# alasdairtran/fourierflow

Measured on AMD Instinct MI355X. Metric: training-steps/sec (whole node), F-FNO 24L 64x64 torus (torus_li/markov/24_layers), higher is better.
Workload: dtype f32

## Files before the change

### fourierflow_amd/_capi.py

```python
from __future__ import annotations

import ctypes as C

ABI_VERSION = 13
BRANCH_SELF_RANGE = 1

P = C.c_void_p
I = C.c_int
F = C.c_float
SZ = C.c_size_t
L = C.c_long


class WnDesc(C.Structure):
    _fields_ = [("g", P), ("v", P), ("w", P), ("dw", P), ("dg", P), ("dv", P),
                ("rows", C.c_int32), ("cols", C.c_int32)]


class FxPackDesc(C.Structure):
    _fields_ = [("src", P), ("dst", P), ("sh", C.c_int32), ("sc", C.c_int32), ("type", C.c_int32), ("pad_", C.c_int32)]


class FusedBranch(C.Structure):
    _fields_ = [("in_", P), ("out", P), ("resid", P), ("spec_save", P), ("planes", P), ("tw", P),
                ("B", C.c_int32), ("M", C.c_int32), ("N", C.c_int32),
                ("K", C.c_int32), ("axis", C.c_int32), ("accumulate", C.c_int32),
                ("planes_format", C.c_int32), ("tile_lines", C.c_int32), ("in_amax", P), ("out_amax", P),
                ("storage", C.c_int32), ("flags", C.c_int32), ("dft_frags", P)]


class FfOpts(C.Structure):
    _fields_ = [("in_amax", P), ("out_amax", P), ("max_workgroups", C.c_int32), ("schedule", C.c_int32),
                ("storage", C.c_int32)]


class LayerFwdDesc(C.Structure):
    _fields_ = [("a", FusedBranch), ("b", FusedBranch), ("branch_kernel", C.c_int32), ("interleave", C.c_int32),
                ("pk1", P), ("b1", P), ("pk2", P), ("b2", P), ("s_sum", P), ("resid", P), ("out", P), ("mask", P),
                ("P", C.c_int32), ("C", C.c_int32), ("H", C.c_int32), ("ff_kernel", C.c_int32),
                ("ff_schedule", C.c_int32), ("ff_max_workgroups", C.c_int32), ("pad0_", C.c_int32), ("pad1_", C.c_int32), ("out_amax", P)]


class LayerBwdDesc(C.Structure):
    _fields_ = [("a", FusedBranch), ("b", FusedBranch), ("branch_kernel", C.c_int32), ("interleave", C.c_int32),
                ("g", P), ("g2", P), ("g_sum", P), ("mask", P), ("pk1b", P), ("pk2b", P), ("ds", P), ("s", P), ("pk1", P),
                ("b1", P), ("partial", P), ("nsplit", C.c_int32), ("P", C.c_int32), ("C", C.c_int32), ("H", C.c_int32),
                ("ff_kernel", C.c_int32), ("ff_schedule", C.c_int32), ("ff_max_workgroups", C.c_int32), ("pad_", C.c_int32), ("g_amax", P), ("s_amax", P), ("ds_amax", P)]


class LayerInferDesc(C.Structure):
    _fields_ = [("a", FusedBranch), ("b", FusedBranch), ("interleave", C.c_int32), ("pad_", C.c_int32),
                ("pk1", P), ("b1", P), ("pk2", P), ("b2", P), ("resid", P), ("out", P), ("C", C.c_int32), ("H", C.c_int32),
                ("out_amax", P)]


class InferStackLayer(C.Structure):
    _fields_ = [("planes_a", P), ("planes_b", P), ("pk1", P), ("b1", P), ("pk2", P), ("b2", P)]


class InferStackDesc(C.Structure):
    _fields_ = [("a", FusedBranch), ("b", FusedBranch), ("layers", P), ("n_layers", C.c_int32), ("C", C.c_int32), ("H", C.c_int32),
                ("mode", C.c_int32), ("last_out", P), ("sync", P)]


class AmaxDesc(C.Structure):
    _fields_ = [("x", P), ("n", C.c_size_t)]


class FxRedDesc(C.Structure):
    _fields_ = [("partial", P), ("dW1", P), ("dW2", P), ("db1", P), ("db2", P)]


class FfWgDesc(C.Structure):
    _fields_ = [("s", P), ("g", P), ("pk1", P), ("b1", P), ("pk1b", P), ("partial", P), ("s_amax", P), ("g_amax", P),
                ("s2", P), ("g2", P)]


class MarkovExtra(C.Structure):
    _fields_ = [("force", P), ("mu", P), ("use_position", C.c_int32), ("pad_", C.c_int32)]


class MarkovAdvanceDesc(C.Structure):
    _fields_ = [("affine", P), ("prev", P), ("traj", P), ("feats", P), ("derived", P), ("force", P), ("mu", P),
                ("force_stride", C.c_int64), ("L", C.c_int32), ("col", C.c_int32), ("D", C.c_int32),
                ("use_position", C.c_int32), ("normalize", C.c_int32), ("low", C.c_float), ("high", C.c_float),
                ("pad_", C.c_int32)]


class PadMap(C.Structure):
    _fields_ = [("size", C.c_int32 * 3), ("padded", C.c_int32 * 3)]


class PadDesc(C.Structure):
    _fields_ = [("plain", P), ("padded", P), ("R", C.c_int32), ("Cc", C.c_int32), ("inner", C.c_int32), ("Cp", C.c_int32)]


class FwPackDesc(C.Structure):
    _fields_ = [("w", P), ("wp", P), ("wpt", P), ("K", C.c_int32), ("real", C.c_int32)]


class X3PackDesc(C.Structure):
    _fields_ = [("planes", P), ("dst", P), ("K", C.c_int32), ("format", C.c_int32)]


class TrDesc(C.Structure):
    _fields_ = [("src", P), ("dst", P), ("rows", C.c_int32), ("cols", C.c_int32)]


class IPhiParams(C.Structure):
    NAMES = ("fc0.weight", "fc0.bias", "fc_code.weight", "fc_code.bias", "fc1.weight", "fc1.bias", "fc2.weight", "fc2.bias",
             "fc3.weight", "fc3.bias", "fc4.weight", "fc4.bias")
    _fields_ = [(n, P) for n in ("fc0_w", "fc0_b", "code_w", "code_b", "fc1_w", "fc1_b", "fc2_w", "fc2_b", "fc3_w", "fc3_b",
                                 "fc4_w", "fc4_b")]


class PcHeadParams(C.Structure):
    _fields_ = [(n, P) for n in ("bs_w", "bs_b", "fc1_w", "fc1_b", "fc2_w", "fc2_b")]


class GatherField(C.Structure):
    _fields_ = [("src", P), ("dst", P), ("src_sample", C.c_int64), ("src_offset", C.c_int64), ("src_q", C.c_int64),
                ("src_r", C.c_int64), ("dst_sample", C.c_int64), ("dst_offset", C.c_int64), ("dst_q", C.c_int64),
                ("dst_r", C.c_int64), ("Q", C.c_int32), ("R", C.c_int32)]


GATHER_MAX_FIELDS = 8

SIGNATURES = {
    "ffno_build_target": (C.c_char_p, []),
    "ffno_abi_version": (I, []),
    "ffno_amax": (I, [P, SZ, P, P]),
    "ffno_amax_batched": (I, [P, I, SZ, P, P]),
    "ffno_lds_tr16_probe": (I, [P, I, P, P, P]),
    "ffno_twiddle_fill_host": (I, [P, I]),
    "ffno_dft_fwd": (I, [P, P, P, I, I, I, I, I, I, I, P]),
    "ffno_fw_pack": (I, [P, P, P, I, I, P]),
    "ffno_fw_pack_batched": (I, [P, I, I, I, P]),
    "ffno_mode_mix": (I, [P, P, P, I, I, I, I, P]),
    "ffno_dft_inv": (I, [P, P, P, P, I, I, I, I, I, I, I, I, P]),
    "ffno_fw_grad_partial": (I, [P, P, P, I, I, I, I, I, I, SZ, SZ, P]),
    "ffno_fw_grad_partial_multi": (I, [P, P, P, I, I, I, I, I, SZ, SZ, SZ, P]),
    "ffno_fw_grad_reduce_multi": (I, [P, P, I, I, I, I, SZ, I, I, P]),
    "ffno_fw_grad_partial_h2": (I, [P, P, P, I, I, I, I, I, I, SZ, SZ, P, P, I, P]),
    "ffno_fw_grad_partial_multi_h2": (I, [P, P, P, I, I, I, I, I, SZ, SZ, SZ, P, P, I, P]),
    "ffno_fw_grad_reduce": (I, [P, P, I, I, I, I, P]),
    "ffno_spectral_fused_pair": (I, [P, P, I, I, I, I, P]),
    "ffno_spectral_x3_supported": (I, [I, I, I]),
    "ffno_spectral_x3_pack_bytes": (SZ, [I, I]),
    "ffno_spectral_x3_dft_frags_bytes": (SZ, [I, I]),
    "ffno_spectral_x3_dft_frags": (I, [P, I, I, I, I, P, P]),
    "ffno_spectral_x3_pack": (I, [P, I, I, I, P]),
    "ffno_spectral_x3": (I, [P, I, I, I, I, P]),
    "ffno_spectral_x3_pair": (I, [P, P, I, I, I, I, I, P]),
    "ffno_spectral_x3_staged_supported": (I, [I, I, I]),
    "ffno_spectral_x3_staged_pair": (I, [P, P, P, P, I, I, I, I, P]),
    "ffno_layer_fwd": (I, [P, P]),
    "ffno_layer_bwd": (I, [P, P]),
    "ffno_infer_mix_bytes": (SZ, [I, I, I]),
    "ffno_layer_infer_supported": (I, [I, I, I, I, I, I, I]),
    "ffno_spectral_x3_mix_pair": (I, [P, P, I, I, P]),
    "ffno_infer_ff": (I, [P, P, P, P, P, P, P, P, I, I, P, P]),
    "ffno_infer_sum": (I, [P, P, P, I, P, P]),
    "ffno_layer_infer": (I, [P, P]),
    "ffno_infer_stack_supported": (I, [I, I, I, I, I, I, I, I]),
    "ffno_infer_stack_sync_words": (SZ, [I]),
    "ffno_infer_stack_trace_words": (SZ, [I]),
    "ffno_infer_stack": (I, [P, P]),
    "ffno_spectral_staged_pair": (I, [P, P, P, P, I, I, I, I, P]),
    "ffno_spectral_fused_supported": (I, [I, I, I]),
    "ffno_spectral_fused": (I, [P, P, P, P, P, P, I, I, I, I, I, I, I, I, I, I, P, P]),
    "ffno_spectral2d_ws_floats": (SZ, [I, I, I, I, I]),
    "ffno_spectral2d_path": (I, [I, I, I, I, I]),
    "ffno_spectral2d_weights_version": (I, [P, C.c_ulonglong]),
    "ffno_spectral2d_fwd": (I, [P, P, P, P, P, P, P, I, I, I, I, I, I, P]),
    "ffno_spectral2d_bwd": (I, [P, P, P, P, P, P, P, P, P, P, I, I, I, I, I, I, I, I, P]),
    "ffno_ff_mask_words": (SZ, [I, I]),
    "ffno_ff_fwd": (I, [P, P, P, P, P, P, P, P, P, I, I, I, P]),
    "ffno_ff_bwd_data": (I, [P, P, P, P, P, P, I, I, I, P]),
    "ffno_ff_wgrad_partial_floats": (SZ, [I, I, I]),
    "ffno_ff_bwd_weights_partial": (I, [P, P, P, P, P, I, I, I, I, P]),
    "ffno_ff_bwd_weights_reduce": (I, [P, P, P, P, P, I, I, I, I, P]),
    "ffno_ffx_supported": (I, [I, I]),
    "ffno_ffx_pack_bytes": (SZ, [I, I]),
    "ffno_ffx_pack": (I, [P, I, I, I, P]),
    "ffno_ffx_fwd": (I, [P, P, P, P, P, P, P, P, I, I, I, P]),
    "ffno_ffx_mask_unpack": (I, [P, P, I, I, I, P]),
    "ffno_ffx_bwd_data": (I, [P, P, P, P, P, I, I, I, P]),
    "ffno_ffx_fwd2": (I, [P, P, P, P, P, P, P, P, P, P, I, I, I, P, P]),
    "ffno_ffx_bwd_data2": (I, [P, P, P, P, P, P, P, I, I, I, P, P]),
    "ffno_ffx_bwd_weights_partial": (I, [P, P, P, P, P, P, I, I, I, I, P]),
    "ffno_ffx_bwd_weights_reduce": (I, [P, P, P, P, P, I, I, I, I, P]),
    "ffno_ffx_bwd_weights_reduce_batched": (I, [P, I, I, I, I, P]),
    "ffno_ffh_pack_bytes": (SZ, [I, I]),
    "ffno_ffh_pack": (I, [P, I, I, I, P]),
    "ffno_ffh_fwd2": (I, [P, P, P, P, P, P, P, P, P, P, I, I, I, P, P]),
    "ffno_ffh_bwd_data2": (I, [P, P, P, P, P, P, P, I, I, I, P, P]),
    "ffno_ffh_bwd_weights_partial": (I, [P, P, P, P, P, P, I, I, I, I, P, P, I, P]),
    "ffno_ffh_bwd_weights_partial_multi": (I, [P, I, I, I, I, I, I, I, P]),
    "ffno_layernorm_fwd": (I, [P, P, P, P, P, P, L, I, F, P]),
    "ffno_layernorm_nsplit": (I, [L]),
    "ffno_layernorm_bwd": (I, [P, P, P, P, P, P, P, P, P, P, L, I, I, P]),
    "ffno_weightnorm_fwd": (I, [P, I, I, P]),
    "ffno_weightnorm_bwd": (I, [P, I, I, P]),
    "ffno_transpose_batched": (I, [P, I, I, I, P]),
    "ffno_lift_fwd": (I, [P, P, P, P, I, I, I, P, P, P]),
    "ffno_lift_bwd": (I, [P, P, P, P, P, I, I, I, I, I, P, P]),
    "ffno_lift_bwd2": (I, [P, P, P, P, P, P, I, I, I, I, I, P, P]),
    "ffno_lift_bwd_data": (I, [P, P, P, I, I, I, P, P]),
    "ffno_lift_fwd_bf16": (I, [P, P, P, P, I, I, I, P, P, P]),
    "ffno_lift_bwd_bf16": (I, [P, P, P, P, P, I, I, I, I, I, P, P]),
    "ffno_head_fwd_bf16": (I, [P, P, P, I, I, I, I, P, P]),
    "ffno_head_bwd_bf16": (I, [P, P, P, P, P, P, I, I, I, I, P, P, P]),
    "ffno_head_fold": (I, [P, P, P, P, P, I, I, I, P]),
    "ffno_head_fwd": (I, [P, P, P, I, I, I, I, P, P]),
    "ffno_head_bwd": (I, [P, P, P, P, P, P, I, I, I, I, P, P, P]),
    "ffno_head_param_grads": (I, [P, P, P, P, P, P, P, P, I, I, I, I, P]),
    "ffno_cdft_rows": (I, [P, P, I, I, I, I, I, P]),
    "ffno_fw2d_pack": (I, [P, P, P, P, I, I, P]),
    "ffno_fw2d_grad_reduce": (I, [P, P, P, I, I, I, I, P]),
    "ffno_cdft_rows2": (I, [P, P, I, I, I, I, I, I, P]),
    "ffno_fw3d_pack": (I, [P, P, P, P, P, P, I, I, I, I, P]),
    "ffno_fw3d_grad_reduce": (I, [P, P, P, P, P, I, I, I, I, I, I, P]),
    "ffno_dct_branch": (I, [P, P, P, P, P, P, P, I, I, I, I, I, I, I, I, P]),
    "ffno_fw_pack_real": (I, [P, P, P, I, I, P]),
    "ffno_mode_mix_real": (I, [P, P, P, I, I, I, P]),
    "ffno_fw_grad_reduce_real": (I, [P, P, I, I, I, I, P]),
    "ffno_cdft_rows_ws_floats": (SZ, [I, I, I, I]),
    "ffno_cdft_rows_mfma": (I, [P, P, P, P, I, I, I, I, I, I, P]),
    "ffno_fw2d_pack2": (I, [P, P, P, P, I, I, I, P]),
    "ffno_fw2d_grad_reduce2": (I, [P, P, P, I, I, I, I, I, P]),
    "ffno_plin_supported": (I, [I, I]),
    "ffno_plin_fwd": (I, [P, I, P, P, P, P, I, P, P, P, L, I, I, I, P]),
    "ffno_plin_bwd_data": (I, [P, I, P, P, P, I, P, L, I, I, I, I, P]),
    "ffno_plin_wgrad_nsplit": (I, [L]),
    "ffno_plin_wgrad_partial_floats": (SZ, [L, I, I]),
    "ffno_plin_bwd_weights": (I, [P, I, P, P, I, P, P, P, L, I, I, I, I, P]),
    "ffno_plin_pos_fwd": (I, [P, I, P, P, P, P, P, P, P, I, P, I, I, I, I, I, I, P]),
    "ffno_plin_pos_bwd_weights": (I, [P, I, P, P, I, P, P, P, P, P, P, P, I, I, I, I, I, I, I, P]),
    "ffno_glin_supported": (I, [I, I]),
    "ffno_glin_fwd": (I, [P, P, P, P, P, L, I, I, I, F, C.c_uint32, P]),
    "ffno_glin_bwd_data": (I, [P, P, P, P, L, I, I, F, C.c_uint32, I, P]),
    "ffno_glin_wgrad_nsplit": (I, [L]),
    "ffno_glin_wgrad_partial_floats": (SZ, [L, I, I]),
    "ffno_glin_bwd_weights": (I, [P, P, P, P, P, P, L, I, I, F, C.c_uint32, I, P]),
    "ffno_dropout": (I, [P, SZ, F, C.c_uint32, P]),
    "ffno_dropout_mask": (I, [P, SZ, F, C.c_uint32, P]),
    "ffno_pad_copy": (I, [P, I, I, P]),
    "ffno_velocity_ws_floats": (SZ, [I, I, I]),
    "ffno_velocity_features": (I, [P, P, P, I, I, I, F, F, P]),
    "ffno_lploss_tmp_floats": (SZ, [I, I]),
    "ffno_lploss_fwd_bwd": (I, [P, P, P, P, P, I, I, F, P, P]),
    "ffno_markov_features": (I, [P, P, P, P, P, P, I, I, I, I, F, F, F, F, I, I, P, P]),
    "ffno_markov_traj_ws_floats": (SZ, [I, I, I, I]),
    "ffno_markov_traj_step": (I, [P, P, P, P, P, P, P, I, I, I, I, I, I, P]),
    "ffno_markov_traj_metrics": (I, [P, P, I, I, I, I, F, P]),
    "ffno_vorticity_coarsen_ws_floats": (SZ, [I, I, I]),
    "ffno_vorticity_coarsen_step": (I, [P, P, P, P, I, I, I, I, I, I, I, F, F, P]),
    "ffno_markov_corr_metrics": (I, [P, P, I, I, I, F, P]),
    "ffno_prediction_export_step": (I, [P, P, P, P, I, I, I, I, I, I, F, F, P]),
    "ffno_energy_spectrum": (I, [P, P, P, I, I, P]),
    "ffno_markov_advance": (I, [P, P, P, I, I, I, P]),
    "ffno_markov_pairs": (I, [P, P, P, P, P, P, P, P, P, P, I, I, I, I, I, I, I, I, P]),
    "ffno_markov_pairs_tf": (I, [P, P, P, P, P, P, P, I, P, P, P, I, I, I, I, I, I, I, I, P]),
    "ffno_sample_gather": (I, [P, I, P, I, I, P]),
    "ffno_adamw_flat":(I, [P, P, P, P, SZ, F, F, F, F, F, I, F, P]),
    "ffno_adam_flat": (I, [P, P, P, P, SZ, F, F, F, F, F, I, F, P]),
    "ffno_axpy": (I, [P, P, F, SZ, P]),
    "ffno_nudft_supported": (I, [I, I, I]),
    "ffno_nudft_modes": (I, [P, P, P, I, I, I, I, I, I, P]),
    "ffno_nudft_points": (I, [P, P, P, P, P, I, I, I, I, I, I, I, P]),
    "ffno_nudft_axis_supported": (I, [I, I, I]),
    "ffno_nudft_axis_modes": (I, [P, P, P, I, I, I, I, I, P]),
    "ffno_nudft_axis_points": (I, [P, P, P, P, P, I, I, I, I, I, I, P]),
    "ffno_axis_modes_to_grid": (I, [P, P, I, I, I, I, I, I, P]),
    "ffno_grid_to_axis_modes": (I, [P, P, I, I, I, I, I, I, P]),
    "ffno_iphi_supported": (I, [I]),
    "ffno_iphi_bwd_ws_floats": (SZ, [I, I, I]),
    "ffno_iphi_fwd": (I, [P, P, P, P, P, P, I, I, I, P]),
    "ffno_iphi_bwd": (I, [P, P, P, P, P, P, P, P, P, I, I, I, P]),
    "ffno_pchead_supported": (I, [I, I, I]),
    "ffno_pchead_partial_floats": (SZ, [I, I, I, I]),
    "ffno_pchead_fwd": (I, [P, P, P, P, P, I, I, I, I, P]),
    "ffno_pchead_bwd": (I, [P, P, P, P, P, P, P, P, I, I, I, I, P]),
    "ffno_ns2d_supported": (I, [I]),
    "ffno_ns2d_derivs": (I, [P, P, I, I, P]),
    "ffno_ns2d_advect": (I, [P, P, SZ, P]),
    "ffno_ns2d_cn_update": (I, [P, P, P, P, F, I, I, I, P]),
    "ffno_ns2d_cn_update_harmonic": (I, [P, P, P, P, F, F, F, F, I, I, I, P]),
    "ffno_ns2d_harmonic_force": (I, [P, P, F, F, F, I, I, I, P]),
    "ffno_kf2d_supported": (I, [I]),
    "ffno_kf2d_derivs": (I, [P, P, F, I, I, P]),
    "ffno_kf2d_stage": (I, [P, P, P, F, F, F, F, F, F, F, I, F, F, F, F, I, I, I, P]),
    "ffno_kf2d_downsample": (I, [P, P, I, I, I, F, P]),
}


def bind(lib: C.CDLL):
    for name, (res, args) in SIGNATURES.items():
        fn = getattr(lib, name)
        fn.restype = res
        fn.argtypes = args
    return list(SIGNATURES)


ERRORS = {-1: "FFNO_EINVAL (null pointer / bad size)", -2: "FFNO_EUNSUPPORTED (shape outside the compiled set)",
          -3: "FFNO_EMODES (modes > L/2+1)"}


def check(rc: int, what: str):
    if rc == 0:
        return
    if rc == -3:
        raise ValueError(f"{what}: {ERRORS[rc]}")
    if rc in (-1, -2):
        raise ValueError(f"{what}: {ERRORS[rc]}")
    raise RuntimeError(f"{what}: HIP launch failed with hipError_t {rc}")
```

### fourierflow_amd/csrc/ffx.hip

```cpp
#include <algorithm>

#include "ffno_device.h"
#include "ffno.h"

#include <string.h>

namespace ffno {

constexpr int kFfRangeTarget = 4;

template <int C, int H, int CPW_ = 1>
struct FxCfg {
    static constexpr int CPW = CPW_;
    static constexpr int NW = H / (32 * CPW);
    static constexpr int NT = NW * 64;
    static constexpr int KS = C / 16;
    static constexpr int CTO = C / 32;
    static constexpr int NV = (32 * C / 4) / NT;
    static constexpr int G = CTO * 4;
    static constexpr int GPW = G / NW;
    static constexpr int PROW = 2 * C + 16;
    static constexpr int PPLANE = 32 * PROW;
    static constexpr int TROW = 64 + 16;
    static constexpr int TPLANE = C * TROW;
    static constexpr int PART = 2 * H * C + H + C;
    static_assert(NV >= 1 && NV * NT * 4 == 32 * C, "tile staging map");
    static_assert(GPW >= 1 && GPW * NW == G, "output reduction map");
};

struct FxPackDesc {
    const float* src;
    u32x4* dst;
    int sh, sc, type, pad;
};

template <class S>
__global__ __launch_bounds__(256) void ffx_pack_kernel(const FxPackDesc* __restrict__ descs, int C, int H) {
    const FxPackDesc d = descs[blockIdx.y];
    const int KS = C / 16, CTO = C / 32, NW = H / 32;
    const int nfrag = d.type == 1 ? NW * KS : NW * CTO * 2;
    const int t = blockIdx.x * blockDim.x + threadIdx.x;
    if (t >= nfrag * 64) return;
    const int frag = t >> 6, lane = t & 63, j = lane & 31, half = lane >> 5;
    float v[8];
    if (d.type == 1) {
        const int w = frag / KS, st = frag % KS;
        for (int e = 0; e < 8; ++e) v[e] = d.src[(long)(32 * w + j) * d.sh + (long)(16 * st + 8 * half + e) * d.sc];
    } else {
        const int s2 = frag & 1, mt = (frag >> 1) % CTO, w = (frag >> 1) / CTO;
        for (int e = 0; e < 8; ++e)
            v[e] = d.src[(long)(32 * w + (e & 3) + 8 * (2 * s2 + (e >> 2)) + 4 * half) * d.sh + (long)(32 * mt + j) * d.sc];
    }
    const typename S::Frag f = S::split8(v[0], v[1], v[2], v[3], v[4], v[5], v[6], v[7]);
    FFNO_UNROLL
    for (int p = 0; p < S::NP; ++p) d.dst[(frag * S::NP + p) * 64 + lane] = S::plane(f, p);
}

__device__ __forceinline__ Bf3 load_frag(const u32x4* __restrict__ pk, int frag, int lane) {
    Bf3 f;
    f.hi = pk[(frag * 3 + 0) * 64 + lane];
    f.mid = pk[(frag * 3 + 1) * 64 + lane];
    f.lo = pk[(frag * 3 + 2) * 64 + lane];
    return f;
}

__device__ __forceinline__ uint32_t push_sign(uint32_t acc, uint32_t x) {
    return plat::shift_in_msb(acc, x);
}
__device__ __forceinline__ uint32_t bit_mask(uint32_t x, int b) {
    return plat::bit_to_mask(x, b);
}

__device__ __forceinline__ Bf3 lds_frag(const char* base, int plane_bytes, int off) {
    Bf3 f;
    f.hi = *reinterpret_cast<const u32x4*>(base + off);
    f.mid = *reinterpret_cast<const u32x4*>(base + plane_bytes + off);
    f.lo = *reinterpret_cast<const u32x4*>(base + 2 * plane_bytes + off);
    return f;
}

__device__ __forceinline__ void stage4(char* base, int plane_bytes, int off, float x, float y, float z, float w) {
    unsigned h0, m0, l0, h1, m1, l1;
    split3_pair(x, y, h0, m0, l0);
    split3_pair(z, w, h1, m1, l1);
    *reinterpret_cast<uint2*>(base + off) = make_uint2(h0, h1);
    *reinterpret_cast<uint2*>(base + plane_bytes + off) = make_uint2(m0, m1);
    *reinterpret_cast<uint2*>(base + 2 * plane_bytes + off) = make_uint2(l0, l1);
}

template <class S>
__device__ __forceinline__ typename S::Frag load_frag_s(const u32x4* __restrict__ pk, int frag, int lane) {
    typename S::Frag f;
    FFNO_UNROLL
    for (int p = 0; p < S::NP; ++p) S::set_plane(f, p, pk[(frag * S::NP + p) * 64 + lane]);
    return f;
}
template <class S>
__device__ __forceinline__ typename S::Frag lds_frag_s(const char* base, int plane_bytes, int off) {
    typename S::Frag f;
    FFNO_UNROLL
    for (int p = 0; p < S::NP; ++p) S::set_plane(f, p, *reinterpret_cast<const u32x4*>(base + p * plane_bytes + off));
    return f;
}
template <class S>
__device__ __forceinline__ void stage4_s(char* base, int plane_bytes, int off, float x, float y, float z, float w) {
    uint2 pl[S::NP];
    S::split4(x, y, z, w, pl);
    FFNO_UNROLL
    for (int p = 0; p < S::NP; ++p) *reinterpret_cast<uint2*>(base + p * plane_bytes + off) = pl[p];
}

template <int C, int H, bool BWD, class S, class ST = StF32>
__global__ __launch_bounds__((FxCfg<C, H>::NT)) void ffx_chain_kernel(const typename ST::T* __restrict__ in,
                                                                     const typename ST::T* __restrict__ in2,
                                                                     typename ST::T* sum_out,
                                                                     const typename ST::T* resid,
                                                                     const u32x4* __restrict__ pk1,
                                                                     const float* __restrict__ bias1,
                                                                     const u32x4* __restrict__ pk2,
                                                                     const float* __restrict__ bias2, typename ST::T* out,
                                                                     uint32_t* mask, int P, const unsigned* in_amax, unsigned* out_amax) {
    using F = FxCfg<C, H>;
    constexpr int NW = F::NW, KS = F::KS, CTO = F::CTO, NV = F::NV, G = F::G, GPW = F::GPW, CPW = F::CPW;
    __shared__ __attribute__((aligned(16))) char sp[2][S::NP * F::PPLANE];
    __shared__ __attribute__((aligned(16))) float part[2][NW * G * 64 * 4];
    __shared__ __attribute__((aligned(16))) float b1s[H];
    __shared__ float b2s[C];

    const int tid = threadIdx.x, lane = tid & 63, wave = tid >> 6;
    const int j = lane & 31, half = lane >> 5;
    const int ntiles = (P + 31) >> 5;
    const float gscale = (S::SCALED && in_amax) ? range_scale(*in_amax, 1, kFfRangeTarget) : 1.f;
    const float rgscale = 1.f / gscale;
    float omax = 0.f;
    __shared__ float rfold[NW];

    using Frag = typename S::Frag;
    Frag A1[CPW][KS], A2[CPW][CTO][2];
    FFNO_UNROLL
    for (int ch = 0; ch < CPW; ++ch) {
        const int q = wave * CPW + ch;
        FFNO_UNROLL
        for (int st = 0; st < KS; ++st) A1[ch][st] = load_frag_s<S>(pk1, q * KS + st, lane);
        FFNO_UNROLL
        for (int mt = 0; mt < CTO; ++mt) {
            FFNO_UNROLL
            for (int s2 = 0; s2 < 2; ++s2) A2[ch][mt][s2] = load_frag_s<S>(pk2, (q * CTO + mt) * 2 + s2, lane);
        }
    }
    if (!BWD) {
        for (int e = tid; e < H; e += F::NT) b1s[e] = bias1[e] * gscale;
        for (int e = tid; e < C; e += F::NT) b2s[e] = bias2[e];
    }

    float4 nS[NV];
    typename ST::Raw4 pA[NV], pB[NV];
    auto gload_raw = [&](int tile) {
        FFNO_UNROLL
        for (int v = 0; v < NV; ++v) {
            const int f = tid + v * F::NT;
            const long px = (long)tile * 32 + f / (C / 4);
            pA[v] = pB[v] = ST::zero4();
            if (px < P) {
                const long off = px * C + 4 * (f % (C / 4));
                pA[v] = ST::ldr4(in + off);
                if (in2) pB[v] = ST::ldr4(in2 + off);
            }
        }
    };
    auto consume = [&](int tile) {
        FFNO_UNROLL
        for (int v = 0; v < NV; ++v) {
            nS[v] = ST::w4(pA[v]);
            if (in2) {
                const float4 b = ST::w4(pB[v]);
                nS[v].x += b.x, nS[v].y += b.y, nS[v].z += b.z, nS[v].w += b.w;
                nS[v] = st_rnd4<ST>(nS[v]);
                if (sum_out) {
                    const int f = tid + v * F::NT;
                    const long px = (long)tile * 32 + f / (C / 4);
                    if (px < P) ST::st4(sum_out + px * C + 4 * (f % (C / 4)), nS[v]);
                }
            }
            if (S::SCALED) nS[v].x *= gscale, nS[v].y *= gscale, nS[v].z *= gscale, nS[v].w *= gscale;
        }
    };
    auto stage = [&](int buf) {
        FFNO_UNROLL
        for (int v = 0; v < NV; ++v) {
            const int f = tid + v * F::NT;
            stage4_s<S>(sp[buf], F::PPLANE, (f / (C / 4)) * F::PROW + (f % (C / 4)) * 8, nS[v].x, nS[v].y, nS[v].z, nS[v].w);
        }
    };
    typename ST::Raw4 rres[GPW], rnext[GPW];
    auto rload = [&](int tile) {
        const long px = (long)tile * 32 + j;
        FFNO_UNROLL
        for (int u = 0; u < GPW; ++u) {
            const int gi = wave * GPW + u;
            rnext[u] = ST::zero4();
            if (!BWD && resid && px < P)
                rnext[u] = ST::ldr4(resid + px * C + 32 * (gi >> 2) + 8 * (gi & 3) + 4 * half);
        }
    };
    auto reduce = [&](int tile, int buf) {
        const long px = (long)tile * 32 + j;
        FFNO_UNROLL
        for (int u = 0; u < GPW; ++u) {
// ... 1544 lines not shown
```

### fourierflow_amd/csrc/pointwise.hip

```cpp
#include "ffno_device.h"
#include "ffno.h"

#include <math.h>

namespace ffno {

static inline int pw_status() {
    hipError_t e = hipGetLastError();
    return e == hipSuccess ? FFNO_OK : (int)e;
}

__global__ __launch_bounds__(256) void wn_fwd_kernel(const ffno_wn_desc* __restrict__ descs) {
    const ffno_wn_desc d = descs[blockIdx.y];
    const int lane = threadIdx.x & 63, row = blockIdx.x * 4 + (threadIdx.x >> 6);
    if (row >= d.rows) return;
    const float* v = d.v + (long)row * d.cols;
    float ss = 0.f;
    for (int c = lane; c < d.cols; c += 64) ss += v[c] * v[c];
    ss = wave_sum(ss);
    const float scale = d.g[row] / sqrtf(ss);
    float* w = d.w + (long)row * d.cols;
    for (int c = lane; c < d.cols; c += 64) w[c] = v[c] * scale;
}

__global__ __launch_bounds__(256) void wn_bwd_kernel(const ffno_wn_desc* __restrict__ descs) {
    const ffno_wn_desc d = descs[blockIdx.y];
    const int lane = threadIdx.x & 63, row = blockIdx.x * 4 + (threadIdx.x >> 6);
    if (row >= d.rows) return;
    const float* v = d.v + (long)row * d.cols;
    const float* dw = d.dw + (long)row * d.cols;
    float ss = 0.f, dot = 0.f;
    for (int c = lane; c < d.cols; c += 64) {
        ss += v[c] * v[c];
        dot += dw[c] * v[c];
    }
    ss = wave_sum(ss);
    dot = wave_sum(dot);
    const float inv = 1.f / sqrtf(ss);
    const float dg = dot * inv;
    const float g = d.g[row];
    if (lane == 0) d.dg[row] = dg;
    float* dv = d.dv + (long)row * d.cols;
    for (int c = lane; c < d.cols; c += 64) dv[c] = g * inv * (dw[c] - dg * inv * v[c]);
}

__global__ __launch_bounds__(256) void transpose_batched_kernel(const ffno_tr_desc* __restrict__ descs) {
    __shared__ float tile[32][33];
    const ffno_tr_desc d = descs[blockIdx.z];
    const int c0 = blockIdx.x * 32, r0 = blockIdx.y * 32;
    if (c0 >= d.cols || r0 >= d.rows) return;
    const int tx = threadIdx.x & 31, ty = threadIdx.x >> 5;
    for (int yy = ty; yy < 32; yy += 8)
        if (r0 + yy < d.rows && c0 + tx < d.cols) tile[yy][tx] = d.src[(long)(r0 + yy) * d.cols + c0 + tx];
    __syncthreads();
    for (int yy = ty; yy < 32; yy += 8)
        if (c0 + yy < d.cols && r0 + tx < d.rows) d.dst[(long)(c0 + yy) * d.rows + r0 + tx] = tile[tx][yy];
}

struct PadMapDev {
    int s1, s2;
    int p0, p1, p2;
    int s0;
    int enabled;
    __device__ __forceinline__ long map(long p) const {
        if (!enabled) return p;
        const long z = p % s2, t = p / s2;
        const long y = t % s1, t2 = t / s1;
        const long x = t2 % s0, b = t2 / s0;
        return ((b * p0 + x) * p1 + y) * p2 + z;
    }
};

static inline PadMapDev make_padmap(const ffno_padmap* pm) {
    PadMapDev d;
    d.enabled = 0;
    d.s0 = d.s1 = d.s2 = d.p0 = d.p1 = d.p2 = 1;
    if (pm) {
        d.s0 = pm->size[0];
        d.s1 = pm->size[1];
        d.s2 = pm->size[2];
        d.p0 = pm->padded[0];
        d.p1 = pm->padded[1];
        d.p2 = pm->padded[2];
        d.enabled = (d.s0 != d.p0 || d.s1 != d.p1 || d.s2 != d.p2) ? 1 : 0;
    }
    return d;
}

template <int C, class ST = StF32>
__global__ __launch_bounds__(512) void lift_fwd_kernel(const float* __restrict__ x, const float* __restrict__ W,
                                                       const float* __restrict__ b, typename ST::T* __restrict__ out, int P,
                                                       int Cin, PadMapDev pm, unsigned* out_amax) {
    FFNO_DYN_SMEM(smem);
    __shared__ float rfold[16];
    float omax = 0.f;
    float* Wt = reinterpret_cast<float*>(smem);
    for (int e = threadIdx.x; e < Cin * C; e += blockDim.x) Wt[(e % Cin) * C + (e / Cin)] = W[e];
    for (int e = threadIdx.x; e < C; e += blockDim.x) Wt[Cin * C + e] = b[e];
    __syncthreads();
    constexpr int LPP = C / 4;
    const int PPB = (int)blockDim.x / LPP;
    const int c4 = (threadIdx.x % LPP) * 4, pl = threadIdx.x / LPP;
    const float4 bias = *reinterpret_cast<const float4*>(Wt + Cin * C + c4);
    const long stride = (long)gridDim.x * PPB;
    for (long p = (long)blockIdx.x * PPB + pl; p < P; p += 2 * stride) {
        const long p1 = p + stride;
        const bool two = p1 < P;
        float4 acc0 = bias, acc1 = bias;
        const float* xp0 = x + p * Cin;
        const float* xp1 = x + (two ? p1 : p) * Cin;
        for (int i = 0; i < Cin; ++i) {
            const float xv0 = xp0[i], xv1 = xp1[i];
            const float4 w = *reinterpret_cast<const float4*>(Wt + i * C + c4);
            acc0.x = fmaf(xv0, w.x, acc0.x);
            acc0.y = fmaf(xv0, w.y, acc0.y);
            acc0.z = fmaf(xv0, w.z, acc0.z);
            acc0.w = fmaf(xv0, w.w, acc0.w);
            acc1.x = fmaf(xv1, w.x, acc1.x);
            acc1.y = fmaf(xv1, w.y, acc1.y);
            acc1.z = fmaf(xv1, w.z, acc1.z);
            acc1.w = fmaf(xv1, w.w, acc1.w);
        }
        ST::st4(out + pm.map(p) * C + c4, acc0);
        acc0 = st_rnd4<ST>(acc0);
        omax = fmaxf(fmaxf(omax, fmaxf(fabsf(acc0.x), fabsf(acc0.y))), fmaxf(fabsf(acc0.z), fabsf(acc0.w)));
        if (two) {
            ST::st4(out + pm.map(p1) * C + c4, acc1);
            acc1 = st_rnd4<ST>(acc1);
            omax = fmaxf(fmaxf(omax, fmaxf(fabsf(acc1.x), fabsf(acc1.y))), fmaxf(fabsf(acc1.z), fabsf(acc1.w)));
        }
    }
    if (out_amax) range_fold(omax, rfold, (int)blockDim.x >> 6, out_amax);
}

template <int C, class ST = StF32>
__global__ __launch_bounds__(256) void lift_bwd_partial_kernel(const float* __restrict__ x,
                                                               const typename ST::T* __restrict__ gout,
                                                               const typename ST::T* __restrict__ gout2,
                                                               float* __restrict__ partial, int P, int Cin,
                                                               int chunk, PadMapDev pm) {
    constexpr int TP = 32;
    constexpr int MAXU = (C * 64) / 256;
    __shared__ __attribute__((aligned(16))) float gs[TP * C];
    __shared__ float xs[TP * 64];
    const int npairs = C * (Cin + 1);
    float acc[MAXU];
    FFNO_UNROLL
    for (int u = 0; u < MAXU; ++u) acc[u] = 0.f;
    const long pbeg = (long)blockIdx.x * chunk, pend = min((long)P, pbeg + chunk);
    for (long p0 = pbeg; p0 < pend; p0 += TP) {
        const int np = (int)min((long)TP, pend - p0);
        __syncthreads();
        for (int e4 = threadIdx.x; e4 < TP * C / 4; e4 += 256) {
            const int e = 4 * e4;
            float4 gvv = make_float4(0.f, 0.f, 0.f, 0.f);
            if ((e / C) < np) {
                const long off = pm.map(p0 + e / C) * C + (e % C);
                gvv = ST::ld4(gout + off);
                if (gout2) {
                    const float4 g2 = ST::ld4(gout2 + off);
                    gvv = make_float4(ST::rnd(gvv.x + g2.x), ST::rnd(gvv.y + g2.y), ST::rnd(gvv.z + g2.z), ST::rnd(gvv.w + g2.w));
                }
            }
            *reinterpret_cast<float4*>(gs + e) = gvv;
        }
        for (int e = threadIdx.x; e < TP * (Cin + 1); e += 256) {
            const int pp = e / (Cin + 1), i = e % (Cin + 1);
            xs[pp * 64 + i] = (pp < np) ? (i < Cin ? x[(p0 + pp) * Cin + i] : 1.f) : 0.f;
        }
        __syncthreads();
        FFNO_UNROLL
        for (int u = 0; u < MAXU; ++u) {
            const int e = u * 256 + threadIdx.x;
            if (e < npairs) {
                const int c = e % C, i = e / C;
                float a = acc[u];
                for (int pp = 0; pp < TP; ++pp) a = fmaf(gs[pp * C + c], xs[pp * 64 + i], a);
                acc[u] = a;
            }
        }
    }
    FFNO_UNROLL
    for (int u = 0; u < MAXU; ++u) {
        const int e = u * 256 + threadIdx.x;
        if (e < npairs) partial[(long)blockIdx.x * npairs + e] = acc[u];
    }
}

template <int C>
__global__ __launch_bounds__(256) void lift_bwd_data_kernel(const float* __restrict__ gout, const float* __restrict__ W,
                                                            float* __restrict__ dx, int P, int Cin, PadMapDev pm) {
    FFNO_DYN_SMEM(smem);
    float* Wt = reinterpret_cast<float*>(smem);
    for (int e = threadIdx.x; e < Cin * C; e += blockDim.x) Wt[(e % Cin) * C + (e / Cin)] = W[e];
    __syncthreads();
    for (long p = (long)blockIdx.x * 256 + threadIdx.x; p < P; p += (long)gridDim.x * 256) {
        const float* g = gout + pm.map(p) * C;
        float4 gv[C / 4];
        FFNO_UNROLL
        for (int q = 0; q < C / 4; ++q) gv[q] = *reinterpret_cast<const float4*>(g + 4 * q);
        for (int i = 0; i < Cin; ++i) {
            float a = 0.f;
            FFNO_UNROLL
            for (int q = 0; q < C / 4; ++q) {
                const float4 w = *reinterpret_cast<const float4*>(Wt + i * C + 4 * q);
                a = fmaf(gv[q].x, w.x, a), a = fmaf(gv[q].y, w.y, a), a = fmaf(gv[q].z, w.z, a), a = fmaf(gv[q].w, w.w, a);
            }
            dx[p * Cin + i] = a;
        }
    }
}

__global__ __launch_bounds__(256) void lift_bwd_reduce_kernel(const float* __restrict__ partial, float* dW, float* db,
                                                              int Cin, int C, int nsplit, int accumulate) {
    __shared__ float red[256];
    const int npairs = C * (Cin + 1);
    const int e = blockIdx.x * 4 + (threadIdx.x & 3), lane = threadIdx.x >> 2;
    float a = 0.f;
    if (e < npairs)
        for (int sp = lane; sp < nsplit; sp += 64) a += partial[(long)sp * npairs + e];
    red[threadIdx.x] = a;
    __syncthreads();
    for (int w = 128; w >= 4; w >>= 1) {
        if ((int)threadIdx.x < w) red[threadIdx.x] += red[threadIdx.x + w];
        __syncthreads();
    }
    if (threadIdx.x < 4 && e < npairs) {
        const int c = e % C, i = e / C;
        float* dst = (i < Cin) ? (dW + c * Cin + i) : (db + c);
        *dst = accumulate ? (*dst + red[threadIdx.x]) : red[threadIdx.x];
    }
}

static constexpr int kHeadMaxOut = 8;

__global__ __launch_bounds__(256) void head_fold_kernel(const float* __restrict__ Wa, const float* __restrict__ ca,
                                                        const float* __restrict__ Wb, const float* __restrict__ cb,
                                                        float* fold, int C, int D, int O) {
    const int e = blockIdx.x * 4 + (threadIdx.x >> 6), lane = threadIdx.x & 63;
    if (e >= O * (C + 1)) return;
    const int o = e / (C + 1), c = e % (C + 1);
    float s = 0.f;
    for (int jd = lane; jd < D; jd += 64) s = fmaf(Wb[o * D + jd], (c == C) ? ca[jd] : Wa[jd * C + c], s);
    FFNO_UNROLL
    for (int m = 32; m >= 1; m >>= 1) s += __shfl_xor(s, m);
    if (lane == 0) fold[e] = s + ((c == C) ? cb[o] : 0.f);
}

template <int C, class ST = StF32>
__global__ __launch_bounds__(256) void head_fwd_kernel(const typename ST::T* __restrict__ b, const float* __restrict__ fold,
                                                       float* y, int P, int O, int accumulate, PadMapDev pm) {
    constexpr int LPP = C / 4, PPB = 256 / LPP;
    const int c4 = (threadIdx.x % LPP) * 4, pl = threadIdx.x / LPP;
    const long npass = ((long)P + PPB - 1) / PPB;
    for (long pass = blockIdx.x; pass < npass; pass += gridDim.x) {
        const long p = pass * PPB + pl;
        float4 v = make_float4(0.f, 0.f, 0.f, 0.f);
        if (p < P) v = ST::ld4(b + pm.map(p) * C + c4);
        for (int o = 0; o < O; ++o) {
            const float4 w = *reinterpret_cast<const float4*>(fold + o * (C + 1) + c4);
            float d = v.x * w.x + v.y * w.y + v.z * w.z + v.w * w.w;
            FFNO_UNROLL
            for (int m = LPP / 2; m >= 1; m >>= 1) d += __shfl_xor(d, m);
            if (p < P && c4 == 0) y[p * O + o] = (accumulate ? y[p * O + o] : 0.f) + d + fold[o * (C + 1) + C];
        }
    }
}

template <int C, class ST = StF32>
__global__ __launch_bounds__(1024) void head_bwd_kernel(const typename ST::T* __restrict__ b, const float* __restrict__ gy,
                                                        const float* __restrict__ fold, typename ST::T* __restrict__ gb,
                                                        float* __restrict__ partial, int P, int O, PadMapDev pm,
                                                        unsigned* gb_amax) {
    constexpr int LPP = C / 4;
    const int PPB = (int)blockDim.x / LPP;
    __shared__ float red[(1024 / LPP) * (C + 4)];
    __shared__ float rfold[16];
    float omax = 0.f;
    const int l = threadIdx.x % LPP, c4 = l * 4, pl = threadIdx.x / LPP;
    float4 acc[kHeadMaxOut];
    float sg[kHeadMaxOut];
    FFNO_UNROLL
    for (int o = 0; o < kHeadMaxOut; ++o) {
        acc[o] = make_float4(0.f, 0.f, 0.f, 0.f);
        sg[o] = 0.f;
    }
    for (long p = (long)blockIdx.x * PPB + pl; p < P; p += (long)gridDim.x * PPB) {
        const long q = pm.map(p);
        const float4 v = ST::ld4(b + q * C + c4);
        float4 gsum = make_float4(0.f, 0.f, 0.f, 0.f);
        FFNO_UNROLL
        for (int o = 0; o < kHeadMaxOut; ++o) {
            if (o < O) {
                const float g = gy[p * O + o];
                const float4 w = *reinterpret_cast<const float4*>(fold + o * (C + 1) + c4);
                acc[o].x = fmaf(g, v.x, acc[o].x);
                acc[o].y = fmaf(g, v.y, acc[o].y);
                acc[o].z = fmaf(g, v.z, acc[o].z);
                acc[o].w = fmaf(g, v.w, acc[o].w);
                sg[o] += g;
                gsum.x = fmaf(g, w.x, gsum.x);
                gsum.y = fmaf(g, w.y, gsum.y);
                gsum.z = fmaf(g, w.z, gsum.z);
                gsum.w = fmaf(g, w.w, gsum.w);
            }
        }
        if (gb) ST::st4(gb + q * C + c4, gsum);
        gsum = st_rnd4<ST>(gsum);
        omax = fmaxf(fmaxf(omax, fmaxf(fabsf(gsum.x), fabsf(gsum.y))), fmaxf(fabsf(gsum.z), fabsf(gsum.w)));
    }
    if (gb && gb_amax) range_fold(omax, rfold, (int)blockDim.x >> 6, gb_amax);
    for (int o = 0; o < O; ++o) {
        __syncthreads();
        float* r = red + pl * (C + 4);
        FFNO_UNROLL
        for (int oo = 0; oo < kHeadMaxOut; ++oo) {
            if (oo == o) {
                r[c4] = acc[oo].x;
                r[c4 + 1] = acc[oo].y;
                r[c4 + 2] = acc[oo].z;
                r[c4 + 3] = acc[oo].w;
                if (l == 0) r[C] = sg[oo];
            }
        }
        __syncthreads();
        for (int e = threadIdx.x; e <= C; e += blockDim.x) {
            float s = 0.f;
            for (int qq = 0; qq < PPB; ++qq) s += red[qq * (C + 4) + e];
            partial[((long)blockIdx.x * O + o) * (C + 1) + e] = s;
        }
    }
}

__global__ __launch_bounds__(256) void head_bwd_reduce_kernel(const float* __restrict__ partial, float* red, int C, int O,
                                                              int nsplit) {
    __shared__ float sm[256];
    const int n = O * (C + 1);
    const int e = blockIdx.x * 4 + (threadIdx.x & 3), lane = threadIdx.x >> 2;
    float a = 0.f;
    if (e < n)
        for (int sp = lane; sp < nsplit; sp += 64) a += partial[(long)sp * n + e];
    sm[threadIdx.x] = a;
    __syncthreads();
    for (int w = 128; w >= 4; w >>= 1) {
        if ((int)threadIdx.x < w) sm[threadIdx.x] += sm[threadIdx.x + w];
        __syncthreads();
    }
    if (threadIdx.x < 4 && e < n) red[e] = sm[threadIdx.x];
}

__global__ __launch_bounds__(256) void head_param_grads_kernel(const float* __restrict__ red, const float* __restrict__ Wa,
                                                               const float* __restrict__ ca, const float* __restrict__ Wb,
                                                               float* dWa, float* dca, float* dWb, float* dcb, int C, int D,
                                                               int O, int accumulate) {
    const int n0 = O * D, n1 = n0 + D, n2 = n1 + D * C, n3 = n2 + O;
    for (int idx = blockIdx.x * blockDim.x + threadIdx.x; idx < n3; idx += gridDim.x * blockDim.x) {
        if (idx < n0) {
            const int e = idx, o = e / D, jd = e % D;
            float s = ca[jd] * red[o * (C + 1) + C];
            for (int c = 0; c < C; ++c) s = fmaf(Wa[jd * C + c], red[o * (C + 1) + c], s);
            dWb[e] = accumulate ? dWb[e] + s : s;
        } else if (idx < n1) {
            const int jd = idx - n0;
            float t = 0.f;
            for (int o = 0; o < O; ++o) t = fmaf(Wb[o * D + jd], red[o * (C + 1) + C], t);
            dca[jd] = accumulate ? dca[jd] + t : t;
        } else if (idx < n2) {
            const int e = idx - n1;
            float t = 0.f;
            for (int o = 0; o < O; ++o) t = fmaf(Wb[o * D + e / C], red[o * (C + 1) + e % C], t);
            dWa[e] = accumulate ? dWa[e] + t : t;
        } else {
            const int o = idx - n2;
            const float S = red[o * (C + 1) + C];
            dcb[o] = accumulate ? dcb[o] + S : S;
        }
    }
}

struct MarkovSrc {
    const float* x;
    const float* force;
    const float* mu;
    int Cx, use_pos;
    long fstride;
};

__device__ __forceinline__ float markov_normalized(float v, const float* derived, int c, int D) {
    return (v - derived[c]) / derived[D + c];
}

__device__ __forceinline__ float markov_raw(const MarkovSrc& src, long p, int c, int M, int N, float low, float high) {
    if (c < src.Cx) return src.x[p * src.Cx + c];
    c -= src.Cx;
    if (src.use_pos) {
        if (c < 2) {
            const int n = (int)(p % N), m = (int)((p / N) % M);
            const int idx = c == 0 ? m : n, size = c == 0 ? M : N;
            return size > 1 ? low + (high - low) * (float)idx / (float)(size - 1) : low;
// ... 229 lines not shown
        metrics[4 + t] = l / (float)B;
        metrics[4 + n_steps + t] = p / (float)B;
    }
    float f = 0.f;
    for (int b = threadIdx.x; b < B; b += 256) {
        float d2 = 0.f, y2 = 0.f;
        for (int t = 0; t < n_steps; ++t) d2 += slice_sum(t, b, 5), y2 += slice_sum(t, b, 3);
        f += sqrtf(d2) / sqrtf(y2);
    }
    full[threadIdx.x] = f;
    __syncthreads();
    if (threadIdx.x == 0) {
        float lf = 0.f, la = 0.f, pm = 0.f;
        for (int i = 0; i < min(B, 256); ++i) lf += full[i];
        int diverged = n_steps;
        for (int t = n_steps - 1; t >= 0; --t)
            if (metrics[4 + n_steps + t] < threshold) diverged = t;
        for (int t = 0; t < n_steps; ++t) la += metrics[4 + t], pm += metrics[4 + n_steps + t];
        metrics[0] = la / (float)n_steps;
        metrics[1] = lf / (float)B;
        metrics[2] = (float)diverged;
        metrics[3] = pm / (float)n_steps;
    }
}

struct MarkovPairs {
    const float* data;
    const int32_t* ids;
    float *x, *y, *dx, *dy;
    const float* f;
    float* f_out;
    const float* mu;
    float* mu_out;
    int n, T, t0, k, P, total;
    int Tf;
};

__global__ __launch_bounds__(256) void markov_pairs_kernel(MarkovPairs a) {
    const int i = blockIdx.y, S = gridDim.x;
    const int chunk = (a.n + S - 1) / S;
    const int beg = blockIdx.x * chunk, end = min(a.n, beg + chunk);
    const int p = a.ids[i];
    const bool ok = (unsigned)p < (unsigned)a.total;
    const int b = ok ? p / a.P : 0, t = ok ? a.t0 + p % a.P : 0;
    const float nan = __builtin_nanf("");
    const long src = (long)b * a.n, dst = (long)i * a.n;
    if (a.mu_out && blockIdx.x == 0 && threadIdx.x == 0) a.mu_out[i] = ok ? a.mu[b] : nan;
    for (int e = beg + threadIdx.x; e < end; e += 256) {
        float xv = nan, yv = nan, pv = nan, fv = nan;
        if (ok) {
            const float* row = a.data + (src + e) * a.T;
            xv = row[t];
            if (a.y || a.dy) yv = row[t + a.k];
            if (a.dx) pv = row[t - a.k];
            if (a.f_out) fv = a.Tf ? a.f[(src + e) * a.Tf + t + a.k] : a.f[src + e];
        }
        if (a.x) a.x[dst + e] = xv;
        if (a.y) a.y[dst + e] = yv;
        if (a.dx) a.dx[dst + e] = xv - pv;
        if (a.dy) a.dy[dst + e] = yv - xv;
        if (a.f_out) a.f_out[dst + e] = fv;
    }
}

struct GatherField {
    const float* src;
    float* dst;
    long src_sample, src_offset, src_q, src_r, dst_sample, dst_offset, dst_q, dst_r;
    int Q, R, vec;
};
struct SampleGather {
    GatherField f[FFNO_GATHER_MAX_FIELDS];
    const int32_t* ids;
    int n;
};

__global__ __launch_bounds__(256) void sample_gather_kernel(SampleGather a) {
    const GatherField& g = a.f[blockIdx.z];
    const int i = blockIdx.y, S = gridDim.x;
    const int id = a.ids[i];
    if ((unsigned)id >= (unsigned)a.n) return;
    const float* sp = g.src + (long)id * g.src_sample + g.src_offset;
    float* dp = g.dst + (long)i * g.dst_sample + g.dst_offset;
    const bool wide = g.vec && (((uintptr_t)sp | (uintptr_t)dp) & 15) == 0;
    const int W = wide ? 4 : 1;
    const int U = (g.R + W - 1) / W;
    const long units = (long)g.Q * U;
    const long chunk = (units + S - 1) / S;
    const long beg = blockIdx.x * chunk, end = beg + chunk < units ? beg + chunk : units;
    for (long u = beg + threadIdx.x; u < end; u += 256) {
        const long q = u / U;
        const int r = (int)(u - q * U) * W;
        const float* s = sp + q * g.src_q + r * g.src_r;
        float* d = dp + q * g.dst_q + r * g.dst_r;
        if (wide && r + 4 <= g.R) {
            *reinterpret_cast<float4*>(d) = *reinterpret_cast<const float4*>(s);
        } else {
            const int m = min(W, g.R - r);
            for (int j = 0; j < m; ++j) d[j * g.dst_r] = s[j * g.src_r];
        }
    }
}

__global__ __launch_bounds__(256) void adamw_kernel(float* __restrict__ p, const float* __restrict__ g,
                                                    float* __restrict__ m, float* __restrict__ v, size_t n, float lr,
                                                    float beta1, float beta2, float eps, float wd, float bc1,
                                                    float bc2_sqrt, float gscale, int decoupled) {
    for (size_t i = (size_t)blockIdx.x * 256 + threadIdx.x; i < n; i += (size_t)gridDim.x * 256) {
        const float gi = decoupled ? g[i] * gscale : fmaf(wd, p[i], g[i] * gscale);
        float pi = decoupled ? p[i] * (1.f - lr * wd) : p[i];
        const float mi = beta1 * m[i] + (1.f - beta1) * gi;
        const float vi = beta2 * v[i] + (1.f - beta2) * gi * gi;
        m[i] = mi;
        v[i] = vi;
        const float denom = sqrtf(vi) / bc2_sqrt + eps;
        pi -= (lr / bc1) * (mi / denom);
        p[i] = pi;
    }
}

__global__ __launch_bounds__(256) void axpy_kernel(float* __restrict__ y, const float* __restrict__ x, float alpha,
                                                   size_t n) {
    for (size_t i = (size_t)blockIdx.x * 256 + threadIdx.x; i < n; i += (size_t)gridDim.x * 256)
        y[i] = fmaf(alpha, x[i], y[i]);
}

}

using namespace ffno;

__global__ __launch_bounds__(256) void amax_kernel(const float* __restrict__ x, size_t n, unsigned* word) {
    __shared__ float red[4];
    float m = 0.f;
    const size_t n4 = n / 4;
    for (size_t i = (size_t)blockIdx.x * 256 + threadIdx.x; i < n4; i += (size_t)gridDim.x * 256) {
        const float4 v = reinterpret_cast<const float4*>(x)[i];
        m = fmaxf(fmaxf(m, fmaxf(fabsf(v.x), fabsf(v.y))), fmaxf(fabsf(v.z), fabsf(v.w)));
    }
    for (size_t i = 4 * n4 + (size_t)blockIdx.x * 256 + threadIdx.x; i < n; i += (size_t)gridDim.x * 256) m = fmaxf(m, fabsf(x[i]));
    range_fold(m, red, 4, word);
}
extern "C" int ffno_amax(const float* x, size_t n, uint32_t* word, void* stream) {
    if (!x || !word || n == 0 || (reinterpret_cast<uintptr_t>(x) & 15u)) return FFNO_EINVAL;
    const int blocks = (int)std::min<size_t>((size_t)4 * device_cu_count(), (n / 4 + 255) / 256 + 1);
    FFNO_LAUNCH(amax_kernel, dim3(blocks), dim3(256), 0, (hipStream_t)stream, x, n, word);
    hipError_t e = hipGetLastError();
    return e == hipSuccess ? FFNO_OK : (int)e;
}

struct AmaxDesc {
    const float* x;
    size_t n;
};
__global__ __launch_bounds__(256) void amax_batched_kernel(const AmaxDesc* __restrict__ descs, unsigned* word) {
    __shared__ float red[4];
    const AmaxDesc d = descs[blockIdx.y];
    const size_t act = min((size_t)gridDim.x, (d.n + 1023) / 1024);
    if (blockIdx.x >= act) return;
    float m = 0.f;
    const bool al = (reinterpret_cast<uintptr_t>(d.x) & 15u) == 0;
    const size_t n4 = al ? d.n / 4 : 0;
    for (size_t i = (size_t)blockIdx.x * 256 + threadIdx.x; i < n4; i += act * 256) {
        const float4 v = reinterpret_cast<const float4*>(d.x)[i];
        m = fmaxf(fmaxf(m, fmaxf(fabsf(v.x), fabsf(v.y))), fmaxf(fabsf(v.z), fabsf(v.w)));
    }
    for (size_t i = 4 * n4 + (size_t)blockIdx.x * 256 + threadIdx.x; i < d.n; i += act * 256) m = fmaxf(m, fabsf(d.x[i]));
    range_fold(m, red, 4, word);
}
extern "C" int ffno_amax_batched(const ffno_amax_desc* descs_dev, int n, size_t max_n, uint32_t* word, void* stream) {
    static_assert(sizeof(ffno_amax_desc) == sizeof(AmaxDesc), "descriptor layout");
    if (!descs_dev || !word || n <= 0 || max_n == 0) return FFNO_EINVAL;
    const int blocks = (int)std::min<size_t>(128, (max_n + 2047) / 2048);
    FFNO_LAUNCH(amax_batched_kernel, dim3(blocks, n), dim3(256), 0, (hipStream_t)stream,
                reinterpret_cast<const AmaxDesc*>(descs_dev), word);
    hipError_t e = hipGetLastError();
    return e == hipSuccess ? FFNO_OK : (int)e;
}

extern "C" const char* ffno_build_target(void) {
    return FFNO_BUILD_TARGET;
}
extern "C" int ffno_abi_version(void) { return FFNO_ABI_VERSION; }

extern "C" int ffno_twiddle_fill_host(float* tw_host, int L) {
    if (!tw_host || L <= 0) return FFNO_EINVAL;
    const double inv = 1.0 / sqrt((double)L);
    for (int jx = 0; jx < L; ++jx) {
        const double th = 2.0 * M_PI * (double)jx / (double)L;
        double c = cos(th), s = sin(th);
        if (4 * jx == L || 4 * jx == 3 * L) c = 0.0;
        if (jx == 0 || 2 * jx == L) s = 0.0;
        tw_host[jx] = (float)(c * inv);
        tw_host[L + jx] = (float)(s * inv);
    }
    return FFNO_OK;
}

extern "C" int ffno_weightnorm_fwd(const ffno_wn_desc* descs_dev, int n, int max_rows, void* stream) {
    if (!descs_dev || n <= 0 || max_rows <= 0) return FFNO_EINVAL;
    FFNO_LAUNCH(wn_fwd_kernel, dim3((max_rows + 3) / 4, n), dim3(256), 0, (hipStream_t)stream, descs_dev);
    return pw_status();
}
extern "C" int ffno_weightnorm_bwd(const ffno_wn_desc* descs_dev, int n, int max_rows, void* stream) {
    if (!descs_dev || n <= 0 || max_rows <= 0) return FFNO_EINVAL;
    FFNO_LAUNCH(wn_bwd_kernel, dim3((max_rows + 3) / 4, n), dim3(256), 0, (hipStream_t)stream, descs_dev);
    return pw_status();
}

extern "C" int ffno_transpose_batched(const ffno_tr_desc* descs_dev, int n, int max_rows, int max_cols, void* stream) {
    if (!descs_dev || n <= 0 || max_rows <= 0 || max_cols <= 0) return FFNO_EINVAL;
    FFNO_LAUNCH(transpose_batched_kernel, dim3((max_cols + 31) / 32, (max_rows + 31) / 32, n), dim3(256), 0,
                (hipStream_t)stream, descs_dev);
    return pw_status();
}

template <class ST>
static int lift_fwd_impl(const float* x, const float* W, const float* b, typename ST::T* out, int P, int Cin, int C,
                         const ffno_padmap* pad, uint32_t* out_amax, void* stream) {
    if (!x || !W || !b || !out || P <= 0 || Cin <= 0) return FFNO_EINVAL;
    if (Cin > 63) return FFNO_EUNSUPPORTED;
    const PadMapDev pm = make_padmap(pad);
    const size_t smem = sizeof(float) * (size_t)(Cin + 1) * C;
    const int ppb = 512 / (C / 4);
    const dim3 grid((unsigned)min(((long)P + ppb - 1) / ppb, (long)device_cu_count())), block(512);
    hipStream_t s = (hipStream_t)stream;
    if (C == 64)
        FFNO_LAUNCH((lift_fwd_kernel<64, ST>), grid, block, smem, s, x, W, b, out, P, Cin, pm, out_amax);
    else if (C == 32)
        FFNO_LAUNCH((lift_fwd_kernel<32, ST>), grid, block, smem, s, x, W, b, out, P, Cin, pm, out_amax);
    else
        return FFNO_EUNSUPPORTED;
    return pw_status();
}
extern "C" int ffno_lift_fwd(const float* x, const float* W, const float* b, float* out, int P, int Cin, int C,
                             const ffno_padmap* pad, uint32_t* out_amax, void* stream) {
    return lift_fwd_impl<StF32>(x, W, b, out, P, Cin, C, pad, out_amax, stream);
}
extern "C" int ffno_lift_fwd_bf16(const float* x, const float* W, const float* b, uint16_t* out, int P, int Cin, int C,
                                  const ffno_padmap* pad, uint32_t* out_amax, void* stream) {
    return lift_fwd_impl<StBf16>(x, W, b, out, P, Cin, C, pad, out_amax, stream);
}

template <class ST>
static int lift_bwd_impl(const float* x, const typename ST::T* gout, const typename ST::T* gout2, float* partial, float* dW, float* db,
                         int P, int Cin, int C, int nsplit, int accumulate, const ffno_padmap* pad, void* stream) {
    if (!x || !gout || !partial || !dW || !db || P <= 0 || Cin <= 0 || nsplit <= 0) return FFNO_EINVAL;
    if (Cin > 63) return FFNO_EUNSUPPORTED;
    const PadMapDev pm = make_padmap(pad);
    const int chunk = (P + nsplit - 1) / nsplit;
    hipStream_t s = (hipStream_t)stream;
    if (C == 64)
        FFNO_LAUNCH((lift_bwd_partial_kernel<64, ST>), dim3(nsplit), dim3(256), 0, s, x, gout, gout2, partial, P, Cin, chunk, pm);
    else if (C == 32)
        FFNO_LAUNCH((lift_bwd_partial_kernel<32, ST>), dim3(nsplit), dim3(256), 0, s, x, gout, gout2, partial, P, Cin, chunk, pm);
    else
        return FFNO_EUNSUPPORTED;
    int rc = pw_status();
    if (rc) return rc;
    const int npairs = C * (Cin + 1);
    FFNO_LAUNCH(lift_bwd_reduce_kernel, dim3((npairs + 3) / 4), dim3(256), 0, s, partial, dW, db, Cin, C, nsplit,
                accumulate);
    return pw_status();
}
extern "C" int ffno_lift_bwd(const float* x, const float* gout, float* partial, float* dW, float* db, int P,
                             int Cin, int C, int nsplit, int accumulate, const ffno_padmap* pad, void* stream) {
    return lift_bwd_impl<StF32>(x, gout, nullptr, partial, dW, db, P, Cin, C, nsplit, accumulate, pad, stream);
}
extern "C" int ffno_lift_bwd2(const float* x, const float* gout, const float* gout2, float* partial, float* dW, float* db, int P,
                              int Cin, int C, int nsplit, int accumulate, const ffno_padmap* pad, void* stream) {
    return lift_bwd_impl<StF32>(x, gout, gout2, partial, dW, db, P, Cin, C, nsplit, accumulate, pad, stream);
}
extern "C" int ffno_lift_bwd_bf16(const float* x, const uint16_t* gout, float* partial, float* dW, float* db, int P,
                                  int Cin, int C, int nsplit, int accumulate, const ffno_padmap* pad, void* stream) {
    return lift_bwd_impl<StBf16>(x, gout, nullptr, partial, dW, db, P, Cin, C, nsplit, accumulate, pad, stream);
}

extern "C" int ffno_lift_bwd_data(const float* gout, const float* W, float* dx, int P, int Cin, int C,
                                  const ffno_padmap* pad, void* stream) {
    if (!gout || !W || !dx || P <= 0 || Cin <= 0) return FFNO_EINVAL;
    if (Cin > 63) return FFNO_EUNSUPPORTED;
    const PadMapDev pm = make_padmap(pad);
    const dim3 grid((unsigned)std::min<long>(((long)P + 255) / 256, 4L * device_cu_count()));
    const size_t smem = sizeof(float) * (size_t)Cin * C;
    hipStream_t s = (hipStream_t)stream;
    if (C == 64)
        FFNO_LAUNCH((lift_bwd_data_kernel<64>), grid, dim3(256), smem, s, gout, W, dx, P, Cin, pm);
    else if (C == 32)
        FFNO_LAUNCH((lift_bwd_data_kernel<32>), grid, dim3(256), smem, s, gout, W, dx, P, Cin, pm);
    else
        return FFNO_EUNSUPPORTED;
    return pw_status();
}

extern "C" int ffno_head_fold(const float* Wa, const float* ca, const float* Wb, const float* cb, float* fold,
                              int C, int D, int O, void* stream) {
    if (!Wa || !ca || !Wb || !cb || !fold || C <= 0 || D <= 0 || O <= 0) return FFNO_EINVAL;
    if (O > kHeadMaxOut) return FFNO_EUNSUPPORTED;
    FFNO_LAUNCH(head_fold_kernel, dim3((O * (C + 1) + 3) / 4), dim3(256), 0, (hipStream_t)stream, Wa, ca, Wb, cb, fold, C,
                D, O);
    return pw_status();
}

template <class ST>
static int head_fwd_impl(const typename ST::T* b, const float* fold, float* y, int P, int C, int O, int accumulate,
                         const ffno_padmap* pad, void* stream) {
    if (!b || !fold || !y || P <= 0 || O <= 0) return FFNO_EINVAL;
    if (O > kHeadMaxOut) return FFNO_EUNSUPPORTED;
    const PadMapDev pm = make_padmap(pad);
    const int ppb = 256 / (C / 4);
    const dim3 grid((unsigned)min(((long)P + ppb - 1) / ppb, 2048L)), block(256);
    hipStream_t s = (hipStream_t)stream;
    if (C == 64)
        FFNO_LAUNCH((head_fwd_kernel<64, ST>), grid, block, 0, s, b, fold, y, P, O, accumulate, pm);
    else if (C == 32)
        FFNO_LAUNCH((head_fwd_kernel<32, ST>), grid, block, 0, s, b, fold, y, P, O, accumulate, pm);
    else
        return FFNO_EUNSUPPORTED;
    return pw_status();
}
extern "C" int ffno_head_fwd(const float* b, const float* fold, float* y, int P, int C, int O, int accumulate,
// ... 236 lines not shown
```

### fourierflow_amd/csrc/spectral.hip

```cpp
#include "ffno_device.h"
#include "ffno_lines.h"
#include "ffno.h"

namespace ffno {

template <int CT>
struct ColVec;
template <>
struct ColVec<1> {
    float v[1];
    __device__ __forceinline__ void load(const float* p) { v[0] = p[0]; }
    __device__ __forceinline__ void store(float* p) const { p[0] = v[0]; }
};
template <>
struct ColVec<2> {
    float v[2];
    __device__ __forceinline__ void load(const float* p) {
        float2 t = *reinterpret_cast<const float2*>(p);
        v[0] = t.x;
        v[1] = t.y;
    }
    __device__ __forceinline__ void store(float* p) const { *reinterpret_cast<float2*>(p) = make_float2(v[0], v[1]); }
};

template <int C, int RT>
__device__ __forceinline__ void dft_fwd_body(const float* __restrict__ x, float* __restrict__ spec,
                                             const float* __restrict__ tw, int R, int L, int K, const LineMap& lm,
                                             int scale_ck, int bidx, int nblk, int Lv) {
    constexpr int CT = C / 32;
    FFNO_DYN_SMEM(smem);
    float* tws = reinterpret_cast<float*>(smem);
    for (int i = threadIdx.x; i < 2 * L; i += blockDim.x) tws[i] = tw[i];
    __syncthreads();

    const int lane = threadIdx.x & 63, wave = threadIdx.x >> 6;
    const int j = lane & 31, half = lane >> 5;
    const int nsteps = (Lv + 1) >> 1;

    const long nitems = (long)R * RT;
    for (long item = (long)bidx * 4 + wave; item < nitems; item += (long)nblk * 4) {
        const int line = (int)(item / RT), rt = (int)(item % RT);
        const int kk = 32 * rt + j, k = kk >> 1, ri = kk & 1;
        const bool valid = kk < 2 * K;
        const float ck = (scale_ck && !(k == 0 || 2 * k == L)) ? 2.f : 1.f;
        const float amul = valid ? (ri ? -ck : ck) : 0.f;
        const int tbase = ri ? L : 0;
        const int km = valid ? k : 0;
        const int step = (2 * km) % L;
        int idx = (km * half) % L;
        const float* xl = x + lm.base(line) + CT * j;
        f32x16 acc[CT];
        FFNO_UNROLL
        for (int ct = 0; ct < CT; ++ct) acc[ct] = zero16();
        constexpr int UN = 8;
        ColVec<CT> b[UN], bn[UN];
        auto load_trip = [&](ColVec<CT> (&dst)[UN], int t0) {
            FFNO_UNROLL
            for (int u = 0; u < UN; ++u) {
                const int n = 2 * (t0 + u) + half;
                if (n < Lv) {
                    dst[u].load(xl + (long)n * lm.elem_stride);
                } else {
                    FFNO_UNROLL
                    for (int ct = 0; ct < CT; ++ct) dst[u].v[ct] = 0.f;
                }
            }
        };
        load_trip(bn, 0);
        for (int t0 = 0; t0 < nsteps; t0 += UN) {
            FFNO_UNROLL
            for (int u = 0; u < UN; ++u) b[u] = bn[u];
            if (t0 + UN < nsteps) load_trip(bn, t0 + UN);
            FFNO_UNROLL
            for (int u = 0; u < UN; ++u) {
                const float a = amul * tws[tbase + idx];
                idx += step;
                if (idx >= L) idx -= L;
                FFNO_UNROLL
                for (int ct = 0; ct < CT; ++ct) acc[ct] = mfma32(a, b[u].v[ct], acc[ct]);
            }
        }
        FFNO_UNROLL
        for (int r = 0; r < 16; ++r) {
            const int kr = 32 * rt + drow(r, half);
            if (kr < 2 * K) {
                ColVec<CT> o;
                FFNO_UNROLL
                for (int ct = 0; ct < CT; ++ct) o.v[ct] = acc[ct][r];
                o.store(spec + (((long)(kr >> 1) * R + line) * 2 + (kr & 1)) * C + CT * j);
            }
        }
    }
}

template <int C, int RT>
__global__ __launch_bounds__(256) void dft_fwd_kernel(const float* __restrict__ x, float* __restrict__ spec,
                                                      const float* __restrict__ tw, int R, int L, int K,
                                                      LineMap lm, int scale_ck) {
    dft_fwd_body<C, RT>(x, spec, tw, R, L, K, lm, scale_ck, blockIdx.x, gridDim.x, L);
}

template <int C, int RT>
__global__ __launch_bounds__(256) void dft_fwd_lv_kernel(const float* __restrict__ x, float* __restrict__ spec,
                                                         const float* __restrict__ tw, int R, int L, int K, LineMap lm,
                                                         int scale_ck, int Lv) {
    dft_fwd_body<C, RT>(x, spec, tw, R, L, K, lm, scale_ck, blockIdx.x, gridDim.x, Lv);
}

struct StageArgs {
    const float* in;
    float* out;
    const float* resid;
    const float* planes;
    const float* tw;
    int R, L, K;
    LineMap lm;
    int accumulate;
};

template <int C, int RT>
__global__ __launch_bounds__(256) void dft_fwd_pair_kernel(StageArgs a, StageArgs b, int n0, int scale_ck) {
    if ((int)blockIdx.x < n0)
        dft_fwd_body<C, RT>(a.in, a.out, a.tw, a.R, a.L, a.K, a.lm, scale_ck, blockIdx.x, n0, a.L);
    else
        dft_fwd_body<C, RT>(b.in, b.out, b.tw, b.R, b.L, b.K, b.lm, scale_ck, blockIdx.x - n0, gridDim.x - n0, b.L);
}

template <int C>
__device__ __forceinline__ void dft_inv_body(const float* __restrict__ spec, float* out, const float* resid,
                                             const float* __restrict__ tw, int R, int L, int K, const LineMap& lm,
                                             int apply_ck, int accumulate, int bidx, int nblk, int Lv) {
    constexpr int CT = C / 32;
    FFNO_DYN_SMEM(smem);
    float* tws = reinterpret_cast<float*>(smem);
    for (int i = threadIdx.x; i < 2 * L; i += blockDim.x) tws[i] = tw[i];
    __syncthreads();

    const int lane = threadIdx.x & 63, wave = threadIdx.x >> 6;
    const int j = lane & 31, half = lane >> 5;
    const float sgn = half ? -1.f : 1.f;
    const int tbase = half ? L : 0;
    const int RTtot = (Lv + 31) >> 5;

    const int NP = (RTtot + 1) >> 1;
    const long nitems = (long)R * NP;
    for (long item = (long)bidx * 4 + wave; item < nitems; item += (long)nblk * 4) {
        const int line = (int)(item / NP);
        const long lbase = lm.base(line) + CT * j;
        {
            const int rt0 = 2 * (int)(item % NP);
            const int n0 = 32 * rt0 + j, n1 = n0 + 32;
            const int st0 = n0 % L, st1 = n1 % L;
            int i0 = 0, i1 = 0;
            f32x16 acc[2][CT];
            FFNO_UNROLL
            for (int q = 0; q < 2; ++q) {
                FFNO_UNROLL
                for (int ct = 0; ct < CT; ++ct) acc[q][ct] = zero16();
            }
            ColVec<CT> b[4], bn[4];
            auto load_trip = [&](ColVec<CT> (&dst)[4], int t0) {
                FFNO_UNROLL
                for (int u = 0; u < 4; ++u) {
                    const int t = t0 + u;
                    if (t < K) {
                        dst[u].load(spec + (((long)t * R + line) * 2 + half) * C + CT * j);
                    } else {
                        FFNO_UNROLL
                        for (int ct = 0; ct < CT; ++ct) dst[u].v[ct] = 0.f;
                    }
                }
            };
            load_trip(bn, 0);
            for (int t0 = 0; t0 < K; t0 += 4) {
                FFNO_UNROLL
                for (int u = 0; u < 4; ++u) b[u] = bn[u];
                if (t0 + 4 < K) load_trip(bn, t0 + 4);
                FFNO_UNROLL
                for (int u = 0; u < 4; ++u) {
                    const int t = t0 + u;
                    const float ck = (apply_ck && !(t == 0 || 2 * t == L)) ? 2.f : 1.f;
                    const float a0 = sgn * ck * tws[tbase + i0];
                    const float a1 = sgn * ck * tws[tbase + i1];
                    i0 += st0;
                    if (i0 >= L) i0 -= L;
                    i1 += st1;
                    if (i1 >= L) i1 -= L;
                    FFNO_UNROLL
                    for (int ct = 0; ct < CT; ++ct) {
                        acc[0][ct] = mfma32(a0, b[u].v[ct], acc[0][ct]);
                        acc[1][ct] = mfma32(a1, b[u].v[ct], acc[1][ct]);
                    }
                }
            }
            FFNO_UNROLL
            for (int q = 0; q < 2; ++q) {
                FFNO_UNROLL
                for (int r = 0; r < 16; ++r) {
                    const int n = 32 * (rt0 + q) + drow(r, half);
                    if (n < Lv) {
                        const long a = lbase + (long)n * lm.elem_stride;
                        ColVec<CT> o;
                        FFNO_UNROLL
                        for (int ct = 0; ct < CT; ++ct) o.v[ct] = acc[q][ct][r];
                        if (accumulate) {
                            ColVec<CT> p;
                            p.load(out + a);
                            FFNO_UNROLL
                            for (int ct = 0; ct < CT; ++ct) o.v[ct] += p.v[ct];
                        }
                        if (resid) {
                            ColVec<CT> p;
                            p.load(resid + a);
                            FFNO_UNROLL
                            for (int ct = 0; ct < CT; ++ct) o.v[ct] += p.v[ct];
                        }
                        o.store(out + a);
                    }
                }
            }
        }
    }
}

template <int C>
__global__ __launch_bounds__(256) void dft_inv_kernel(const float* __restrict__ spec, float* out,
                                                      const float* resid, const float* __restrict__ tw,
                                                      int R, int L, int K, LineMap lm, int apply_ck,
                                                      int accumulate) {
    dft_inv_body<C>(spec, out, resid, tw, R, L, K, lm, apply_ck, accumulate, blockIdx.x, gridDim.x, L);
}

template <int C>
__global__ __launch_bounds__(256) void dft_inv_lv_kernel(const float* __restrict__ spec, float* out, const float* resid,
                                                         const float* __restrict__ tw, int R, int L, int K, LineMap lm,
                                                         int apply_ck, int accumulate, int Lv) {
    dft_inv_body<C>(spec, out, resid, tw, R, L, K, lm, apply_ck, accumulate, blockIdx.x, gridDim.x, Lv);
}

template <int C>
__global__ __launch_bounds__(256) void dft_inv_pair_kernel(StageArgs a, StageArgs b, int n0, int apply_ck) {
    if ((int)blockIdx.x < n0)
        dft_inv_body<C>(a.in, a.out, a.resid, a.tw, a.R, a.L, a.K, a.lm, apply_ck, a.accumulate, blockIdx.x, n0, a.L);
    else
        dft_inv_body<C>(b.in, b.out, b.resid, b.tw, b.R, b.L, b.K, b.lm, apply_ck, b.accumulate, blockIdx.x - n0,
                        gridDim.x - n0, b.L);
}

__global__ void fw_pack_kernel(const float* __restrict__ w, float* __restrict__ wp, float* __restrict__ wpt,
                               int C, int K) {
    const long total = (long)C * C * K * 2;
    for (long e = (long)blockIdx.x * blockDim.x + threadIdx.x; e < total; e += (long)gridDim.x * blockDim.x) {
        const int o = e % C;
        const int i = (e / C) % C;
        const int ri = (e / ((long)C * C)) % 2;
        const int k = e / ((long)C * C * 2);
        const float v = w[(((long)i * C + o) * K + k) * 2 + ri];
        wp[e] = v;
        wpt[(((long)k * 2 + ri) * C + o) * C + i] = v;
    }
}

__global__ void fw_pack_batched_kernel(const ffno_fwpack_desc* __restrict__ descs, int C) {
    const ffno_fwpack_desc d = descs[blockIdx.y];
    const int K = d.K;
    const long total = (long)C * C * K * 2;
    for (long e = (long)blockIdx.x * blockDim.x + threadIdx.x; e < total; e += (long)gridDim.x * blockDim.x) {
        const int o = e % C;
        const int i = (e / C) % C;
        const int ri = (e / ((long)C * C)) % 2;
        const int k = e / ((long)C * C * 2);
        const float v = d.real ? (ri ? 0.f : d.w[((long)i * C + o) * K + k]) : d.w[(((long)i * C + o) * K + k) * 2 + ri];
        d.wp[e] = v;
        d.wpt[(((long)k * 2 + ri) * C + o) * C + i] = v;
    }
}

template <int C, bool REAL = false>
__device__ __forceinline__ void mode_mix_body(const float* __restrict__ spec_in, const float* __restrict__ planes,
                                              float* __restrict__ spec_out, int R, int conj_t, int k) {
    constexpr int CT = C / 32;
    constexpr int PARTS = REAL ? 1 : 2;
    __shared__ __attribute__((aligned(16))) float smem_mix[2 * C * C];
    float* Wr = smem_mix;
    float* Wi = Wr + C * C;

    const int lane = threadIdx.x & 63, wave = threadIdx.x >> 6;
    const int j = lane & 31, half = lane >> 5;
    const float* xin = spec_in + (long)k * R * 2 * C;
    float* yout = spec_out + (long)k * R * 2 * C;
    const int nitems = PARTS * ((R + 31) >> 5);
    int item = blockIdx.x * 4 + wave;

    float a[C];
    auto load_a = [&](int it) {
        const int row = (it / PARTS) * 32 + j;
        FFNO_UNROLL
        for (int u = 0; u < C / 4; ++u) {
            float4 v = make_float4(0.f, 0.f, 0.f, 0.f);
            if (it < nitems && row < R) v = *reinterpret_cast<const float4*>(xin + ((long)row * 2 + half) * C + 4 * u);
            a[4 * u + 0] = v.x;
            a[4 * u + 1] = v.y;
            a[4 * u + 2] = v.z;
            a[4 * u + 3] = v.w;
        }
    };
    load_a(item);
    {
        const float* pk = planes + (long)k * 2 * C * C;
        for (int i = threadIdx.x * 4; i < PARTS * C * C; i += blockDim.x * 4)
            *reinterpret_cast<float4*>(Wr + i) = *reinterpret_cast<const float4*>(pk + i);
    }
    __syncthreads();

    for (; item < nitems; item += gridDim.x * 4) {
        const int row0 = (item / PARTS) * 32, q = REAL ? 0 : (item & 1);
        const float* plane = (REAL || half == q) ? Wr : Wi;
        const float sign = REAL ? 1.f
                                : (conj_t == 0 ? ((half == 1 && q == 0) ? -1.f : 1.f) : ((half == 0 && q == 1) ? -1.f : 1.f));
        f32x16 acc[CT];
        FFNO_UNROLL
        for (int ct = 0; ct < CT; ++ct) acc[ct] = zero16();
        FFNO_UNROLL
        for (int t = 0; t < C; ++t) {
            if ((t & 7) == 0) FFNO_SCHED_FENCE();
            FFNO_UNROLL
            for (int ct = 0; ct < CT; ++ct) {
                const float b = sign * plane[t * C + 32 * ct + j];
                acc[ct] = mfma32(a[t], b, acc[ct]);
            }
        }
        FFNO_SCHED_FENCE();
        load_a(item + gridDim.x * 4);
        FFNO_UNROLL
        for (int ct = 0; ct < CT; ++ct) {
            FFNO_UNROLL
            for (int r = 0; r < 16; ++r) {
                const int row = row0 + drow(r, half);
                if (row < R) yout[((long)row * 2 + q) * C + 32 * ct + j] = acc[ct][r];
            }
        }
    }
}

template <int C>
__global__ __launch_bounds__(256, 2) void mode_mix_kernel(const float* __restrict__ spec_in,
                                                       const float* __restrict__ planes,
                                                       float* __restrict__ spec_out, int R, int K,
                                                       int conj_t) {
    mode_mix_body<C>(spec_in, planes, spec_out, R, conj_t, blockIdx.y);
}

template <int C>
__global__ __launch_bounds__(256, 2) void mode_mix_real_kernel(const float* __restrict__ spec_in,
                                                            const float* __restrict__ planes,
                                                            float* __restrict__ spec_out, int R, int K) {
    mode_mix_body<C, true>(spec_in, planes, spec_out, R, 0, blockIdx.y);
}

template <int C>
__global__ __launch_bounds__(256, 2) void mode_mix_pair_kernel(StageArgs a, StageArgs b, int conj_t) {
    if ((int)blockIdx.y < a.K)
        mode_mix_body<C>(a.in, a.planes, a.out, a.R, conj_t, blockIdx.y);
    else
        mode_mix_body<C>(b.in, b.planes, b.out, b.R, conj_t, blockIdx.y - a.K);
}

template <int C>
struct FusedCfg {
    static constexpr int LINES = 8;
    static constexpr int KMAX = 1024 / C;
    static constexpr int LSMAX = 2 * KMAX * C + 4;
};

struct FusedArgs {
    const float* in;
    float* out;
    const float* resid;
    float* spec_save;
    const float* planes;
    const float* tw;
    int R, L, K;
    LineMap lm;
    int fwd_ck, inv_ck, conj_t, accumulate;
    unsigned* out_amax;
};

template <int C>
__device__ __forceinline__ void spectral_fused_body(const FusedArgs& A, int bidx) {
    const float* __restrict__ in = A.in;
    float* out = A.out;
    const float* resid = A.resid;
    float* __restrict__ spec_save = A.spec_save;
    const float* __restrict__ planes = A.planes;
    const float* __restrict__ tw = A.tw;
    const int R = A.R, L = A.L, K = A.K;
    const LineMap lm = A.lm;
    const int fwd_ck = A.fwd_ck, inv_ck = A.inv_ck, conj_t = A.conj_t, accumulate = A.accumulate;
    using F = FusedCfg<C>;
    constexpr int CT = C / 32;
    __shared__ __attribute__((aligned(16))) float XS[F::LINES * F::LSMAX];
    FFNO_DYN_SMEM(smem);
    float* tws = reinterpret_cast<float*>(smem);
    for (int i = threadIdx.x; i < 2 * L; i += blockDim.x) tws[i] = tw[i];

    const int lane = threadIdx.x & 63, wave = threadIdx.x >> 6;
    const int j = lane & 31, half = lane >> 5;
    const int LS = 2 * K * C + 4;
    const int line = bidx * F::LINES + wave;
    const bool live = line < R;
    float* xs = XS + wave * LS;
    __syncthreads();

    {
        const int kk = j, k = kk >> 1, ri = kk & 1;
        const bool rowok = kk < 2 * K;
        const float ck = (fwd_ck && !(k == 0 || 2 * k == L)) ? 2.f : 1.f;
        const float amul = rowok ? (ri ? -ck : ck) : 0.f;
        const int tbase = ri ? L : 0;
        const int km = rowok ? k : 0;
        const int step = (2 * km) % L;
        int idx = (km * half) % L;
        f32x16 acc[CT];
        FFNO_UNROLL
        for (int ct = 0; ct < CT; ++ct) acc[ct] = zero16();
        if (live) {
            const float* xl = in + lm.base(line) + CT * j;
            const int nsteps = (L + 1) >> 1;
// ... 1288 lines not shown
```

### fourierflow_amd/csrc/spectral_x3.hip

```cpp
#include <type_traits>

#include "ffno_device.h"
#include "ffno_lines.h"
#include "ffno_x3_dft.h"
#include "ffno_infer_body.h"
#include "ffno.h"

namespace ffno {

struct X3Cfg {
    static constexpr int C = 64;
    static constexpr int NW = 8;
    static constexpr int KK = 32;
    static constexpr int RS = 68;
    static constexpr int LSF = KK * RS + 8;
    static constexpr int FRAG = 3 * 64;
    static constexpr int MODE_FRAGS = 16;
};

struct X3Args {
    const float* in;
    float* out;
    const float* resid;
    float* spec_save;
    const u32x4* wpk;
    const float* tw;
    int R, L, K;
    LineMap lm;
    int fwd_ck, inv_ck, conj_t, accumulate;
    const unsigned* in_amax;
    unsigned* out_amax;
    const u32x4* dft;
    u32x4* mix_out;
    float* mix_scale;
    int self_range;
};

struct X3PackDesc {
    const float* planes;
    u32x4* dst;
    int K, format;
};

__global__ __launch_bounds__(256) void x3_pack_kernel(const X3PackDesc* __restrict__ descs) {
    constexpr int C = X3Cfg::C;
    const X3PackDesc d = descs[blockIdx.y];
    const int nfrag = d.K * X3Cfg::MODE_FRAGS;
    const int t = blockIdx.x * blockDim.x + threadIdx.x;
    if (t >= nfrag * 64) return;
    const int frag = t >> 6, lane = t & 63, j = lane & 31, half = lane >> 5;
    const int pt = frag & 3, st = (frag >> 2) & 3, k = frag >> 4;
    const int p = pt >> 1, tt = pt & 1;
    const float* src = d.planes + ((long)(k * 2 + p) * C + (16 * st + 8 * half)) * C + 2 * j + tt;
    float v[8];
    FFNO_UNROLL
    for (int e = 0; e < 8; ++e) v[e] = src[(long)e * C];
    if (d.format == 1) {
        const Hf2 f = split2_8(v[0], v[1], v[2], v[3], v[4], v[5], v[6], v[7]);
        const int fo = (k * 4 + pt) * 4 + st;
        d.dst[(fo * 2 + 0) * 64 + lane] = f.hi;
        d.dst[(fo * 2 + 1) * 64 + lane] = f.lo;
        return;
    }
    if (d.format == 2) {
        const int fm = frag & 15, s2 = fm & 1, t16 = (fm >> 1) & 3, pp = fm >> 3;
        const int j16 = lane & 15, g = lane >> 4;
        const float* src2 = d.planes + ((long)(k * 2 + pp) * C + (32 * s2 + 8 * g)) * C + 4 * j16 + t16;
        float w[8];
        FFNO_UNROLL
        for (int e = 0; e < 8; ++e) w[e] = src2[(long)e * C];
        const Hf2 f = split2_8(w[0], w[1], w[2], w[3], w[4], w[5], w[6], w[7]);
        d.dst[(frag * 2 + 0) * 64 + lane] = f.hi;
        d.dst[(frag * 2 + 1) * 64 + lane] = f.lo;
        return;
    }
    const Bf3 f = split3_8(v[0], v[1], v[2], v[3], v[4], v[5], v[6], v[7]);
    d.dst[(frag * 3 + 0) * 64 + lane] = f.hi;
    d.dst[(frag * 3 + 1) * 64 + lane] = f.mid;
    d.dst[(frag * 3 + 2) * 64 + lane] = f.lo;
}

__device__ __forceinline__ Bf3 x3_load_frag(const u32x4* __restrict__ pk, int frag, int lane) {
    Bf3 f;
    f.hi = pk[(frag * 3 + 0) * 64 + lane];
    f.mid = pk[(frag * 3 + 1) * 64 + lane];
    f.lo = pk[(frag * 3 + 2) * 64 + lane];
    return f;
}

__global__ __launch_bounds__(64) void x3k_dft_frags_kernel(const float* __restrict__ tw, int L, int K, int fwd_ck, int inv_ck,
                                                           X3kDft d, u32x4* __restrict__ out) {
    const int frag = blockIdx.x, lane = threadIdx.x, j = lane & 31, half = lane >> 5;
    float f[8];
    if (frag < d.nfwd) {
        const int u = frag & 3, chunk = (frag >> 2) % d.nchunks, rt = (frag >> 2) / d.nchunks;
        const int kk = 32 * rt + j, k = kk >> 1, ri = kk & 1;
        const bool rowok = kk < 2 * K;
        const float ck = (fwd_ck && !(k == 0 || 2 * k == L)) ? 2.f : 1.f;
        const float amul = rowok ? (ri ? -ck : ck) : 0.f;
        const int km = rowok ? k : 0;
        FFNO_UNROLL
        for (int e = 0; e < 8; ++e) {
            const int n = 16 * (4 * chunk + u) + 8 * half + e;
            f[e] = n < L ? amul * tw[(ri ? L : 0) + (int)(((long)km * n) % L)] : 0.f;
        }
    } else {
        const int g = frag - d.nfwd, st = g % d.NST, tile = g / d.NST;
        const int n = 32 * tile + j;
        FFNO_UNROLL
        for (int e = 0; e < 8; ++e) {
            const int kk = 16 * st + 8 * half + e, t = kk >> 1, part = kk & 1;
            const float ck = (inv_ck && !(t == 0 || 2 * t == L)) ? 2.f : 1.f;
            f[e] = (kk < 2 * K && n < L) ? (part ? -ck : ck) * tw[(part ? L : 0) + (int)(((long)n * t) % L)] : 0.f;
        }
    }
    const Hf2 h = split2_8(f[0], f[1], f[2], f[3], f[4], f[5], f[6], f[7]);
    out[(frag * 2 + 0) * 64 + lane] = h.hi;
    out[(frag * 2 + 1) * 64 + lane] = h.lo;
}
template <int NL, bool MIXH2, class ST = StF32, bool MIXOUT = false, bool EXTLDS = false, bool DFTTAB = false>
__device__ __forceinline__ void spectral_x3_body(const X3Args A, int bidx, int skew_cycles, float* ext_lds = nullptr, int tid_in = 0,
                                                 unsigned long long* tr = nullptr) {
    using F = X3Cfg;
    constexpr int C = F::C, RS = F::RS, LSF = F::LSF;
    constexpr int NLW = NL / F::NW;
    constexpr bool DFTH2 = MIXH2;
    using DftFrag = typename std::conditional<DFTH2, Hf3, Bf3>::type;
    static_assert(NL == 16 || NL == 8, "16 or 8 lines per workgroup");
    __shared__ __attribute__((aligned(16))) float XS_own[EXTLDS ? 4 : NL * F::LSF];
    float* XS = XS_own;
    float* tws;
    if constexpr (EXTLDS) {
        XS = ext_lds;
        tws = ext_lds + NL * F::LSF;
    } else {
        FFNO_DYN_SMEM(smem);
        tws = reinterpret_cast<float*>(smem);
    }

    const float* __restrict__ in = A.in;
    const int R = A.R, L = A.L, K = A.K;
    const LineMap lm = A.lm;
    const float rs_w = (MIXH2 && A.wpk && A.in_amax) ? range_scale(*A.in_amax, 1 + (ceil_log2_int(L) + 1) / 2, 15) : 1.f;
    const float rrs = 1.f / rs_w;
    const float sx_w = (DFTH2 && A.in_amax) ? range_scale(*A.in_amax, 0, 10) : 1.f;
    const float unx_w = DFTH2 ? kHf2Unscale / sx_w : 1.f;
    float omax = 0.f;
    __shared__ float rfold[F::NW];
    __shared__ float lrrs[MIXOUT ? NL : 1];

    const int tidx = EXTLDS ? tid_in : (int)threadIdx.x;
    const int lane = tidx & 63, wave = tidx >> 6;
    const int j = lane & 31, half = lane >> 5;
    const int lw = NLW * wave;
    const int line0 = bidx * NL + lw;
    const bool live0 = line0 < R, live1 = NLW > 1 && line0 + 1 < R;
    const long es = lm.elem_stride;
    const unsigned lo0 = (unsigned)((lm.base(min(line0, R - 1)) + 2 * j) * ST::BYTES);
    const unsigned lo1 = (unsigned)((lm.base(min(line0 + 1, R - 1)) + 2 * j) * ST::BYTES);
    if (skew_cycles > 0) plat::sleep_cycles(skew_cycles);

    {
        const int kk = j, k = kk >> 1, ri = kk & 1;
        const bool rowok = kk < 2 * K;
        const float ck = (A.fwd_ck && !(k == 0 || 2 * k == L)) ? 2.f : 1.f;
        const float amul = rowok ? (ri ? -ck : ck) : 0.f;
        const int tbase = ri ? L : 0;
        const int km = rowok ? k : 0;

        using Raw = typename std::conditional<ST::BF16, unsigned, float2>::type;
        Raw raw[4][8];
        const unsigned esb = (unsigned)(es * ST::BYTES);
        auto load_rows = [&](int chunk, int u, unsigned lo) {
            FFNO_UNROLL
            for (int e = 0; e < 8; ++e) {
                const int n = min(16 * (4 * chunk + u) + 8 * half + e, L - 1);
                raw[u][e] = *reinterpret_cast<const Raw*>(reinterpret_cast<const char*>(in) + (lo + (unsigned)n * esb));
            }
        };
        DftFrag Ff[4];
        const int k8 = (km * 8) % L;
        static_assert(!DFTTAB || DFTH2, "the table holds split-fp16 fragments");
        auto build_F = [&](int chunk) {
            if constexpr (DFTTAB) {
                FFNO_UNROLL
                for (int u = 0; u < 4; ++u) Ff[u] = x3k_load_dft(A.dft, chunk * 4 + u, lane);
                return;
            }
            int idx = (km * (64 * chunk + 8 * half)) % L;
            FFNO_UNROLL
            for (int u = 0; u < 4; ++u) {
                float f[8];
                FFNO_UNROLL
                for (int e = 0; e < 8; ++e) {
                    const int n = 16 * (4 * chunk + u) + 8 * half + e;
                    f[e] = n < L ? amul * tws[tbase + idx] : 0.f;
                    idx += km;
                    if (idx >= L) idx -= L;
                }
                idx += k8;
                if (idx >= L) idx -= L;
                if constexpr (DFTH2)
                    Ff[u] = split2s_8(f[0], f[1], f[2], f[3], f[4], f[5], f[6], f[7]);
                else
                    Ff[u] = split3_8(f[0], f[1], f[2], f[3], f[4], f[5], f[6], f[7]);
            }
        };
        const int nchunks = (L + 63) >> 6;
        if constexpr (DFTTAB) build_F(0);
        FFNO_UNROLL
        for (int u = 0; u < 4; ++u) load_rows(0, u, lo0);
        if constexpr (!DFTTAB) {
            for (int i = tidx; i < 2 * L; i += blockDim.x) tws[i] = A.tw[i];
            __syncthreads();
        }
        if (tr && tidx == 0) tr[3] = plat::realtime();
        if constexpr (!DFTTAB) build_F(0);
        if (tr && tidx == 0) tr[6] = plat::realtime();
        FFNO_UNROLL
        for (int ln = 0; ln < NLW; ++ln) {
            f32x16 acc0 = zero16(), acc1 = zero16();
            float sx = sx_w, unx = unx_w, rs = rs_w;
            if constexpr (MIXOUT && !ST::BF16) {
                if (A.self_range) {
                    float lmx = 0.f;
                    FFNO_UNROLL
                    for (int u = 0; u < 4; ++u) {
                        FFNO_UNROLL
                        for (int e = 0; e < 8; ++e) lmx = fmaxf(lmx, fmaxf(fabsf(raw[u][e].x), fabsf(raw[u][e].y)));
                    }
                    FFNO_UNROLL
                    for (int sh = 32; sh >= 1; sh >>= 1) lmx = fmaxf(lmx, __shfl_xor(lmx, sh));
// ... 2555 lines not shown
```

### fourierflow_amd/engine.py

```python
from __future__ import annotations

import collections
import ctypes
import os
from typing import Dict, List, NamedTuple, Optional, Sequence, Tuple

import numpy as np
import torch

from . import _capi, _lib
from ._corner_chain import CornerChain
from ._engine_core import EngineCore

_p = _lib.ptr

MODES = {"full": 0, "low-pass": 1, "no-fourier": 2}
HEAD_DIM = 128
_SUPPORTED_CH = {(64, 256), (64, 128), (32, 128), (32, 64)}
X3_INTERLEAVE = 3
FF_WGRAD_ROUNDS = 3
FW_GRAD_WGS = 512


def _fmix32(h: int) -> int:
# ... 96 lines not shown
        self.SY = self.SD = None
        self.SY2 = self.SD2 = None
        self.T = self.G1 = None
        self.TS = None
        self.chain = self.scr = None
        self.mask_words = None
        self.rw_kinds = self.RW = None
        self.rw_bwd_clean = False
        self.TL = self.LNS = None
        self.TLF = self.LNSF = None
        self.DT = self.DTF = None
        self.lnpart = None
        self.F = self.YL = None
        self.MASKF = self.DSF = None
        self.GF = self.redl = None
        self.HG = None
        self.DA = self.glpart = None
        self.MASK = None
        self.DS = None
        self.G = self.defer_wgrad = None
        self.lazy_sums = None
        self.nsplit_ff = self.nsplit_ffm = None
        self.ffpart = None
        self.defer_reduce = self.ffparts = None
        self.wg_jobs = self.wg_table = None
        self.red_jobs = self.red_table = None
        self.nsplit_fw = self.fwpart = None
        self.fwpart_multi = self.fwgrad_tab = self.fwgrad_sig = None
        self.nsplit_lift = self.liftpart = None
        self.nsplit_head = self.headpart = None
        self.red = None
        self.MIX = None
        self.stack_sync = None
        self.stack_late = None
        self.stack_checked = False
        self.stack_calls = 0


class FFNOEngine(EngineCore):

    can_return_view = True

    def __init__(self, *, modes, width: int, input_dim: int, n_layers: int, factor: int, share_weight: bool,
                 share_fork: bool = False, ff_weight_norm: bool = False, mode: str = "full", spatial_dims: int = 2,
                 padding: int = 0, output_dim: int = 1, use_fork: bool = False, first_axis_first: bool = False,
                 spectral: str = "factorized", layer_norm: bool = False, n_ff_layers: int = 2, dropout: float = 0.0,
                 in_dropout: float = 0.0):
        if mode not in MODES:
            raise ValueError(f"mode must be one of {list(MODES)}, got {mode!r}")
        if spatial_dims not in (2, 3):
            raise ValueError("spatial_dims must be 2 or 3")
        C, H = width, factor * width
        if (C, H) not in _SUPPORTED_CH:
            raise ValueError(f"(width, factor*width)=({C},{H}) is outside the compiled HIP kernel set {_SUPPORTED_CH}")
        if not (0 < input_dim < 64):
            raise ValueError("input_dim must be in 1..63")
        if not (1 <= output_dim <= 8):
            raise ValueError("output_dim must be in 1..8")
        if n_ff_layers < 2:
            raise NotImplementedError("n_ff_layers = 1 (a single width -> width linear) is not built")
        if not (0.0 <= dropout < 1.0 and 0.0 <= in_dropout < 1.0):
            raise ValueError("dropout / in_dropout must lie in [0, 1)")
        self.n_ff, self.dropout, self.in_dropout = int(n_ff_layers), float(dropout), float(in_dropout)
        self.general_ff = self.n_ff != 2 or self.dropout > 0.0
        self.drop_seed = int(torch.initial_seed()) & 0x7FFFFFFF
        self.layer_norm = bool(layer_norm)
        if spectral not in ("factorized", "plus", "dct"):
            raise ValueError("spectral must be 'factorized', 'plus' or 'dct'")
        if spectral == "dct" and mode != "full":
            raise ValueError("the DCT operators (CNOFactorized*) have no `mode` switch")
        if spectral == "plus" and (spatial_dims != 2 or padding or mode == "low-pass"):
            raise ValueError("the non-factorized (FNOPlus2DBlock) spectral conv is 2-D, unpadded, mode 'full' or 'no-fourier'")
        self.spectral = spectral
        self.nd = spatial_dims
        self.first_axis_first = bool(first_axis_first)
        self.Ks: Tuple[int, ...] = tuple(modes) if isinstance(modes, (tuple, list)) else (int(modes),) * spatial_dims
        if len(self.Ks) != spatial_dims:
            raise ValueError("one mode count per spatial axis")
        self.K = self.Ks[0]
        self.C, self.H, self.Cin, self.L, self.O, self.pad = C, H, input_dim, n_layers, output_dim, padding
        self.mode, self.mode_id = mode, MODES[mode]
        self.share_weight, self.share_fork, self.wnorm = share_weight, share_fork, ff_weight_norm
        self.use_fork = use_fork
        self._plain_layer = not (use_fork or self.layer_norm or self.general_ff)

        self.linears: Dict[str, _Linear] = {}
        shapes: Dict[str, Tuple[int, ...]] = {}

        def add_linear(prefix, rows, cols):
            if prefix in self.linears:
                return
            self.linears[prefix] = _Linear(prefix, rows, cols, ff_weight_norm)
            if ff_weight_norm:
                shapes[prefix + "weight_g"] = (rows, 1)
                shapes[prefix + "weight_v"] = (rows, cols)
            else:
                shapes[prefix + "weight"] = (rows, cols)
            shapes[prefix + "bias"] = (rows,)
            if layer_norm and prefix.endswith(f"_ff.layers.{self.n_ff - 1}.0."):
                shapes[prefix[:-2] + "3.weight"] = (rows,)
                shapes[prefix[:-2] + "3.bias"] = (rows,)

        add_linear("in_proj.", C, input_dim)
        self.ff_prefix: List[str] = []
        self.fc_prefix: List[str] = []
        self.fw_names: List[Tuple[str, ...]] = []
        def add_ff(prefix):
            for k in range(self.n_ff):
                add_linear(prefix + f"layers.{k}.0.", C if k == self.n_ff - 1 else H, C if k == 0 else H)

        if share_fork:
            if use_fork:
                add_ff("forecast_ff.")
            add_ff("backcast_ff.")
        for l in range(n_layers):
            if use_fork:
                fc = "forecast_ff." if share_fork else f"spectral_layers.{l}.forecast_ff."
                self.fc_prefix.append(fc)
                add_ff(fc)
            fp = "backcast_ff." if share_fork else f"spectral_layers.{l}.backcast_ff."
            self.ff_prefix.append(fp)
            add_ff(fp)
            if mode == "full":
                base = "fourier_weight." if share_weight else f"spectral_layers.{l}.fourier_weight."
                names = tuple(base + str(w) for w in range(self.nd))
                self.fw_names.append(names)
                for w, n in enumerate(names):
                    shapes.setdefault(n, (C, C, self.Ks[w], self.Ks[w], 2) if spectral == "plus"
                                      else (C, C, self.Ks[w]) if spectral == "dct" else (C, C, self.Ks[w], 2))
        add_linear("out.0.", HEAD_DIM, C)
        add_linear("out.1.", output_dim, HEAD_DIM)
        self._lay_out(shapes)
        self._fw_sets: List[Tuple[str, ...]] = []
        for names in self.fw_names:
            if names not in self._fw_sets:
                self._fw_sets.append(names)
        self._fw_set_of = [self._fw_sets.index(names) for names in self.fw_names] or [0] * n_layers

        self._reset_state()
        self.use_fused = True
        self.use_x3 = True
        self.ff_wgrad_deferred = True
        self.ff_lazy_sums = "s"
        self.ff_schedule = 0
        self.ff_max_workgroups = 0
        self.x3_min_lines = 1
        self.ff_wgrad_slices = 512 if width == 32 else 256
        self.use_layer_calls = True
        self.infer_self_range = True
        self.infer_stack_any_batch = False
        self.infer_min_lines = None
        self.timer = None
        self.weight_range_check_every = 1
        self._read_environment()

    def _read_environment(self):
        env = os.environ
        self.ff_split = env.get("FFNO_FF_SPLIT", "fp16x2")
        self.x3_mix_split = env.get("FFNO_X3_MIX_SPLIT", "fp16x2")
        self.storage = env.get("FFNO_STORAGE", "fp32")
        self.use_infer_layer = env.get("FFNO_INFER_LAYER", "1") != "0"
        self.use_infer_stack = env.get("FFNO_INFER_STACK", "1") != "0"
        self.ff_defer_max_bytes = int(env.get("FFNO_FF_DEFER_MAX_BYTES", 16 << 30))

    def _reset_state(self):
        self.params: Dict[str, torch.Tensor] = {}
        self.device = None
        self._bind_sig = None
        self._issue_stream = None
        self._training = False
        self._drop_calls = 0
        self._in_drop_seed = 0
        self._last_plan = None
        self._saved = None
        self.dx = None
        self.forecast_list = []
        self.infer_stack_last = False
        self._wr_count = 0
        self._wr_warned = False
        self._reset_device_state()

    def _reset_device_state(self):
        self._ptr_sig = None
        self._prep_sig = None
        self._ws = None
        self._ws_key = None
        self._ws_cache = {}
        self._tw: Dict[int, torch.Tensor] = {}
        self._dft_tabs = {}
        self._desc_dev = None
        self._n_desc = 0
        self._max_rows = 0
        self._fx_flat = None
        self._fx_dev = None
        self._n_fx = 0
        self._fwpack = _lib.CachedTable()
        self._x3pack = _lib.CachedTable()
        self._wr_word = None
        self._wr_late = _DeferredWord(self.device)
        self._wr_table = _lib.CachedTable()

    def _bf16(self) -> bool:
        if self.storage not in ("fp32", "bf16"):
            raise ValueError("storage must be 'fp32' or 'bf16', got %r" % (self.storage,))
        return self.storage == "bf16"

    def _st(self) -> int:
        return 1 if self._bf16() else 0

    def _conc(self) -> bool:
        return bool(self._ffx() and not self.use_fork
                    and self.mode != "no-fourier" and self.spectral == "factorized")

    @staticmethod
    def _schedule(fused, views):
        n = len(fused)
        fz = [w for w in range(n) if fused[w]]
        sg = [w for w in range(n) if not fused[w]]
        pair = None
        if len(fz) >= 2:
            pair = (fz[-2], fz[-1])
            if (views[pair[0]].K > 16) != (views[pair[1]].K > 16):
                pair = None
        elif len(sg) >= 2:
            a, b = sg[-2], sg[-1]
            rt = lambda v: (2 * v.K + 31) // 32
            if rt(views[a]) == rt(views[b]) <= 4:
                pair = (a, b)
        if pair is None:
            return list(range(n)), None
        return [w for w in range(n) if w not in pair], pair

    def _pair(self, name, ws, v0, v1, src, dst0, dst1, resid0, save0, save1, planes0, planes1, fwd: bool, st, acc0: int = 0,
              fused: bool = True, x3: bool = False, rin=None, rout=None, resid1=None):
        lib = _lib.get_lib()
        ck_f, ck_i, conj = (0, 1, 0) if fwd else (1, 0, 1)
        if not fused:
            sv0 = save0 if save0 is not None else ws.SD
            sv1 = save1 if save1 is not None else ws.SD2
            ba = self._branch(v0, src, dst0, resid0, sv0, planes0, acc0, False, fwd, None, rout if x3 else None)
            bb = self._branch(v1, src, dst1, resid1, sv1, planes1, 0, False, fwd, None, rout if x3 else None)
            fn = lib.ffno_spectral_x3_staged_pair if x3 else lib.ffno_spectral_staged_pair
            self._k("spectral_staged_pair" + ("" if fwd else "(adj)"), fn, ctypes.byref(ba),
                    ctypes.byref(bb), _p(ws.SY), _p(ws.SY2), self.C, ck_f, ck_i, conj, st)
            if not x3:
                self._fold(dst0, rout, st)
                self._fold(dst1, rout, st)
            return
        ba = self._branch(v0, src, dst0, resid0, save0, planes0, acc0, x3, fwd, rin, rout)
        bb = self._branch(v1, src, dst1, resid1, save1, planes1, 0, x3, fwd, rin, rout)
        if x3:
            self._k(name, lib.ffno_spectral_x3_pair, ctypes.byref(ba), ctypes.byref(bb), self.C, ck_f, ck_i, conj,
                    X3_INTERLEAVE, st)
            return
        self._k(name, lib.ffno_spectral_fused_pair, ctypes.byref(ba), ctypes.byref(bb), self.C, ck_f, ck_i, conj, st)

    def _branch(self, v, src, dst, resid, save, planes, acc, x3=False, fwd=True, rin=None, rout=None):
        fmt = int(v.x3fmt) if (x3 and planes is not None and self._x3_h2()) else 0
        dft = self._dft_frags(v.L, v.K, fwd) if fmt else None
        return _capi.FusedBranch(_p(src), _p(dst), resid, _p(save), _p(planes), _p(self._twiddle(v.L)), v.Bv, v.Mv, v.Nv, v.K,
                                 v.a01, acc, fmt, 0, rin if fmt else None, rout, self._st(), 0, _p(dft))

    def _dft_frags(self, L: int, K: int, fwd: bool):
        key = (L, K, bool(fwd))
        tab = self._dft_tabs.get(key)
        if tab is None:
            lib = _lib.get_lib()
            nb = int(lib.ffno_spectral_x3_dft_frags_bytes(L, K)) if self.C in (32, 64) else 0
            if nb:
                tab = torch.empty(nb // 4, dtype=torch.int32, device=self.device)
                ck_f, ck_i = (0, 1) if fwd else (1, 0)
                self._k("dft_frags", lib.ffno_spectral_x3_dft_frags, _p(self._twiddle(L)), L, K, ck_f, ck_i, _p(tab),
                        _lib.current_stream(self.device))
            else:
                tab = False
            self._dft_tabs[key] = tab
        return tab if tab is not False else None

    def _ranged(self) -> bool:
        return bool((self._ffx() and self._h2()) or (self.use_x3 and self.spectral == "factorized" and self._x3_h2()))

    def _rw(self, ws, kind: str, l: int):
        return ctypes.c_void_p(ws.RW.data_ptr() + 4 * (ws.rw_kinds[kind] * (self.L + 1) + l)) if self._ranged() else None

    def _fw_words(self, ws, l0: int):
        if not (self._x3_h2() and self._ranged() and self.spectral == "factorized" and self.use_x3):
            return None, None
        return self._rw(ws, "x", l0), self._rw(ws, "d", l0)

    def _fold(self, t, word, st):
        if word is None or t is None:
            return
        self._k("amax", _lib.get_lib().ffno_amax, _p(t), t.numel(), word, st)

    def _x3_h2(self) -> bool:
        if self.x3_mix_split not in ("fp16x2", "bf16x3"):
            raise ValueError("x3_mix_split must be 'fp16x2' or 'bf16x3', got %r" % (self.x3_mix_split,))
        return self.x3_mix_split == "fp16x2"

    def _ffx(self) -> bool:
        return not self.general_ff

    def _h2(self) -> bool:
        if self.ff_split not in ("fp16x2", "bf16x3"):
            raise ValueError("ff_split must be 'fp16x2' or 'bf16x3', got %r" % (self.ff_split,))
        return self.ff_split == "fp16x2"

    def _ffs_fwd2(self, s, s2, s_sum, resid, l0, b0, b1, out, mask, P, st, rin=None, rout=None):
        lib = _lib.get_lib()
        fn = lib.ffno_ffh_fwd2 if self._h2() else lib.ffno_ffx_fwd2
        o = _capi.FfOpts(rin, rout, int(self.ff_max_workgroups), int(self.ff_schedule), self._st())
        self._k("ff_fwd", fn, _p(s), _p(s2), _p(s_sum), _p(resid), _p(l0.fx[0]), _p(b0), _p(l0.fx[1]), _p(b1), _p(out), _p(mask),
                P, self.C, self.H, ctypes.byref(o), st)

    def _ffs_bwd2(self, g, g2, g_sum, mask, l0, ds, P, st, rin=None, rout=None):
        lib = _lib.get_lib()
        fn = lib.ffno_ffh_bwd_data2 if self._h2() else lib.ffno_ffx_bwd_data2
        o = _capi.FfOpts(rin, rout, int(self.ff_max_workgroups), int(self.ff_schedule), self._st())
        self._k("ff_bwd_data", fn, _p(g), _p(g2), _p(g_sum), _p(mask), _p(l0.fx[2]), _p(l0.fx[3]), _p(ds),
                P, self.C, self.H, ctypes.byref(o), st)

    def _ffs_wgrad(self, s, g, l0, b0, part, P, nsplit, st, rs=None, rg=None):
        lib = _lib.get_lib()
        args = (_p(s), _p(g), _p(l0.fx[0]), _p(b0), _p(l0.fx[2]), _p(part), P, self.C, self.H, nsplit)
        if self._h2():
            self._k("ff_bwd_weights_partial", lib.ffno_ffh_bwd_weights_partial, *args, rs, rg, self._st(), st)
        else:
            self._k("ff_bwd_weights_partial", lib.ffno_ffx_bwd_weights_partial, *args, st)

    def bind(self, params: Dict[str, torch.Tensor]):
        sig = tuple(params[n].data_ptr() for n in self.param_names) if all(n in params for n in self.param_names) else None
        if sig is not None and self.params and sig == self._bind_sig:
            self.params = {n: params[n] for n in self.param_names}
            return
        dev = self._validate(params)
        self.params = {n: params[n] for n in self.param_names}
        self._bind_sig = sig
        if dev != self.device:
            self.device = dev
            self._alloc_param_buffers()
        self._ptr_sig = None

    def _alloc_param_buffers(self):
        dev = self.device
        f32 = dict(dtype=torch.float32, device=dev)
        self.gflat = torch.zeros(self.n_params, **f32)
        n_eff = sum(l.rows * l.cols for l in self.linears.values()) if self.wnorm else 0
        self.weff_flat = torch.empty(max(n_eff, 1), **f32)
        self.gweff_flat = torch.zeros(max(n_eff, 1), **f32)
        self.fold = torch.zeros(self.O * (self.C + 1), **f32)
        plane_modes = [2 * self.K * self.K] if self.spectral == "plus" else list(self.Ks)
        self.planes = [[(torch.empty(2 * K * self.C * self.C, **f32), torch.empty(2 * K * self.C * self.C, **f32))
                        for K in plane_modes] for _ in range(max(len(self._fw_sets), 1))]
        lib = _lib.get_lib()
        self.xplanes = [[None] * len(plane_modes) for _ in self.planes]
        if self.spectral == "factorized" and self.mode == "full":
            for si in range(len(self.planes)):
                for w, K in enumerate(plane_modes):
                    nb = int(lib.ffno_spectral_x3_pack_bytes(self.C, K))
                    if nb:
                        self.xplanes[si][w] = tuple(torch.empty(nb // 4, dtype=torch.int32, device=dev) for _ in range(2))
        self._reset_device_state()

    def _refresh_pointers(self):
        sig = tuple(self.params[n].data_ptr() for n in self.param_names) + (self.ff_split,)
        if sig == self._ptr_sig:
            return
        self._ptr_sig = sig
        off = 0
        descs = []
        for lin in self.linears.values():
            n = lin.rows * lin.cols
            if lin.wnorm:
                lin.weff = self.weff_flat[off:off + n].view(lin.rows, lin.cols)
                lin.gweff = self.gweff_flat[off:off + n].view(lin.rows, lin.cols)
                off += n
                g, v = self.params[lin.prefix + "weight_g"], self.params[lin.prefix + "weight_v"]
                descs.append(_capi.WnDesc(g.data_ptr(), v.data_ptr(), lin.weff.data_ptr(), lin.gweff.data_ptr(),
                                          self.grad_view(lin.prefix + "weight_g").data_ptr(),
                                          self.grad_view(lin.prefix + "weight_v").data_ptr(), lin.rows, lin.cols))
            else:
                lin.weff = self.params[lin.prefix + "weight"]
                lin.gweff = self.grad_view(lin.prefix + "weight")
        self._n_desc = len(descs)
        lib = _lib.get_lib()
        blocks = list(dict.fromkeys(self.ff_prefix + self.fc_prefix))
        if self._ffx():
            words = int((lib.ffno_ffh_pack_bytes if self._h2() else lib.ffno_ffx_pack_bytes)(self.C, self.H)) // 4
            if self._fx_flat is None or self._fx_flat.numel() != 4 * words * len(blocks):
                self._fx_flat = torch.empty(4 * words * len(blocks), dtype=torch.int32, device=self.device)
            fdescs = []
            for bi, pfx in enumerate(blocks):
                l0, l1 = self.linears[pfx + "layers.0.0."], self.linears[pfx + "layers.1.0."]
                pk = [self._fx_flat[(4 * bi + q) * words:(4 * bi + q + 1) * words] for q in range(4)]
                l0.fx = pk
                l1.fx = pk
                C_, H_ = self.C, self.H
                for (src, sh, sc, ty), dst in zip(((l0.weff, C_, 1, 1), (l1.weff, 1, H_, 2), (l1.weff, 1, H_, 1),
                                                   (l0.weff, C_, 1, 2)), pk):
                    fdescs.append(_capi.FxPackDesc(src.data_ptr(), dst.data_ptr(), sh, sc, ty, 0))
            self._n_fx = len(fdescs)
            self._fx_dev = _lib.device_table(_capi.FxPackDesc, fdescs, self.device)
        self._max_rows = max([l.rows for l in self.linears.values()])
        self._desc_dev = _lib.device_table(_capi.WnDesc, descs, self.device) if descs else None

    def _twiddle(self, L: int) -> torch.Tensor:
        tw = self._tw.get(L)
        if tw is None:
            tw = self._tw[L] = _lib.twiddle(L, self.device)
        return tw

    def _views(self, B: int, Sp: Sequence[int]) -> List[_View]:
        C = self.C
        if self.spectral == "plus":
            return [CornerChain(B, Sp, (self.K, self.K), C, lambda *a: self._k(*a), self.device)]
        if self.nd == 2:
            M, N = Sp
            if self.first_axis_first:
                return [_View(B, M, N, 1, self.Ks[0], C), _View(B, M, N, 0, self.Ks[1], C)]
            return [_View(B, M, N, 0, self.Ks[0], C), _View(B, M, N, 1, self.Ks[1], C)]
        X, Y, Z = Sp
        return [_View(B, X, Y * Z, 1, self.Ks[0], C),
                _View(B * X, Y, Z, 1, self.Ks[1], C),
                _View(B, X * Y, Z, 0, self.Ks[2], C)]

    def _workspace_key(self, B: int, S: Tuple[int, ...], save: bool):
        return (B, tuple(S), bool(save), self._ffx(), self._conc(), self.general_ff, self._bf16(),
                (self._h2(), self._ranged(), bool(self.ff_wgrad_deferred), str(self.ff_lazy_sums), int(self.ff_wgrad_slices),
                 bool(self.use_x3), bool(self.use_fused), int(self.ff_defer_max_bytes)))

    def _workspace(self, B: int, S: Tuple[int, ...], save: bool):
        key = self._workspace_key(B, S, save)
        if self._ws_key == key:
            return self._ws
        cache = self._ws_cache
        if key in cache:
            self._ws, self._ws_key = cache[key], key
            return self._ws
        lib = _lib.get_lib()
        dev, C, H, L, O = self.device, self.C, self.H, self.L, self.O
        Sp = tuple(s + self.pad for s in S)
        P_in = B * int(np.prod(S))
        P = B * int(np.prod(Sp))
        f32 = dict(dtype=torch.float32, device=dev)
        act = dict(dtype=torch.bfloat16 if self._bf16() else torch.float32, device=dev)
        ns = L if save else 1
        ws = _Workspace()
        ws.P, ws.P_in, ws.Sp = P, P_in, Sp
        ws.views = self._views(B, Sp)
        if self.pad:
            s3 = (1,) * (3 - self.nd) + tuple(S)
            p3 = (1,) * (3 - self.nd) + tuple(Sp)
            ws.padmap = _capi.PadMap((ctypes.c_int32 * 3)(*s3), (ctypes.c_int32 * 3)(*p3))
            ws.pm = ctypes.byref(ws.padmap)
        ws.X = torch.empty(P, C, **act)
        ws.Blast = torch.empty(P, C, **act)
        ws.Y = torch.empty(P_in * O, **f32)
        ws.S = torch.empty(ns, P, C, **act)
        nv = len(ws.views)
        ws.SXall = [torch.empty(ns, v.spec, **f32) for v in ws.views]
        ws.SY = torch.empty(max(v.spec for v in ws.views), **f32)
        ws.SD = torch.empty(max(v.spec for v in ws.views), **f32)
        if self._conc():
            ws.SD2 = torch.empty_like(ws.SD)
            ws.SY2 = torch.empty_like(ws.SY)
            ws.T = torch.empty(P, C, **act)
            if save:
                ws.G1 = torch.empty(P, C, **act)
        if self.spectral == "plus":
            ws.chain = ws.views[0]
            ws.scr = ws.chain.scratch(lambda n: torch.empty(n, **f32))
        ws.mask_words = int(lib.ffno_ff_mask_words(P, H))
        ws.rw_kinds = {"x": 0, "s": 1, "g": 2, "d": 3, "t": 4, "f": 5}
        ws.RW = torch.zeros(len(ws.rw_kinds) * (L + 1), dtype=torch.int32, device=dev)
        if self.layer_norm:
            ws.TL = torch.empty(ns, P, C, **f32)
            ws.LNS = torch.empty(ns, P, 2, **f32)
            if self.use_fork:
                ws.TLF = torch.empty(ns, P, C, **f32)
                ws.LNSF = torch.empty(ns, P, 2, **f32)
            if save:
                ws.DT = torch.empty(P, C, **f32)
                ws.lnpart = torch.empty(2 * C * int(lib.ffno_layernorm_nsplit(P)), **f32)
                if self.use_fork:
                    ws.DTF = torch.empty(P, C, **f32)
        if self.use_fork:
            ws.F = torch.empty(ns, P, C, **f32)
            ws.YL = torch.empty(L, P_in * O, **f32)
        if self.general_ff:
            kinds = ["backcast"] + (["forecast"] if self.use_fork else [])
            ws.HG = {kind: [[torch.empty(P, H, **f32) for _ in range(self.n_ff - 1)] for _ in range(ns)] for kind in kinds}
            if save:
                ws.DA = [torch.empty(P, H, **f32) for _ in range(2)]
                ws.glpart = torch.empty(int(lib.ffno_glin_wgrad_partial_floats(P, H, H)), **f32)
        if save and self.use_fork:
            ws.MASKF = torch.zeros(ns, ws.mask_words, dtype=torch.int32, device=dev)
            ws.DSF = torch.empty(P, C, **f32)
            ws.GF = torch.empty(P, C, **f32)
            ws.redl = torch.empty(O * (C + 1), **f32)
        if save:
            ws.MASK = torch.zeros(ns, ws.mask_words, dtype=torch.int32, device=dev)
            ws.DS = torch.empty(P, C, **act)
            ws.defer_wgrad = bool(self.ff_wgrad_deferred and self._ffx() and self._h2() and self._ranged() and not self.share_fork
                                  and self._plain_layer and (C, H) in ((64, 256), (32, 128)) and self.mode != "no-fourier")
            if 2 * L * P * C * (2 if self._bf16() else 4) > int(self.ff_defer_max_bytes):
                ws.defer_wgrad = False
            ws.G = [torch.empty(P, C, **act) for _ in range(L + 1 if ws.defer_wgrad else 2)]
            if self.ff_lazy_sums not in ("s", "0", ""):
                raise ValueError("ff_lazy_sums must be 's' or '0', got %r" % (self.ff_lazy_sums,))
            ws.lazy_sums = "s" if (ws.defer_wgrad and self.ff_lazy_sums == "s" and self._conc() and (C, H) == (64, 256)) else ""
            if ws.lazy_sums:
                ws.TS = [torch.empty(P, C, **act) for _ in range(L)]
            ws.SDall = [torch.empty(L, v.spec, **f32) for v in ws.views] if self.mode == "full" else None
            ws.nsplit_ff = max(1, min(int(self.ff_wgrad_slices), (P + 127) // 128))
            cus = torch.cuda.get_device_properties(dev).multi_processor_count if dev.type == "cuda" else 256
            ws.nsplit_ffm = max(1, min(ws.nsplit_ff, (FF_WGRAD_ROUNDS * (3 if H <= 128 else 1) * cus) // L))
            ws.wg_table = _lib.CachedTable()
            ws.ffpart = torch.empty(int(lib.ffno_ff_wgrad_partial_floats(C, H, ws.nsplit_ff)), **f32)
            ws.defer_reduce = bool(self._ffx() and not self.share_fork)
            if ws.defer_reduce:
                njobs = L * (2 if self.use_fork else 1)
                ws.ffparts = torch.empty(njobs, ws.ffpart.numel(), **f32)
                ws.red_table = _lib.CachedTable()
            ws.nsplit_fw = [max(1, min(max(1, FW_GRAD_WGS // v.K), (L * v.R + 63) // 64)) for v in ws.views]
            if self.spectral == "plus":
                ws.nsplit_fw = [1]
            ws.fwpart = [[torch.empty(ws.nsplit_fw[w] * 2 * ws.views[w].modes * C * C, **f32) for w in range(nv)]
                         for _ in range(max(len(self._fw_sets), 1))]
            ws.fwpart_multi, ws.fwgrad_tab, ws.fwgrad_sig = [None] * nv, [None] * nv, [None] * nv
            ws.nsplit_lift = max(1, min(1024, (P_in + 127) // 128))
            ws.liftpart = torch.empty(ws.nsplit_lift * C * (self.Cin + 1), **f32)
            ws.nsplit_head = max(1, min(256, (P_in + 255) // 256))
            ws.headpart = torch.empty(ws.nsplit_head * O * (C + 1), **f32)
            ws.red = torch.empty(O * (C + 1), **f32)
        self._ws, self._ws_key = ws, key
        cache[key] = ws
        while len(cache) > 4:
            cache.pop(next(iter(cache)))
        return ws

    def _saved_pass(self, what: str = "backward()") -> _Saved:
        sv = self._saved
        if sv is None:
            raise RuntimeError(f"{what} needs a preceding forward(save_for_backward=True)")
        if self._workspace_key(sv.B, sv.S, True) != sv.ws_key:
            raise RuntimeError("an engine attribute that shapes the workspace (ff_split / x3_mix_split / ff_wgrad_deferred / "
                               "ff_lazy_sums / ff_wgrad_slices / use_x3 / use_fused / storage) changed between forward() and "
                               "backward(): run the forward pass again")
        return sv

    def weights_changed(self):
        self._prep_sig = None

    def _prepare_weights(self, st, x3fmt: List[int]):
        lib = _lib.get_lib()
        self._refresh_pointers()
        try:
            sig = (tuple((t.data_ptr(), t._version) for t in self.params.values()), self.ff_split, self.x3_mix_split,
                   tuple(x3fmt), self.use_x3, getattr(st, "value", st))
        except RuntimeError:
            sig = None
        if sig is not None and sig == self._prep_sig:
            return
        self._prep_sig = sig
        if self._desc_dev is not None:
            self._k("weightnorm_fwd", lib.ffno_weightnorm_fwd, _p(self._desc_dev), self._n_desc, self._max_rows, st)
        if self._ffx() and self._n_fx:
            self._k("ffx_pack", lib.ffno_ffh_pack if self._h2() else lib.ffno_ffx_pack, _p(self._fx_dev), self._n_fx, self.C,
                    self.H, st)
        for i, names in enumerate(self._fw_sets if self.spectral == "plus" else []):
            self._k("fw2d_pack", lib.ffno_fw2d_pack, _p(self.params[names[0]]), _p(self.params[names[1]]),
                    _p(self.planes[i][0][0]), _p(self.planes[i][0][1]), self.C, self.K, st)
        if self.spectral != "plus" and self._fw_sets:
            rows = tuple((self.params[n].data_ptr(), self.planes[i][w][0].data_ptr(), self.planes[i][w][1].data_ptr(), self.Ks[w],
                          int(self.spectral == "dct")) for i, names in enumerate(self._fw_sets) for w, n in enumerate(names))
            self._k("fw_pack", lib.ffno_fw_pack_batched, _p(self._fwpack.get(_capi.FwPackDesc, rows, self.device)), len(rows),
                    self.C, max(self.Ks), st)
            if self.use_x3 and any(x is not None for row in self.xplanes for x in row):
                rows = tuple((self.planes[i][w][d].data_ptr(), xp[d].data_ptr(), self.Ks[w], x3fmt[w])
                             for i, row in enumerate(self.xplanes) for w, xp in enumerate(row) if xp is not None for d in range(2))
                self._k("fw_pack_x3", lib.ffno_spectral_x3_pack, _p(self._x3pack.get(_capi.X3PackDesc, rows, self.device)),
                        len(rows), self.C, max(r[2] for r in rows), st)
        o0, o1 = self.linears["out.0."], self.linears["out.1."]
        self._k("head_fold", lib.ffno_head_fold, _p(o0.weff), _p(self.params["out.0.bias"]), _p(o1.weff),
                _p(self.params["out.1.bias"]), _p(self.fold), self.C, HEAD_DIM, self.O, st)
        self._check_weight_range(st, x3fmt)

    def _check_weight_range(self, st, x3fmt: List[int]):
        every = int(self.weight_range_check_every)
        fp16_ff, fp16_mix = self._ffx() and self._h2(), any(x3fmt)
        if every <= 0 or not (fp16_ff or fp16_mix):
            return
        host = self._wr_late.take()
        if host is not None:
            wmax = float(host.view(torch.float32)[0])
            if 0.0 < wmax < 2.0 ** -9 and not self._wr_warned:
                import warnings
                self._wr_warned = True
                warnings.warn(f"every weight that goes into the split-fp16 packs is below {wmax:.3g}: the packs keep a fixed "
                              f"absolute error of 2^-36 there, i.e. relative accuracy degrades as the weights shrink "
                              f"(1e-6 at 2e-5); ff_split / x3_mix_split = 'bf16x3' is exact at any magnitude", RuntimeWarning)
            if not wmax < 65504.0:
                raise FloatingPointError(
                    f"a weight of magnitude {wmax:.3g} does not fit the split-fp16 packs (|W| < 65504): set "
                    f"engine.ff_split = engine.x3_mix_split = 'bf16x3' (FFNO_FF_SPLIT / FFNO_X3_MIX_SPLIT) -- any fp32 range")
        self._wr_count += 1
        if (self._wr_count - 1) % every or self._wr_late.pending:
            return
        lib = _lib.get_lib()
        if self._wr_word is None:
            self._wr_word = torch.zeros(1, dtype=torch.int32, device=self.device)
        self._wr_word.zero_()
        srcs = []
        if fp16_ff:
            if self.wnorm:
                srcs.append(self.weff_flat)
            else:
                srcs += [self.params[p + "weight"] for p in self.linears if "_ff." in p and p + "weight" in self.params]
        if fp16_mix:
            srcs += [self.params[n] for names in self._fw_sets for n in names]
        rows = tuple((t.data_ptr(), t.numel()) for t in srcs)
        self._k("amax", lib.ffno_amax_batched, _p(self._wr_table.get(_capi.AmaxDesc, rows, self.device)), len(rows),
                max(n for _, n in rows), _p(self._wr_word), st)
        self._wr_late.post(self._wr_word)

    def _ff_weights(self, l, prefixes=None):
        fp = (prefixes or self.ff_prefix)[l]
        l0, l1 = self.linears[fp + "layers.0.0."], self.linears[fp + "layers.1.0."]
        return l0, l1, self.params[fp + "layers.0.0.bias"], self.params[fp + "layers.1.0.bias"]

    def _ff_bwd_weights(self, ws, s, s2, g, l0, l1, b0, gb0, gb1, accumulate, P, st, rs=None, rg=None):
        lib = _lib.get_lib()
        if ws.defer_reduce:
            assert not accumulate
            part = ws.ffparts[len(ws.red_jobs)]
            if ws.wg_jobs is not None:
                ws.wg_jobs.append((s.data_ptr(), g.data_ptr(), l0.fx[0].data_ptr(), b0.data_ptr(), l0.fx[2].data_ptr(),
                                   part.data_ptr(), rs.value, rg.value, s2.data_ptr() if s2 is not None else 0, 0))
            else:
                self._ffs_wgrad(s, g, l0, b0, part, P, ws.nsplit_ff, st, rs, rg)
            ws.red_jobs.append((part.data_ptr(), l0.gweff.data_ptr(), l1.gweff.data_ptr(), gb0.data_ptr(), gb1.data_ptr()))
        else:
            self._ffs_wgrad(s, g, l0, b0, ws.ffpart, P, ws.nsplit_ff, st, rs, rg)
            self._k("ff_bwd_weights_reduce", lib.ffno_ffx_bwd_weights_reduce, _p(ws.ffpart), _p(l0.gweff), _p(l1.gweff),
                    _p(gb0), _p(gb1), self.C, self.H, ws.nsplit_ff, accumulate, st)

    def _drop_args(self, layer: int, kind: str, k: int):
        if not (self.dropout > 0.0 and self._training):
            return 0.0, 0
        return self.dropout, _site_seed(self.drop_seed, self._drop_calls, layer, k + 1, int(kind == "forecast"))

    def _ffg_fwd(self, ws, prefix, kind, layer, sv, s, resid, out, P, st, rout=None):
        lib = _lib.get_lib()
        a = s
        for k in range(self.n_ff):
            last = k == self.n_ff - 1
            lin = self.linears[prefix + f"layers.{k}.0."]
            dst = out if last else ws.HG[kind][sv][k]
            p, seed = self._drop_args(layer, kind, k)
            self._k("ff_fwd", lib.ffno_glin_fwd, _p(a), _p(lin.weff), _p(self.params[prefix + f"layers.{k}.0.bias"]),
                    _p(resid) if last else None, _p(dst), P, lin.cols, lin.rows, int(not last), p, seed, st)
            a = dst
        self._fold(out, rout, st)

    def _ffg_bwd(self, ws, prefix, kind, layer, s, g, ds, accumulate, P, st, rout=None):
        lib = _lib.get_lib()
        gv = self.grad_view
        g_cur = g
        for k in reversed(range(self.n_ff)):
            last = k == self.n_ff - 1
            lin = self.linears[prefix + f"layers.{k}.0."]
            x_in = s if k == 0 else ws.HG[kind][layer][k - 1]
            y = None if last else ws.HG[kind][layer][k]
            p, seed = self._drop_args(layer, kind, k)
            self._k("ff_bwd_weights_partial", lib.ffno_glin_bwd_weights, _p(g_cur), _p(y), _p(x_in), _p(ws.glpart), _p(lin.gweff),
                    _p(gv(prefix + f"layers.{k}.0.bias")), P, lin.cols, lin.rows, p, seed, int(accumulate), st)
            dx = ds if k == 0 else ws.DA[k & 1]
            self._k("ff_bwd_data", lib.ffno_glin_bwd_data, _p(g_cur), _p(y), _p(lin.weff), _p(dx), P, lin.cols, lin.rows, p, seed,
                    0, st)
            g_cur = dx
        self._fold(ds, rout, st)

    def _planes_for(self, si, w, adj: int, x3: bool):
        if self.mode != "full":
            return None
        return self.xplanes[si][w][adj] if x3 else self.planes[si][w][adj]

    def _can_fuse(self, views):
        lib = _lib.get_lib()
        if self.spectral == "plus":
            return [False]
        if self.spectral == "dct":
            return [False] * len(views)
        return [bool(self.use_fused and self.mode != "no-fourier"
                     and (lib.ffno_spectral_fused_supported(self.C, v.K, v.L) or self._x3_ok(w, v, views)))
                for w, v in enumerate(views)]

    def _x3_ok(self, w, v, views) -> bool:
        lib = _lib.get_lib()
        if not (self.use_x3 and self.spectral == "factorized" and self.mode != "no-fourier"):
            return False
        P4 = 4 * self.C * max(u.Bv * u.Mv * u.Nv for u in views)
        return bool(v.R >= self.x3_min_lines and P4 < 2 ** 32 and lib.ffno_spectral_x3_supported(self.C, v.K, v.L)
                    and (self.mode != "full" or self.xplanes[0][w] is not None))

    def _infer_ok(self, ws, conc, pair, singles, x3pair, fused) -> bool:
        if not (self.use_infer_layer and conc and pair is not None and not singles and x3pair and fused[pair[0]]):
            return False
        if not (self.nd == 2 and self.mode == "full" and self.spectral == "factorized" and self._ffx() and self._h2() and self._x3_h2()
                and not self._bf16() and self._plain_layer and (self.C, self.H) == (64, 256)):
            return False
        va, vb = ws.views[pair[0]], ws.views[pair[1]]
        if {va.a01, vb.a01} != {0, 1} or (va.Bv, va.Mv, va.Nv) != (vb.Bv, vb.Mv, vb.Nv):
            return False
        if any(v.x3fmt != 1 for v in (va, vb)):
            return False
        row, col = (va, vb) if va.a01 == 0 else (vb, va)
        lib = _lib.get_lib()
        if not lib.ffno_layer_infer_supported(va.Bv, va.Mv, va.Nv, self.C, self.H, row.K, col.K):
            return False
        if self._dft_frags(row.L, row.K, True) is None or self._dft_frags(col.L, col.K, True) is None:
            return False
        cus = torch.cuda.get_device_properties(self.device).multi_processor_count if self.device.type == "cuda" else 256
        need = self.infer_min_lines if self.infer_min_lines is not None else 4 * cus + 1
        return va.R + vb.R >= need

    def _stack_pays(self, B: int) -> bool:
        if self.infer_stack_any_batch:
            return True
        if B <= 16:
            return True
        tail = B % 32
        return tail == 0 or tail > 16

    def _run_infer_stack(self, ws, pair, st) -> bool:
        lib = _lib.get_lib()
        C, H, L = self.C, self.H, self.L
        a, b = pair
        va, vb = ws.views[a], ws.views[b]
        row, col = (va, vb) if va.a01 == 0 else (vb, va)
        if int(lib.ffno_infer_stack_supported(va.Bv, va.Mv, va.Nv, C, H, row.K, col.K, L)) != 2:
            return False
        if not self._stack_pays(va.Bv):
            return False
        if ws.stack_sync is None:
            n = int(lib.ffno_infer_stack_sync_words(va.Bv))
            ws.stack_sync = torch.zeros(n, dtype=torch.int32, device=self.device)
            ws.stack_late = _DeferredWord(self.device)
        host = ws.stack_late.take()
        if host is not None and int(host[0]) != 0:
            self.use_infer_stack = False
            raise RuntimeError("ffno_infer_stack: the previous forward pass reported a workgroup without a group or a barrier "
                               "time-out (error word %d): its result was invalid; the persistent launch is now off for this "
                               "engine (engine.use_infer_stack)" % int(host[0]))
        ba = self._branch(va, ws.X, ws.MIX[0], None, None, None, 0, True, True, None, None)
        bb = self._branch(vb, ws.X, ws.MIX[1], None, None, None, 0, True, True, None, None)
        for br, v in ((ba, va), (bb, vb)):
            br.planes_format, br.flags, br.in_amax = 1, _capi.BRANCH_SELF_RANGE, None
            br.dft_frags = _p(self._dft_frags(v.L, v.K, True))
        rows = []
        for l in range(L):
            si = self._fw_set_of[l]
            l0, l1, b0, b1 = self._ff_weights(l)
            rows.append(_capi.InferStackLayer(_p(self._planes_for(si, a, 0, True)), _p(self._planes_for(si, b, 0, True)), _p(l0.fx[0]),
                                              _p(b0), _p(l0.fx[1]), _p(b1)))
        arr = (_capi.InferStackLayer * L)(*rows)
        d = _capi.InferStackDesc(ba, bb, ctypes.cast(arr, ctypes.c_void_p), L, C, H, 0, _p(ws.Blast), _p(ws.stack_sync))
        rc = self._timed("infer_stack", lib.ffno_infer_stack, ctypes.byref(d), st)
        if rc != 0:
            self.use_infer_stack = False
            return False
        err_word = ws.stack_sync[-1:]
        ws.stack_calls += 1
        if not ws.stack_checked:
            ws.stack_checked = True
            if int(err_word.cpu()[0]) != 0:
                self.use_infer_stack = False
# ... 538 lines not shown
```

### include/ffno.h

```cpp
#ifndef FFNO_H_
#define FFNO_H_

#include <stddef.h>
#include <stdint.h>

#ifdef __cplusplus
extern "C" {
#endif

#define FFNO_OK 0
#define FFNO_EINVAL (-1)
#define FFNO_EUNSUPPORTED (-2)
#define FFNO_EMODES (-3)

#define FFNO_STORE_F32 0
#define FFNO_STORE_BF16 1

#define FFNO_MODE_FULL 0
#define FFNO_MODE_LOWPASS 1
#define FFNO_MODE_NOFOURIER 2

const char* ffno_build_target(void);
#define FFNO_ABI_VERSION 13
int ffno_abi_version(void);

int ffno_amax(const float* x, size_t n, uint32_t* word, void* stream);
typedef struct ffno_amax_desc {
    const float* x;
    size_t n;
} ffno_amax_desc;
int ffno_amax_batched(const ffno_amax_desc* descs_dev, int n, size_t max_n, uint32_t* word, void* stream);

int ffno_twiddle_fill_host(float* tw_host, int L);

int ffno_dft_fwd(const float* x, float* spec, const float* tw, int B, int M, int N, int C, int K,
                 int axis, int scale_ck, void* stream);

int ffno_fw_pack(const float* w, float* wp, float* wpt, int C, int K, void* stream);
typedef struct ffno_fwpack_desc {
    const float* w;
    float* wp;
    float* wpt;
    int32_t K, real;
} ffno_fwpack_desc;
int ffno_fw_pack_batched(const ffno_fwpack_desc* descs, int n, int C, int max_K, void* stream);

int ffno_mode_mix(const float* spec_in, const float* planes, float* spec_out, int R, int C, int K,
                  int conj_transpose, void* stream);

int ffno_dft_inv(const float* spec, float* out, const float* resid, const float* tw, int B, int M,
                 int N, int C, int K, int axis, int apply_ck, int accumulate, void* stream);

int ffno_fw_grad_partial(const float* spec_x, const float* spec_dy, float* partial, int R, int C,
                         int K, int nsplit, int beta, int nlayers, size_t layer_stride_x,
                         size_t layer_stride_dy, void* stream);
int ffno_fw_grad_reduce(const float* partial, float* gw, int C, int K, int nsplit, int accumulate,
                        void* stream);
int ffno_fw_grad_partial_h2(const float* spec_x, const float* spec_dy, float* partial, int R, int C, int K, int nsplit, int beta,
                            int nlayers, size_t layer_stride_x, size_t layer_stride_dy, const uint32_t* x_words,
                            const uint32_t* d_words, int L, void* stream);
int ffno_fw_grad_partial_multi_h2(const float* spec_x, const float* spec_dy, float* partial, int R, int C, int K, int nsplit, int n,
                                  size_t stride_x, size_t stride_dy, size_t stride_p, const uint32_t* x_words,
                                  const uint32_t* d_words, int L, void* stream);
int ffno_fw_grad_partial_multi(const float* spec_x, const float* spec_dy, float* partial, int R, int C, int K,
                               int nsplit, int n, size_t stride_x, size_t stride_dy, size_t stride_p,
                               void* stream);
int ffno_fw_grad_reduce_multi(const float* partial, float* const* gws, int n, int C, int K, int nsplit,
                              size_t stride_p, int accumulate, int real, void* stream);

int ffno_spectral_fused_supported(int C, int K, int L);
int ffno_spectral_fused(const float* in, float* out, const float* resid, float* spec_save,
                        const float* planes, const float* tw, int B, int M, int N, int C, int K,
                        int axis, int scale_ck_fwd, int apply_ck_inv, int conj_transpose,
                        int accumulate, uint32_t* out_amax , void* stream);
typedef struct ffno_fused_branch {
    const float* in;
    float* out;
    const float* resid;
    float* spec_save;
    const float* planes;
    const float* tw;
    int32_t B, M, N;
    int32_t K, axis, accumulate;
    int32_t planes_format;
    int32_t tile_lines;
    const uint32_t* in_amax;
    uint32_t* out_amax;
    int32_t storage;
    int32_t flags;
    const void* dft_frags;
} ffno_fused_branch;
#define FFNO_PLANES_BF16X3 0
#define FFNO_PLANES_FP16X2 1
#define FFNO_PLANES_FP16X2_M16 2
#define FFNO_BRANCH_SELF_RANGE 1
#define FFNO_X3_TILE_LATENCY 1
#define FFNO_X3_TILE_LATENCY_SPLIT 2
size_t ffno_spectral_x3_dft_frags_bytes(int L, int K);
int ffno_spectral_x3_dft_frags(const float* tw, int L, int K, int scale_ck_fwd, int apply_ck_inv, void* frags, void* stream);
int ffno_spectral_fused_pair(const ffno_fused_branch* a, const ffno_fused_branch* b, int C, int scale_ck_fwd,
                             int apply_ck_inv, int conj_transpose, void* stream);
typedef struct ffno_x3pack_desc {
    const float* planes;
    void* dst;
    int32_t K;
    int32_t format;
} ffno_x3pack_desc;
int ffno_spectral_x3_supported(int C, int K, int L);
size_t ffno_spectral_x3_pack_bytes(int C, int K);
int ffno_spectral_x3_pack(const ffno_x3pack_desc* descs_dev, int n, int C, int max_K, void* stream);
int ffno_spectral_x3(const ffno_fused_branch* br, int C, int scale_ck_fwd, int apply_ck_inv, int conj_transpose,
                     void* stream);
int ffno_spectral_x3_pair(const ffno_fused_branch* a, const ffno_fused_branch* b, int C, int scale_ck_fwd,
                          int apply_ck_inv, int conj_transpose, int interleave, void* stream);
int ffno_spectral_x3_staged_supported(int C, int K, int L);
int ffno_spectral_x3_staged_pair(const ffno_fused_branch* a, const ffno_fused_branch* b, float* mix_a, float* mix_b, int C,
                                 int scale_ck_fwd, int apply_ck_inv, int conj_transpose, void* stream);

#define FFNO_BRANCH_FUSED 0
#define FFNO_BRANCH_X3 1
#define FFNO_FF_BF16X3 0
#define FFNO_FF_FP16X2 1
typedef struct ffno_layer_fwd_desc {
    ffno_fused_branch a, b;
    int32_t branch_kernel, interleave;
    const void* pk1;
    const float* b1;
    const void* pk2;
    const float* b2;
    float* s_sum;
    const float* resid;
    float* out;
    void* mask;
    int32_t P, C, H;
    int32_t ff_kernel;
    int32_t ff_schedule, ff_max_workgroups, pad0_, pad1_;
    uint32_t* out_amax;
} ffno_layer_fwd_desc;
typedef struct ffno_layer_bwd_desc {
    ffno_fused_branch a, b;
    int32_t branch_kernel, interleave;
    const float* g;
    const float* g2;
    float* g_sum;
    const void* mask;
    const void* pk1b;
    const void* pk2b;
    float* ds;
    const float* s;
    const void* pk1;
    const float* b1;
    float* partial;
    int32_t nsplit, P, C, H;
    int32_t ff_kernel, ff_schedule, ff_max_workgroups, pad_;
    const uint32_t* g_amax;
    const uint32_t* s_amax;
    uint32_t* ds_amax;
} ffno_layer_bwd_desc;
int ffno_layer_fwd(const ffno_layer_fwd_desc* d, void* stream);
int ffno_layer_bwd(const ffno_layer_bwd_desc* d, void* stream);

typedef struct ffno_layer_infer_desc {
    ffno_fused_branch a, b;
    int32_t interleave, pad_;
    const void* pk1;
    const float* b1;
    const void* pk2;
    const float* b2;
    const float* resid;
    float* out;
    int32_t C, H;
    uint32_t* out_amax;
} ffno_layer_infer_desc;
size_t ffno_infer_mix_bytes(int C, int K, int lines);
int ffno_layer_infer_supported(int B, int M, int N, int C, int H, int K_rows, int K_cols);
int ffno_spectral_x3_mix_pair(const ffno_fused_branch* a, const ffno_fused_branch* b, int C, int interleave, void* stream);
int ffno_infer_ff(const ffno_fused_branch* a, const ffno_fused_branch* b, const void* pk1, const float* b1, const void* pk2,
                  const float* b2, const float* resid, float* out, int C, int H, uint32_t* out_amax, void* stream);
int ffno_infer_sum(const ffno_fused_branch* a, const ffno_fused_branch* b, float* out, int C, uint32_t* out_amax, void* stream);
int ffno_layer_infer(const ffno_layer_infer_desc* d, void* stream);

typedef struct ffno_infer_stack_layer {
    const void* planes_a;
    const void* planes_b;
    const void* pk1;
    const float* b1;
    const void* pk2;
    const float* b2;
} ffno_infer_stack_layer;
typedef struct ffno_infer_stack_desc {
    ffno_fused_branch a, b;
    const ffno_infer_stack_layer* layers;
    int32_t n_layers, C, H, mode;
    float* last_out;
    uint32_t* sync;
} ffno_infer_stack_desc;
int ffno_infer_stack_supported(int B, int M, int N, int C, int H, int K_rows, int K_cols, int n_layers);
size_t ffno_infer_stack_sync_words(int B);
size_t ffno_infer_stack_trace_words(int n_layers);
int ffno_infer_stack(const ffno_infer_stack_desc* d, void* stream);

int ffno_spectral_staged_pair(const ffno_fused_branch* a, const ffno_fused_branch* b, float* mix_a,
                              float* mix_b, int C, int scale_ck_fwd, int apply_ck_inv,
                              int conj_transpose, void* stream);

size_t ffno_spectral2d_ws_floats(int B, int M, int N, int C, int K);
#define FFNO_SPECTRAL2D_STAGES 0
#define FFNO_SPECTRAL2D_FUSED_X3 1
int ffno_spectral2d_path(int B, int M, int N, int C, int K);
int ffno_spectral2d_weights_version(const float* ws, unsigned long long version);
int ffno_spectral2d_fwd(const float* x, const float* w_y, const float* w_x, float* out, float* ws,
                        const float* tw_n, const float* tw_m, int B, int M, int N, int C, int K,
                        int mode, void* stream);
int ffno_spectral2d_bwd(const float* x, const float* w_y, const float* w_x, const float* gy,
                        float* gx, float* gw_y, float* gw_x, float* ws, const float* tw_n,
                        const float* tw_m, int B, int M, int N, int C, int K, int mode,
                        int accumulate_gx, int accumulate_gw, void* stream);

size_t ffno_ff_mask_words(int P, int H);
int ffno_ff_fwd(const float* s, const float* resid, const float* W1, const float* b1,
                const float* W2, const float* b2, float* out, float* h, uint32_t* mask, int P,
                int C, int H, void* stream);
int ffno_ff_bwd_data(const float* db, const uint32_t* mask, const float* W1t, const float* W2t,
                     float* dh, float* ds, int P, int C, int H, void* stream);
size_t ffno_ff_wgrad_partial_floats(int C, int H, int nsplit);
int ffno_ff_bwd_weights_partial(const float* s, const float* db, const float* h, const float* dh,
                                float* partial, int P, int C, int H, int nsplit, void* stream);
int ffno_ff_bwd_weights_reduce(const float* partial, float* dW1, float* dW2, float* db1, float* db2,
                               int C, int H, int nsplit, int accumulate, void* stream);

typedef struct ffno_fxpack_desc {
    const float* src;
    void* dst;
    int32_t sh, sc;
    int32_t type;
    int32_t pad_;
} ffno_fxpack_desc;
int ffno_ffx_supported(int C, int H);
typedef struct ffno_ff_opts {
    const uint32_t* in_amax;
    uint32_t* out_amax;
    int32_t max_workgroups;
    int32_t schedule;
    int32_t storage;
} ffno_ff_opts;
#define FFNO_FF_SCHED_IN_PHASE 1
#define FFNO_FF_SCHED_WAVE_TILES 2
#define FFNO_FF_SCHED_ROLE_SPLIT 3
size_t ffno_ffx_pack_bytes(int C, int H);
int ffno_ffx_pack(const ffno_fxpack_desc* descs_dev, int n, int C, int H, void* stream);
int ffno_ffx_fwd(const float* s, const float* resid, const void* pk1, const float* b1, const void* pk2,
                 const float* b2, float* out, void* mask, int P, int C, int H, void* stream);
int ffno_ffx_mask_unpack(const void* mask, uint8_t* active, int P, int C, int H, void* stream);
int ffno_ffx_fwd2(const float* s, const float* s2, float* s_sum, const float* resid, const void* pk1, const float* b1,
                  const void* pk2, const float* b2, float* out, void* mask, int P, int C, int H, const ffno_ff_opts* opts,
                  void* stream);
int ffno_ffx_bwd_data2(const float* db, const float* db2, float* db_sum, const void* mask, const void* pk1b,
                       const void* pk2b, float* ds, int P, int C, int H, const ffno_ff_opts* opts, void* stream);
int ffno_ffx_bwd_data(const float* db, const void* mask, const void* pk1b, const void* pk2b, float* ds,
                      int P, int C, int H, void* stream);
int ffno_ffx_bwd_weights_partial(const float* s, const float* db, const void* pk1, const float* b1,
                                 const void* pk1b, float* partial, int P, int C, int H, int nsplit,
                                 void* stream);
int ffno_ffx_bwd_weights_reduce(const float* partial, float* dW1, float* dW2, float* db1, float* db2,
                                int C, int H, int nsplit, int accumulate, void* stream);
typedef struct ffno_fxred_desc {
    const float* partial;
    float* dW1;
    float* dW2;
    float* db1;
    float* db2;
} ffno_fxred_desc;
int ffno_ffx_bwd_weights_reduce_batched(const ffno_fxred_desc* descs_dev, int n, int C, int H, int nsplit,
                                        void* stream);

size_t ffno_ffh_pack_bytes(int C, int H);
int ffno_ffh_pack(const ffno_fxpack_desc* descs_dev, int n, int C, int H, void* stream);
int ffno_ffh_fwd2(const float* s, const float* s2, float* s_sum, const float* resid, const void* pk1, const float* b1,
                  const void* pk2, const float* b2, float* out, void* mask, int P, int C, int H, const ffno_ff_opts* opts,
                  void* stream);
int ffno_ffh_bwd_data2(const float* db, const float* db2, float* db_sum, const void* mask, const void* pk1b,
                       const void* pk2b, float* ds, int P, int C, int H, const ffno_ff_opts* opts, void* stream);
int ffno_ffh_bwd_weights_partial(const float* s, const float* db, const void* pk1, const float* b1, const void* pk1b,
                                 float* partial, int P, int C, int H, int nsplit, const uint32_t* s_amax,
                                 const uint32_t* db_amax, int storage , void* stream);
typedef struct ffno_ffwg_desc {
    const void* s;
    const void* g;
    const void* pk1;
    const float* b1;
    const void* pk1b;
    float* partial;
    const uint32_t* s_amax;
    const uint32_t* g_amax;
    const void* s2;
    const void* g2;
} ffno_ffwg_desc;
int ffno_ffh_bwd_weights_partial_multi(const ffno_ffwg_desc* descs, int n, int P, int C, int H, int nsplit, int storage,
                                       int two_addends , void* stream);

int ffno_lds_tr16_probe(const uint16_t* image, int n16, const int32_t* byte_off, uint16_t* out, void* stream);

int ffno_layernorm_fwd(const float* t, const float* gamma, const float* beta, const float* resid, float* out, float* stats,
                       long P, int C, float eps, void* stream);
int ffno_layernorm_nsplit(long P);
int ffno_layernorm_bwd(const float* t, const float* stats, const float* gamma, const float* g, const float* g2, float* g_sum,
                       float* dt, float* partial, float* dgamma, float* dbeta, long P, int C, int accumulate, void* stream);

typedef struct ffno_wn_desc {
    const float* g;
    const float* v;
    float* w;
    const float* dw;
    float* dg;
    float* dv;
    int32_t rows;
    int32_t cols;
} ffno_wn_desc;
int ffno_weightnorm_fwd(const ffno_wn_desc* descs_dev, int n, int max_rows, void* stream);
int ffno_weightnorm_bwd(const ffno_wn_desc* descs_dev, int n, int max_rows, void* stream);

typedef struct ffno_tr_desc {
    const float* src;
    float* dst;
    int32_t rows;
    int32_t cols;
} ffno_tr_desc;
int ffno_transpose_batched(const ffno_tr_desc* descs_dev, int n, int max_rows, int max_cols, void* stream);

typedef struct ffno_padmap {
    int32_t size[3];
    int32_t padded[3];
} ffno_padmap;

int ffno_lift_fwd(const float* x, const float* W, const float* b, float* out, int P, int Cin, int C,
                  const ffno_padmap* pad, uint32_t* out_amax , void* stream);
int ffno_lift_bwd(const float* x, const float* gout, float* partial, float* dW, float* db, int P,
                  int Cin, int C, int nsplit, int accumulate, const ffno_padmap* pad, void* stream);
int ffno_lift_fwd_bf16(const float* x, const float* W, const float* b, uint16_t* out, int P, int Cin, int C,
                       const ffno_padmap* pad, uint32_t* out_amax, void* stream);
int ffno_lift_bwd2(const float* x, const float* gout, const float* gout2, float* partial, float* dW, float* db, int P,
                   int Cin, int C, int nsplit, int accumulate, const ffno_padmap* pad, void* stream);
int ffno_lift_bwd_bf16(const float* x, const uint16_t* gout, float* partial, float* dW, float* db, int P,
                       int Cin, int C, int nsplit, int accumulate, const ffno_padmap* pad, void* stream);
int ffno_lift_bwd_data(const float* gout, const float* W, float* dx, int P, int Cin, int C,
                       const ffno_padmap* pad, void* stream);

int ffno_head_fold(const float* Wa, const float* ca, const float* Wb, const float* cb, float* fold,
                   int C, int D, int O, void* stream);
int ffno_head_fwd(const float* b, const float* fold, float* y, int P, int C, int O, int accumulate,
                  const ffno_padmap* pad, void* stream);
int ffno_head_bwd(const float* b, const float* gy, const float* fold, float* gb, float* partial,
                  float* red, int P, int C, int O, int nsplit, const ffno_padmap* pad,
                  uint32_t* gb_amax , void* stream);
int ffno_head_fwd_bf16(const uint16_t* b, const float* fold, float* y, int P, int C, int O, int accumulate,
                       const ffno_padmap* pad, void* stream);
int ffno_head_bwd_bf16(const uint16_t* b, const float* gy, const float* fold, uint16_t* gb, float* partial,
                       float* red, int P, int C, int O, int nsplit, const ffno_padmap* pad, uint32_t* gb_amax, void* stream);
int ffno_head_param_grads(const float* red, const float* Wa, const float* ca, const float* Wb,
                          float* dWa, float* dca, float* dWb, float* dcb, int C, int D, int O,
                          int accumulate, void* stream);

int ffno_cdft_rows(const float* in, float* out, int B, int M, int C, int K, int inverse, void* stream);
int ffno_fw2d_pack(const float* w0, const float* w1, float* wp, float* wpt, int C, int K, void* stream);
int ffno_fw2d_grad_reduce(const float* partial, float* gw0, float* gw1, int C, int K, int nsplit,
                          int accumulate, void* stream);
int ffno_cdft_rows2(const float* in, float* out, int B, int M, int C, int Kx, int Ky, int inverse,
                    void* stream);
int ffno_fw2d_pack2(const float* w0, const float* w1, float* wp, float* wpt, int C, int Kx, int Ky,
                    void* stream);
int ffno_fw2d_grad_reduce2(const float* partial, float* gw0, float* gw1, int C, int Kx, int Ky, int nsplit,
                           int accumulate, void* stream);
size_t ffno_cdft_rows_ws_floats(int B, int C, int Kx, int Ky);
int ffno_cdft_rows_mfma(const float* in, float* out, float* ws, const float* tw, int B, int M, int C,
                        int Kx, int Ky, int inverse, void* stream);

int ffno_fw3d_pack(const float* w1, const float* w2, const float* w3, const float* w4, float* wp, float* wpt,
                   int C, int K1, int K2, int K3, void* stream);
int ffno_fw3d_grad_reduce(const float* partial, float* g1, float* g2, float* g3, float* g4, int C, int K1,
                          int K2, int K3, int nsplit, int accumulate, void* stream);

int ffno_dct_branch(const float* in, float* out, const float* resid, float* spec, float* mix,
                    const float* planes, const float* tw2, int B, int M, int N, int C, int K, int axis,
                    int conj_transpose, int accumulate, void* stream);
int ffno_fw_pack_real(const float* w, float* wp, float* wpt, int C, int K, void* stream);
int ffno_mode_mix_real(const float* spec_in, const float* planes, float* spec_out, int R, int C, int K,
                       void* stream);
int ffno_fw_grad_reduce_real(const float* partial, float* gw, int C, int K, int nsplit, int accumulate,
                             void* stream);

size_t ffno_velocity_ws_floats(int B, int X, int Y);
int ffno_velocity_features(const float* vorticity, float* out, float* ws, int B, int X, int Y,
                           float len_x, float len_y, void* stream);

size_t ffno_lploss_tmp_floats(int B, int n_per_sample);
int ffno_lploss_fwd_bwd(const float* pred, const float* target, float* loss_out, float* gpred,
                        float* tmp, int B, int n_per_sample, float gscale, const float* affine,
                        void* stream);

typedef struct ffno_markov_extra {
    const float* force;
    const float* mu;
    int32_t use_position;
    int32_t pad_;
} ffno_markov_extra;
int ffno_markov_features(const float* x, float* state, float* derived, const float* noise, float* out,
                         float* partial, int B, int M, int N, int Cx, float low, float high,
                         float noise_std, float eps, int accumulate, int normalize,
                         const ffno_markov_extra* extra, void* stream);

size_t ffno_markov_traj_ws_floats(int B, int M, int N, int n_steps);
int ffno_markov_traj_step(const float* out, const float* affine, const float* prev, const float* data, float* im,
                          float* preds, float* sums, int B, int M, int N, int T, int n_steps, int t, void* stream);
int ffno_markov_traj_metrics(const float* sums, float* metrics, int B, int M, int N, int n_steps, float threshold,
                             void* stream);

size_t ffno_vorticity_coarsen_ws_floats(int B, int m, int n_steps);
int ffno_vorticity_coarsen_step(const float* vel, const float* corr, float* preds2, float* sums, int B, int X, int Y, int m,
                                int Tc, int n_steps, int t, float len_x, float len_y, void* stream);
int ffno_markov_corr_metrics(const float* sums, float* metrics, int B, int m, int n_steps, float threshold, void* stream);

int ffno_prediction_export_step(const float* vel, float* vort, float* vx, float* vy, int B, int X, int Y, int m, int n_steps,
                                int t, float len_x, float len_y, void* stream);
int ffno_energy_spectrum(const float* u_h, const float* v_h, float* E, int n_img, int m, void* stream);

typedef struct ffno_markov_advance_desc {
    const float* affine;
    const float* prev;
    float* traj;
    float* feats;
    const float* derived;
    const float* force;
    const float* mu;
    int64_t force_stride;
    int32_t L, col, D;
    int32_t use_position, normalize;
    float low, high;
    int32_t pad_;
} ffno_markov_advance_desc;
int ffno_markov_advance(const float* out, float* field, const ffno_markov_advance_desc* desc, int B, int M, int N,
                        void* stream);

int ffno_markov_pairs(const float* data, const int32_t* ids, float* x, float* y, float* dx, float* dy, const float* f,
                      float* f_out, const float* mu, float* mu_out, int n, int M, int N, int T, int t0, int k, int P, int B,
                      void* stream);
int ffno_markov_pairs_tf(const float* data, const int32_t* ids, float* x, float* y, float* dx, float* dy, const float* f, int Tf,
                         float* f_out, const float* mu, float* mu_out, int n, int M, int N, int T, int t0, int k, int P, int B,
                         void* stream);

#define FFNO_GATHER_MAX_FIELDS 8
typedef struct ffno_gather_field {
    const float* src;
    float* dst;
    int64_t src_sample, src_offset, src_q, src_r;
    int64_t dst_sample, dst_offset, dst_q, dst_r;
    int32_t Q, R;
} ffno_gather_field;
int ffno_sample_gather(const ffno_gather_field* fields, int n_fields, const int32_t* ids, int n, int B, void* stream);

int ffno_adamw_flat(float* p, const float* g, float* m, float* v, size_t n, float lr, float beta1,
                    float beta2, float eps, float weight_decay, int step, float grad_scale,
                    void* stream);
int ffno_adam_flat(float* p, const float* g, float* m, float* v, size_t n, float lr, float beta1,
                   float beta2, float eps, float weight_decay, int step, float grad_scale, void* stream);

#define FFNO_ACT_NONE 0
#define FFNO_ACT_RELU 1
#define FFNO_ACT_GELU 2
int ffno_plin_supported(int Cin, int Cout);
int ffno_plin_fwd(const float* x, int ldx, const float* W, const float* b, const float* add, float* out,
                  int ldo, const float* res, float* out2, float* pre_out, long P, int Cin, int Cout,
                  int act_mode, void* stream);
int ffno_plin_bwd_data(const float* g, int ldg, const float* act, const float* W, float* dx, int ldx,
                       float* dpre_out, long P, int Cin, int Cout, int accumulate, int act_mode,
// ... 100 lines not shown
```

Measured before the change: 182.8.

## Fuse per-step weight preparation into a single multi-section prepare kernel

Adds a step_prepare kernel that runs weight-norm, FF fragment packing, Fourier weight packing, x3 packing, head fold and amax range checks in one launch, split by block-index sections. Weight-normalised FF weights are packed straight from g and v, with row scales computed in LDS, so the separate weight-norm write and reread is skipped. The x3 planes are built directly from parameters. The aim is to remove several small kernel launches and intermediate memory traffic per training step, at the cost of a large multi-role kernel and some recomputed row norms across blocks.

```diff
diff --git a/fourierflow_amd/_capi.py b/fourierflow_amd/_capi.py
--- a/fourierflow_amd/_capi.py
+++ b/fourierflow_amd/_capi.py
@@ -2,7 +2,7 @@
 
 import ctypes as C
 
-ABI_VERSION = 13
+ABI_VERSION = 14
 BRANCH_SELF_RANGE = 1
 
 P = C.c_void_p
@@ -101,6 +101,23 @@
 
 class X3PackDesc(C.Structure):
     _fields_ = [("planes", P), ("dst", P), ("K", C.c_int32), ("format", C.c_int32)]
+
+
+class FxPrepDesc(C.Structure):
+    _fields_ = [("src", P), ("g", P), ("dst", P), ("sh", C.c_int32), ("sc", C.c_int32), ("type", C.c_int32), ("cols", C.c_int32)]
+
+
+class X3PrepDesc(C.Structure):
+    _fields_ = [("w", P), ("dst", P), ("K", C.c_int32), ("format", C.c_int32), ("transposed", C.c_int32), ("pad_", C.c_int32)]
+
+
+class PrepPlan(C.Structure):
+    _fields_ = [("wn", P), ("fx", P), ("fw", P), ("x3", P), ("amax", P), ("word", P), ("amax_max_n", C.c_size_t),
+                ("head_wa", P), ("head_ga", P), ("head_ca", P), ("head_wb", P), ("head_gb", P), ("head_cb", P), ("fold", P),
+                ("n_wn", C.c_int32), ("wn_max_rows", C.c_int32), ("wn_amax", C.c_int32), ("n_fx", C.c_int32),
+                ("ff_split", C.c_int32), ("n_fw", C.c_int32), ("fw_max_K", C.c_int32), ("n_x3", C.c_int32),
+                ("x3_max_K", C.c_int32), ("n_amax", C.c_int32), ("C", C.c_int32), ("H", C.c_int32), ("D", C.c_int32),
+                ("O", C.c_int32)]
 
 
 class TrDesc(C.Structure):
@@ -202,6 +219,8 @@
     "ffno_layernorm_bwd": (I, [P, P, P, P, P, P, P, P, P, P, L, I, I, P]),
     "ffno_weightnorm_fwd": (I, [P, I, I, P]),
     "ffno_weightnorm_bwd": (I, [P, I, I, P]),
+    "ffno_step_prepare_supported": (I, [I, I]),
+    "ffno_step_prepare": (I, [P, P]),
     "ffno_transpose_batched": (I, [P, I, I, I, P]),
     "ffno_lift_fwd": (I, [P, P, P, P, I, I, I, P, P, P]),
     "ffno_lift_bwd": (I, [P, P, P, P, P, I, I, I, I, I, P, P]),
diff --git a/fourierflow_amd/csrc/ffno_prep.h b/fourierflow_amd/csrc/ffno_prep.h
--- /dev/null
+++ b/fourierflow_amd/csrc/ffno_prep.h
@@ -0,0 +1,165 @@
+#pragma once
+#include "ffno_device.h"
+
+namespace ffno {
+
+__device__ __forceinline__ float wn_row_scale(const float* __restrict__ g, const float* __restrict__ v, int row, int cols,
+                                              int lane) {
+    const float* vr = v + (long)row * cols;
+    float ss = 0.f;
+    for (int c = lane; c < cols; c += 64) ss += vr[c] * vr[c];
+    ss = wave_sum(ss);
+    return g[row] / sqrtf(ss);
+}
+
+template <int NPL, int U>
+__device__ __forceinline__ void wn_row_scales(const float* __restrict__ g, const float* __restrict__ v, int r0, int stride,
+                                              int rend, int cols, int lane, float (&x)[U][NPL], float (&sc)[U]) {
+    float gg[U];
+    FFNO_UNROLL
+    for (int u = 0; u < U; ++u) {
+        const int row = r0 + u * stride;
+        gg[u] = row < rend ? g[row] : 0.f;
+        FFNO_UNROLL
+        for (int q = 0; q < NPL; ++q) {
+            const int c = lane + 64 * q;
+            x[u][q] = (row < rend && c < cols) ? v[(long)row * cols + c] : 0.f;
+        }
+    }
+    FFNO_UNROLL
+    for (int u = 0; u < U; ++u) {
+        float ss = 0.f;
+        FFNO_UNROLL
+        for (int q = 0; q < NPL; ++q) {
+            ss += x[u][q] * x[u][q];
+            FFNO_PIN(ss);
+        }
+        ss = wave_sum(ss);
+        sc[u] = r0 + u * stride < rend ? gg[u] / sqrtf(ss) : 0.f;
+    }
+}
+template <int NPL, int U>
+__device__ __forceinline__ void wn_scales_to_lds_n(const float* __restrict__ g, const float* __restrict__ v, int row0, int nrows,
+                                                   int cols, float* scale, int wave, int lane) {
+    for (int r = row0 + wave; r < row0 + nrows; r += 4 * U) {
+        float x[U][NPL], sc[U];
+        wn_row_scales<NPL, U>(g, v, r, 4, row0 + nrows, cols, lane, x, sc);
+        FFNO_UNROLL
+        for (int u = 0; u < U; ++u)
+            if (lane == 0 && r + 4 * u < row0 + nrows) scale[r + 4 * u - row0] = sc[u];
+    }
+}
+template <int U>
+__device__ __forceinline__ void wn_scales_to_lds(const float* __restrict__ g, const float* __restrict__ v, int row0, int nrows,
+                                                 int cols, float* scale, int wave, int lane) {
+    if (cols <= 64)
+        wn_scales_to_lds_n<1, U>(g, v, row0, nrows, cols, scale, wave, lane);
+    else if (cols <= 128)
+        wn_scales_to_lds_n<2, (U > 32 ? 32 : U)>(g, v, row0, nrows, cols, scale, wave, lane);
+    else if (cols <= 256)
+        wn_scales_to_lds_n<4, (U > 16 ? 16 : U)>(g, v, row0, nrows, cols, scale, wave, lane);
+    else
+        for (int r = wave; r < nrows; r += 4) {
+            const float sc = wn_row_scale(g, v, row0 + r, cols, lane);
+            if (lane == 0) scale[r] = sc;
+        }
+}
+
+struct StoredWeights {
+    const float* w;
+    __device__ __forceinline__ float operator()(long off) const { return w[off]; }
+};
+struct NormedWeights {
+    const float* v;
+    const float* scale;
+    int cols, row0;
+    __device__ __forceinline__ float operator()(long off) const {
+        float x = v[off] * scale[(int)((unsigned)off / (unsigned)cols) - row0];
+        FFNO_PIN(x);
+        return x;
+    }
+};
+
+template <class S, class Src>
+__device__ __forceinline__ void fx_pack_body(const Src& src, u32x4* dst, int sh, int sc, int type, int C, int H, int t) {
+    const int KS = C / 16, CTO = C / 32, NW = H / 32;
+    const int nfrag = type == 1 ? NW * KS : NW * CTO * 2;
+    if (t >= nfrag * 64) return;
+    const int frag = t >> 6, lane = t & 63, j = lane & 31, half = lane >> 5;
+    float v[8];
+    if (type == 1) {
+        const int w = frag / KS, st = frag % KS;
+        for (int e = 0; e < 8; ++e) v[e] = src((long)(32 * w + j) * sh + (long)(16 * st + 8 * half + e) * sc);
+    } else {
+        const int s2 = frag & 1, mt = (frag >> 1) % CTO, w = (frag >> 1) / CTO;
+        for (int e = 0; e < 8; ++e)
+            v[e] = src((long)(32 * w + (e & 3) + 8 * (2 * s2 + (e >> 2)) + 4 * half) * sh + (long)(32 * mt + j) * sc);
+    }
+    const typename S::Frag f = S::split8(v[0], v[1], v[2], v[3], v[4], v[5], v[6], v[7]);
+    FFNO_UNROLL
+    for (int p = 0; p < S::NP; ++p) dst[(frag * S::NP + p) * 64 + lane] = S::plane(f, p);
+}
+
+__device__ __forceinline__ void fw_pack_body(const float* __restrict__ w, float* __restrict__ wp, float* __restrict__ wpt, int C,
+                                             int K, int real, int bx, int nb) {
+    const long total = (long)C * C * K * 2;
+    for (long e = (long)bx * blockDim.x + threadIdx.x; e < total; e += (long)nb * blockDim.x) {
+        const int o = e % C;
+        const int i = (e / C) % C;
+        const int ri = (e / ((long)C * C)) % 2;
+        const int k = e / ((long)C * C * 2);
+        const float v = real ? (ri ? 0.f : w[((long)i * C + o) * K + k]) : w[(((long)i * C + o) * K + k) * 2 + ri];
+        wp[e] = v;
+        wpt[(((long)k * 2 + ri) * C + o) * C + i] = v;
+    }
+}
+
+struct StoredPlanes {
+    const float* planes;
+    __device__ __forceinline__ float operator()(int k, int p, int i, int o) const {
+        return planes[((long)(k * 2 + p) * 64 + i) * 64 + o];
+    }
+};
+struct ParamPlanes {
+    const float* w;
+    int K, transposed;
+    __device__ __forceinline__ float operator()(int k, int p, int i, int o) const {
+        return transposed ? w[(((long)o * 64 + i) * K + k) * 2 + p] : w[(((long)i * 64 + o) * K + k) * 2 + p];
+    }
+};
+
+template <class Src>
+__device__ __forceinline__ void x3_pack_body(const Src& src, u32x4* dst, int K, int format, int t) {
+    const int nfrag = K * 16;
+    if (t >= nfrag * 64) return;
+    const int frag = t >> 6, lane = t & 63, j = lane & 31, half = lane >> 5;
+    const int pt = frag & 3, st = (frag >> 2) & 3, k = frag >> 4;
+    const int p = pt >> 1, tt = pt & 1;
+    if (format == 2) {
+        const int fm = frag & 15, s2 = fm & 1, t16 = (fm >> 1) & 3, pp = fm >> 3;
+        const int j16 = lane & 15, g = lane >> 4;
+        float w[8];
+        FFNO_UNROLL
+        for (int e = 0; e < 8; ++e) w[e] = src(k, pp, 32 * s2 + 8 * g + e, 4 * j16 + t16);
+        const Hf2 f = split2_8(w[0], w[1], w[2], w[3], w[4], w[5], w[6], w[7]);
+        dst[(frag * 2 + 0) * 64 + lane] = f.hi;
+        dst[(frag * 2 + 1) * 64 + lane] = f.lo;
+        return;
+    }
+    float v[8];
+    FFNO_UNROLL
+    for (int e = 0; e < 8; ++e) v[e] = src(k, p, 16 * st + 8 * half + e, 2 * j + tt);
+    if (format == 1) {
+        const Hf2 f = split2_8(v[0], v[1], v[2], v[3], v[4], v[5], v[6], v[7]);
+        const int fo = (k * 4 + pt) * 4 + st;
+        dst[(fo * 2 + 0) * 64 + lane] = f.hi;
+        dst[(fo * 2 + 1) * 64 + lane] = f.lo;
+        return;
+    }
+    const Bf3 f = split3_8(v[0], v[1], v[2], v[3], v[4], v[5], v[6], v[7]);
+    dst[(frag * 3 + 0) * 64 + lane] = f.hi;
+    dst[(frag * 3 + 1) * 64 + lane] = f.mid;
+    dst[(frag * 3 + 2) * 64 + lane] = f.lo;
+}
+
+}
diff --git a/fourierflow_amd/csrc/ffx.hip b/fourierflow_amd/csrc/ffx.hip
--- a/fourierflow_amd/csrc/ffx.hip
+++ b/fourierflow_amd/csrc/ffx.hip
@@ -1,6 +1,7 @@
 #include <algorithm>
 
 #include "ffno_device.h"
+#include "ffno_prep.h"
 #include "ffno.h"
 
 #include <string.h>
@@ -37,23 +38,7 @@
 template <class S>
 __global__ __launch_bounds__(256) void ffx_pack_kernel(const FxPackDesc* __restrict__ descs, int C, int H) {
     const FxPackDesc d = descs[blockIdx.y];
-    const int KS = C / 16, CTO = C / 32, NW = H / 32;
-    const int nfrag = d.type == 1 ? NW * KS : NW * CTO * 2;
-    const int t = blockIdx.x * blockDim.x + threadIdx.x;
-    if (t >= nfrag * 64) return;
-    const int frag = t >> 6, lane = t & 63, j = lane & 31, half = lane >> 5;
-    float v[8];
-    if (d.type == 1) {
-        const int w = frag / KS, st = frag % KS;
-        for (int e = 0; e < 8; ++e) v[e] = d.src[(long)(32 * w + j) * d.sh + (long)(16 * st + 8 * half + e) * d.sc];
-    } else {
-        const int s2 = frag & 1, mt = (frag >> 1) % CTO, w = (frag >> 1) / CTO;
-        for (int e = 0; e < 8; ++e)
-            v[e] = d.src[(long)(32 * w + (e & 3) + 8 * (2 * s2 + (e >> 2)) + 4 * half) * d.sh + (long)(32 * mt + j) * d.sc];
-    }
-    const typename S::Frag f = S::split8(v[0], v[1], v[2], v[3], v[4], v[5], v[6], v[7]);
-    FFNO_UNROLL
-    for (int p = 0; p < S::NP; ++p) d.dst[(frag * S::NP + p) * 64 + lane] = S::plane(f, p);
+    fx_pack_body<S>(StoredWeights{d.src}, d.dst, d.sh, d.sc, d.type, C, H, (int)(blockIdx.x * blockDim.x + threadIdx.x));
 }
 
 __device__ __forceinline__ Bf3 load_frag(const u32x4* __restrict__ pk, int frag, int lane) {
diff --git a/fourierflow_amd/csrc/pointwise.hip b/fourierflow_amd/csrc/pointwise.hip
--- a/fourierflow_amd/csrc/pointwise.hip
+++ b/fourierflow_amd/csrc/pointwise.hip
@@ -1,4 +1,5 @@
 #include "ffno_device.h"
+#include "ffno_prep.h"
 #include "ffno.h"
 
 #include <math.h>
@@ -15,10 +16,7 @@
     const int lane = threadIdx.x & 63, row = blockIdx.x * 4 + (threadIdx.x >> 6);
     if (row >= d.rows) return;
     const float* v = d.v + (long)row * d.cols;
-    float ss = 0.f;
-    for (int c = lane; c < d.cols; c += 64) ss += v[c] * v[c];
-    ss = wave_sum(ss);
-    const float scale = d.g[row] / sqrtf(ss);
+    const float scale = wn_row_scale(d.g, d.v, row, d.cols, lane);
     float* w = d.w + (long)row * d.cols;
     for (int c = lane; c < d.cols; c += 64) w[c] = v[c] * scale;
 }
@@ -234,17 +232,22 @@
 
 static constexpr int kHeadMaxOut = 8;
 
+template <class SrcA, class SrcB>
+__device__ __forceinline__ void head_fold_body(const SrcA& Wa, const float* __restrict__ ca, const SrcB& Wb,
+                                               const float* __restrict__ cb, float* fold, int C, int D, int O, int bx) {
+    const int e = bx * 4 + (threadIdx.x >> 6), lane = threadIdx.x & 63;
+    if (e >= O * (C + 1)) return;
+    const int o = e / (C + 1), c = e % (C + 1);
+    float s = 0.f;
+    for (int jd = lane; jd < D; jd += 64) s = fmaf(Wb(o * D + jd), (c == C) ? ca[jd] : Wa(jd * C + c), s);
+    FFNO_UNROLL
+    for (int m = 32; m >= 1; m >>= 1) s += __shfl_xor(s, m);
+    if (lane == 0) fold[e] = s + ((c == C) ? cb[o] : 0.f);
+}
 __global__ __launch_bounds__(256) void head_fold_kernel(const float* __restrict__ Wa, const float* __restrict__ ca,
                                                         const float* __restrict__ Wb, const float* __restrict__ cb,
                                                         float* fold, int C, int D, int O) {
-    const int e = blockIdx.x * 4 + (threadIdx.x >> 6), lane = threadIdx.x & 63;
-    if (e >= O * (C + 1)) return;
-    const int o = e / (C + 1), c = e % (C + 1);
-    float s = 0.f;
-    for (int jd = lane; jd < D; jd += 64) s = fmaf(Wb[o * D + jd], (c == C) ? ca[jd] : Wa[jd * C + c], s);
-    FFNO_UNROLL
-    for (int m = 32; m >= 1; m >>= 1) s += __shfl_xor(s, m);
-    if (lane == 0) fold[e] = s + ((c == C) ? cb[o] : 0.f);
+    head_fold_body(StoredWeights{Wa}, ca, StoredWeights{Wb}, cb, fold, C, D, O, blockIdx.x);
 }
 
 template <int C, class ST = StF32>
@@ -780,20 +783,167 @@
     const float* x;
     size_t n;
 };
-__global__ __launch_bounds__(256) void amax_batched_kernel(const AmaxDesc* __restrict__ descs, unsigned* word) {
-    __shared__ float red[4];
-    const AmaxDesc d = descs[blockIdx.y];
-    const size_t act = min((size_t)gridDim.x, (d.n + 1023) / 1024);
-    if (blockIdx.x >= act) return;
+__device__ __forceinline__ void amax_body(const AmaxDesc d, unsigned* word, float* red, unsigned bx, unsigned nb) {
+    const size_t act = min((size_t)nb, (d.n + 1023) / 1024);
+    if (bx >= act) return;
     float m = 0.f;
     const bool al = (reinterpret_cast<uintptr_t>(d.x) & 15u) == 0;
     const size_t n4 = al ? d.n / 4 : 0;
-    for (size_t i = (size_t)blockIdx.x * 256 + threadIdx.x; i < n4; i += act * 256) {
+    for (size_t i = (size_t)bx * 256 + threadIdx.x; i < n4; i += act * 256) {
         const float4 v = reinterpret_cast<const float4*>(d.x)[i];
         m = fmaxf(fmaxf(m, fmaxf(fabsf(v.x), fabsf(v.y))), fmaxf(fabsf(v.z), fabsf(v.w)));
     }
-    for (size_t i = 4 * n4 + (size_t)blockIdx.x * 256 + threadIdx.x; i < d.n; i += act * 256) m = fmaxf(m, fabsf(d.x[i]));
+    for (size_t i = 4 * n4 + (size_t)bx * 256 + threadIdx.x; i < d.n; i += act * 256) m = fmaxf(m, fabsf(d.x[i]));
     range_fold(m, red, 4, word);
+}
+__global__ __launch_bounds__(256) void amax_batched_kernel(const AmaxDesc* __restrict__ descs, unsigned* word) {
+    __shared__ float red[4];
+    amax_body(descs[blockIdx.y], word, red, blockIdx.x, gridDim.x);
+}
+
+struct PrepSections {
+    int b_fold, b_wn, b_x3, b_fw, b_amax;
+    int bpj_fx, bpj_wn, bpj_x3, bpj_fw, bpj_amax;
+};
+static constexpr int kPrepMaxRows = 256;
+
+template <int NPL>
+__device__ __forceinline__ float wn_write_rows(const ffno_wn_desc& d, int r0, int lane) {
+    float x[4][NPL], sc[4];
+    wn_row_scales<NPL, 4>(d.g, d.v, r0, 4, d.rows, d.cols, lane, x, sc);
+    float m = 0.f;
+    FFNO_UNROLL
+    for (int u = 0; u < 4; ++u) {
+        const int row = r0 + 4 * u;
+        FFNO_UNROLL
+        for (int q = 0; q < NPL; ++q) {
+            const int c = lane + 64 * q;
+            if (row < d.rows && c < d.cols) {
+                const float w = x[u][q] * sc[u];
+                d.w[(long)row * d.cols + c] = w;
+                m = fmaxf(m, fabsf(w));
+            }
+        }
+    }
+    return m;
+}
+
+__device__ __forceinline__ void range_fold_if_larger(float m, float* red, int nwaves, unsigned* word) {
+    FFNO_UNROLL
+    for (int s = 32; s >= 1; s >>= 1) m = fmaxf(m, __shfl_xor(m, s));
+    if ((threadIdx.x & 63) == 0) red[threadIdx.x >> 6] = m;
+    __syncthreads();
+    if (threadIdx.x == 0) {
+        for (int w = 1; w < nwaves; ++w) m = fmaxf(m, red[w]);
+        if (f2u(m) != 0u && f2u(m) > __atomic_load_n(word, __ATOMIC_RELAXED)) atomicMax(word, f2u(m));
+    }
+}
+
+template <class S>
+__global__ __launch_bounds__(256) void step_prepare_kernel(const ffno_prep_plan P, const PrepSections s) {
+    __shared__ float scale[kPrepMaxRows + kHeadMaxOut];
+    __shared__ float red[4];
+    const int b = blockIdx.x, lane = threadIdx.x & 63, wave = threadIdx.x >> 6;
+    if (b < s.b_fold) {
+        const ffno_fxprep_desc d = P.fx[b / s.bpj_fx];
+        const int t = (b % s.bpj_fx) * 256 + threadIdx.x;
+        if (!d.g) {
+            fx_pack_body<S>(StoredWeights{d.src}, reinterpret_cast<u32x4*>(d.dst), d.sh, d.sc, d.type, P.C, P.H, t);
+            return;
+        }
+        const int frag0 = ((b % s.bpj_fx) * 256) >> 6;
+        const int w = d.type == 1 ? frag0 / (P.C / 16) : (frag0 >> 1) / (P.C / 32);
+        const bool hid_rows = d.sh == d.cols;
+        const int row0 = hid_rows ? 32 * w : 0, nrows = hid_rows ? 32 : P.C;
+        if (hid_rows)
+            wn_scales_to_lds<8>(d.g, d.src, row0, nrows, d.cols, scale, wave, lane);
+        else
+            wn_scales_to_lds<4>(d.g, d.src, row0, nrows, d.cols, scale, wave, lane);
+        __syncthreads();
+        fx_pack_body<S>(NormedWeights{d.src, scale, d.cols, row0}, reinterpret_cast<u32x4*>(d.dst), d.sh, d.sc, d.type, P.C, P.H, t);
+    } else if (b < s.b_wn) {
+        if (!P.head_ga) {
+            head_fold_body(StoredWeights{P.head_wa}, P.head_ca, StoredWeights{P.head_wb}, P.head_cb, P.fold, P.C, P.D, P.O,
+                           b - s.b_fold);
+            return;
+        }
+        wn_scales_to_lds<8>(P.head_ga, P.head_wa, 0, P.D, P.C, scale, wave, lane);
+        wn_scales_to_lds<8>(P.head_gb, P.head_wb, 0, P.O, P.D, scale + P.D, wave, lane);
+        __syncthreads();
+        head_fold_body(NormedWeights{P.head_wa, scale, P.C, 0}, P.head_ca, NormedWeights{P.head_wb, scale + P.D, P.D, 0},
+                       P.head_cb, P.fold, P.C, P.D, P.O, b - s.b_fold);
+    } else if (b < s.b_x3) {
+        const ffno_wn_desc d = P.wn[(b - s.b_wn) / s.bpj_wn];
+        const int rb = (b - s.b_wn) % s.bpj_wn;
+        if (rb * 16 >= d.rows) return;
+        float m = 0.f;
+        if (d.cols <= 64)
+            m = wn_write_rows<1>(d, rb * 16 + wave, lane);
+        else if (d.cols <= 128)
+            m = wn_write_rows<2>(d, rb * 16 + wave, lane);
+        else if (d.cols <= 256)
+            m = wn_write_rows<4>(d, rb * 16 + wave, lane);
+        else
+            for (int row = rb * 16 + wave; row < min(rb * 16 + 16, d.rows); row += 4) {
+                const float* v = d.v + (long)row * d.cols;
+                const float sc = wn_row_scale(d.g, d.v, row, d.cols, lane);
+                float* wo = d.w + (long)row * d.cols;
+                for (int c = lane; c < d.cols; c += 64) {
+                    const float x = v[c] * sc;
+                    wo[c] = x;
+                    m = fmaxf(m, fabsf(x));
+                }
+            }
+        if (P.word && P.wn_amax) range_fold_if_larger(m, red, 4, P.word);
+    } else if (b < s.b_fw) {
+        const ffno_x3prep_desc d = P.x3[(b - s.b_x3) / s.bpj_x3];
+        x3_pack_body(ParamPlanes{d.w, d.K, d.transposed}, reinterpret_cast<u32x4*>(d.dst), d.K, d.format,
+                     ((b - s.b_x3) % s.bpj_x3) * 256 + (int)threadIdx.x);
+    } else if (b < s.b_amax) {
+        const ffno_fwpack_desc d = P.fw[(b - s.b_fw) / s.bpj_fw];
+        fw_pack_body(d.w, d.wp, d.wpt, P.C, d.K, d.real, (b - s.b_fw) % s.bpj_fw, s.bpj_fw);
+    } else {
+        const ffno_amax_desc d = P.amax[(b - s.b_amax) / s.bpj_amax];
+        amax_body(AmaxDesc{d.x, d.n}, P.word, red, (b - s.b_amax) % s.bpj_amax, s.bpj_amax);
+    }
+}
+
+extern "C" int ffno_step_prepare_supported(int C, int H) { return (C == 64 && H % 32 == 0 && H >= 32) ? 1 : 0; }
+
+extern "C" int ffno_step_prepare(const ffno_prep_plan* plan, void* stream) {
+    if (!plan) return FFNO_EINVAL;
+    const ffno_prep_plan& P = *plan;
+    if (!ffno_step_prepare_supported(P.C, P.H)) return FFNO_EUNSUPPORTED;
+    if (P.n_wn < 0 || P.n_fx < 0 || P.n_fw < 0 || P.n_x3 < 0 || P.n_amax < 0) return FFNO_EINVAL;
+    if ((P.n_wn && (!P.wn || P.wn_max_rows <= 0)) || (P.n_fx && !P.fx) || (P.n_fw && (!P.fw || P.fw_max_K <= 0)) ||
+        (P.n_x3 && (!P.x3 || P.x3_max_K <= 0)) || (P.n_amax && (!P.amax || !P.word || P.amax_max_n == 0)))
+        return FFNO_EINVAL;
+    if (P.n_fx && P.ff_split != FFNO_FF_BF16X3 && P.ff_split != FFNO_FF_FP16X2) return FFNO_EINVAL;
+    if (P.x3_max_K > 64) return FFNO_EUNSUPPORTED;
+    const bool head = P.fold != nullptr;
+    if (head) {
+        if (!P.head_wa || !P.head_ca || !P.head_wb || !P.head_cb || P.D <= 0 || P.O <= 0) return FFNO_EINVAL;
+        if (!P.head_ga != !P.head_gb) return FFNO_EINVAL;
+        if (P.D > kPrepMaxRows || P.O > kHeadMaxOut) return FFNO_EUNSUPPORTED;
+    }
+    PrepSections s;
+    s.bpj_fx = (P.C * P.H / 8 + 255) / 256;
+    s.bpj_wn = (P.wn_max_rows + 15) / 16;
+    s.bpj_x3 = P.x3_max_K * 16 * 64 / 256;
+    s.bpj_fw = (int)std::min(((long)P.C * P.C * P.fw_max_K * 2 + 255) / 256, 256L);
+    s.bpj_amax = (int)std::min<size_t>(128, (P.amax_max_n + 2047) / 2048);
+    s.b_fold = P.n_fx * s.bpj_fx;
+    s.b_wn = s.b_fold + (head ? (P.O * (P.C + 1) + 3) / 4 : 0);
+    s.b_x3 = s.b_wn + P.n_wn * s.bpj_wn;
+    s.b_fw = s.b_x3 + P.n_x3 * s.bpj_x3;
+    s.b_amax = s.b_fw + P.n_fw * s.bpj_fw;
+    const int nblocks = s.b_amax + P.n_amax * s.bpj_amax;
+    if (nblocks <= 0) return FFNO_EINVAL;
+    if (P.ff_split == FFNO_FF_FP16X2)
+        FFNO_LAUNCH((step_prepare_kernel<SplitHf2>), dim3(nblocks), dim3(256), 0, (hipStream_t)stream, P, s);
+    else
+        FFNO_LAUNCH((step_prepare_kernel<SplitBf3>), dim3(nblocks), dim3(256), 0, (hipStream_t)stream, P, s);
+    return pw_status();
 }
 extern "C" int ffno_amax_batched(const ffno_amax_desc* descs_dev, int n, size_t max_n, uint32_t* word, void* stream) {
     static_assert(sizeof(ffno_amax_desc) == sizeof(AmaxDesc), "descriptor layout");
diff --git a/fourierflow_amd/csrc/spectral.hip b/fourierflow_amd/csrc/spectral.hip
--- a/fourierflow_amd/csrc/spectral.hip
+++ b/fourierflow_amd/csrc/spectral.hip
@@ -1,5 +1,6 @@
 #include "ffno_device.h"
 #include "ffno_lines.h"
+#include "ffno_prep.h"
 #include "ffno.h"
 
 namespace ffno {
@@ -263,17 +264,7 @@
 
 __global__ void fw_pack_batched_kernel(const ffno_fwpack_desc* __restrict__ descs, int C) {
     const ffno_fwpack_desc d = descs[blockIdx.y];
-    const int K = d.K;
-    const long total = (long)C * C * K * 2;
-    for (long e = (long)blockIdx.x * blockDim.x + threadIdx.x; e < total; e += (long)gridDim.x * blockDim.x) {
-        const int o = e % C;
-        const int i = (e / C) % C;
-        const int ri = (e / ((long)C * C)) % 2;
-        const int k = e / ((long)C * C * 2);
-        const float v = d.real ? (ri ? 0.f : d.w[((long)i * C + o) * K + k]) : d.w[(((long)i * C + o) * K + k) * 2 + ri];
-        d.wp[e] = v;
-        d.wpt[(((long)k * 2 + ri) * C + o) * C + i] = v;
-    }
+    fw_pack_body(d.w, d.wp, d.wpt, C, d.K, d.real, blockIdx.x, gridDim.x);
 }
 
 template <int C, bool REAL = false>
diff --git a/fourierflow_amd/csrc/spectral_x3.hip b/fourierflow_amd/csrc/spectral_x3.hip
--- a/fourierflow_amd/csrc/spectral_x3.hip
+++ b/fourierflow_amd/csrc/spectral_x3.hip
@@ -4,6 +4,7 @@
 #include "ffno_lines.h"
 #include "ffno_x3_dft.h"
 #include "ffno_infer_body.h"
+#include "ffno_prep.h"
 #include "ffno.h"
 
 namespace ffno {
@@ -43,41 +44,9 @@
 };
 
 __global__ __launch_bounds__(256) void x3_pack_kernel(const X3PackDesc* __restrict__ descs) {
-    constexpr int C = X3Cfg::C;
+    static_assert(X3Cfg::C == 64 && X3Cfg::MODE_FRAGS == 16, "x3_pack_body is written for these");
     const X3PackDesc d = descs[blockIdx.y];
-    const int nfrag = d.K * X3Cfg::MODE_FRAGS;
-    const int t = blockIdx.x * blockDim.x + threadIdx.x;
-    if (t >= nfrag * 64) return;
-    const int frag = t >> 6, lane = t & 63, j = lane & 31, half = lane >> 5;
-    const int pt = frag & 3, st = (frag >> 2) & 3, k = frag >> 4;
-    const int p = pt >> 1, tt = pt & 1;
-    const float* src = d.planes + ((long)(k * 2 + p) * C + (16 * st + 8 * half)) * C + 2 * j + tt;
-    float v[8];
-    FFNO_UNROLL
-    for (int e = 0; e < 8; ++e) v[e] = src[(long)e * C];
-    if (d.format == 1) {
-        const Hf2 f = split2_8(v[0], v[1], v[2], v[3], v[4], v[5], v[6], v[7]);
-        const int fo = (k * 4 + pt) * 4 + st;
-        d.dst[(fo * 2 + 0) * 64 + lane] = f.hi;
-        d.dst[(fo * 2 + 1) * 64 + lane] = f.lo;
-        return;
-    }
-    if (d.format == 2) {
-        const int fm = frag & 15, s2 = fm & 1, t16 = (fm >> 1) & 3, pp = fm >> 3;
-        const int j16 = lane & 15, g = lane >> 4;
-        const float* src2 = d.planes + ((long)(k * 2 + pp) * C + (32 * s2 + 8 * g)) * C + 4 * j16 + t16;
-        float w[8];
-        FFNO_UNROLL
-        for (int e = 0; e < 8; ++e) w[e] = src2[(long)e * C];
-        const Hf2 f = split2_8(w[0], w[1], w[2], w[3], w[4], w[5], w[6], w[7]);
-        d.dst[(frag * 2 + 0) * 64 + lane] = f.hi;
-        d.dst[(frag * 2 + 1) * 64 + lane] = f.lo;
-        return;
-    }
-    const Bf3 f = split3_8(v[0], v[1], v[2], v[3], v[4], v[5], v[6], v[7]);
-    d.dst[(frag * 3 + 0) * 64 + lane] = f.hi;
-    d.dst[(frag * 3 + 1) * 64 + lane] = f.mid;
-    d.dst[(frag * 3 + 2) * 64 + lane] = f.lo;
+    x3_pack_body(StoredPlanes{d.planes}, d.dst, d.K, d.format, (int)(blockIdx.x * blockDim.x + threadIdx.x));
 }
 
 __device__ __forceinline__ Bf3 x3_load_frag(const u32x4* __restrict__ pk, int frag, int lane) {
diff --git a/fourierflow_amd/engine.py b/fourierflow_amd/engine.py
--- a/fourierflow_amd/engine.py
+++ b/fourierflow_amd/engine.py
@@ -272,6 +272,7 @@
         self.infer_min_lines = None
         self.timer = None
         self.weight_range_check_every = 1
+        self.step_edges = True
         self._read_environment()
 
     def _read_environment(self):
@@ -314,8 +315,10 @@
         self._fx_flat = None
         self._fx_dev = None
         self._n_fx = 0
+        self._fxprep_dev = None
         self._fwpack = _lib.CachedTable()
         self._x3pack = _lib.CachedTable()
+        self._x3prep = _lib.CachedTable()
         self._wr_word = None
         self._wr_late = _DeferredWord(self.device)
         self._wr_table = _lib.CachedTable()
@@ -509,7 +512,7 @@
             words = int((lib.ffno_ffh_pack_bytes if self._h2() else lib.ffno_ffx_pack_bytes)(self.C, self.H)) // 4
             if self._fx_flat is None or self._fx_flat.numel() != 4 * words * len(blocks):
                 self._fx_flat = torch.empty(4 * words * len(blocks), dtype=torch.int32, device=self.device)
-            fdescs = []
+            fdescs, pdescs = [], []
             for bi, pfx in enumerate(blocks):
                 l0, l1 = self.linears[pfx + "layers.0.0."], self.linears[pfx + "layers.1.0."]
                 pk = [self._fx_flat[(4 * bi + q) * words:(4 * bi + q + 1) * words] for q in range(4)]
@@ -519,8 +522,15 @@
                 for (src, sh, sc, ty), dst in zip(((l0.weff, C_, 1, 1), (l1.weff, 1, H_, 2), (l1.weff, 1, H_, 1),
                                                    (l0.weff, C_, 1, 2)), pk):
                     fdescs.append(_capi.FxPackDesc(src.data_ptr(), dst.data_ptr(), sh, sc, ty, 0))
+                for (lin, sh, sc, ty), dst in zip(((l0, C_, 1, 1), (l1, 1, H_, 2), (l1, 1, H_, 1), (l0, C_, 1, 2)), pk):
+                    if lin.wnorm:
+                        g, v = self.params[lin.prefix + "weight_g"], self.params[lin.prefix + "weight_v"]
+                        pdescs.append(_capi.FxPrepDesc(v.data_ptr(), g.data_ptr(), dst.data_ptr(), sh, sc, ty, lin.cols))
+                    else:
+                        pdescs.append(_capi.FxPrepDesc(lin.weff.data_ptr(), None, dst.data_ptr(), sh, sc, ty, lin.cols))
             self._n_fx = len(fdescs)
             self._fx_dev = _lib.device_table(_capi.FxPackDesc, fdescs, self.device)
+            self._fxprep_dev = _lib.device_table(_capi.FxPrepDesc, pdescs, self.device)
         self._max_rows = max([l.rows for l in self.linears.values()])
         self._desc_dev = _lib.device_table(_capi.WnDesc, descs, self.device) if descs else None
 
@@ -683,6 +693,9 @@
         if sig is not None and sig == self._prep_sig:
             return
         self._prep_sig = sig
+        if self._step_prepare_ok():
+            self._step_prepare(st, x3fmt)
+            return
         if self._desc_dev is not None:
             self._k("weightnorm_fwd", lib.ffno_weightnorm_fwd, _p(self._desc_dev), self._n_desc, self._max_rows, st)
         if self._ffx() and self._n_fx:
@@ -707,10 +720,19 @@
         self._check_weight_range(st, x3fmt)
 
     def _check_weight_range(self, st, x3fmt: List[int]):
+        srcs = self._weight_range_due(x3fmt)
+        if srcs is None:
+            return
+        rows = tuple((t.data_ptr(), t.numel()) for t in srcs)
+        self._k("amax", _lib.get_lib().ffno_amax_batched, _p(self._wr_table.get(_capi.AmaxDesc, rows, self.device)), len(rows),
+                max(n for _, n in rows), _p(self._wr_word), st)
+        self._wr_late.post(self._wr_word)
+
+    def _weight_range_due(self, x3fmt: List[int]):
         every = int(self.weight_range_check_every)
         fp16_ff, fp16_mix = self._ffx() and self._h2(), any(x3fmt)
         if every <= 0 or not (fp16_ff or fp16_mix):
-            return
+            return None
         host = self._wr_late.take()
         if host is not None:
             wmax = float(host.view(torch.float32)[0])
@@ -726,8 +748,7 @@
                     f"engine.ff_split = engine.x3_mix_split = 'bf16x3' (FFNO_FF_SPLIT / FFNO_X3_MIX_SPLIT) -- any fp32 range")
         self._wr_count += 1
         if (self._wr_count - 1) % every or self._wr_late.pending:
-            return
-        lib = _lib.get_lib()
+            return None
         if self._wr_word is None:
             self._wr_word = torch.zeros(1, dtype=torch.int32, device=self.device)
         self._wr_word.zero_()
@@ -739,10 +760,41 @@
                 srcs += [self.params[p + "weight"] for p in self.linears if "_ff." in p and p + "weight" in self.params]
         if fp16_mix:
             srcs += [self.params[n] for names in self._fw_sets for n in names]
-        rows = tuple((t.data_ptr(), t.numel()) for t in srcs)
-        self._k("amax", lib.ffno_amax_batched, _p(self._wr_table.get(_capi.AmaxDesc, rows, self.device)), len(rows),
-                max(n for _, n in rows), _p(self._wr_word), st)
-        self._wr_late.post(self._wr_word)
+        return srcs
+
+    def _step_prepare_ok(self) -> bool:
+        return bool(self.step_edges and self.nd == 2 and self.spectral == "factorized" and self._plain_layer and self._ffx()
+                    and self.O <= 8 and _lib.get_lib().ffno_step_prepare_supported(self.C, self.H))
+
+    def _step_prepare(self, st, x3fmt: List[int]):
+        lib, dev = _lib.get_lib(), self.device
+        srcs = self._weight_range_due(x3fmt)
+        wn_amax = bool(srcs) and srcs[0] is self.weff_flat
+        srcs = (srcs or [])[1:] if wn_amax else (srcs or [])
+        amax_rows = tuple((t.data_ptr(), t.numel()) for t in srcs)
+        fw_rows = tuple((self.params[n].data_ptr(), self.planes[i][w][0].data_ptr(), self.planes[i][w][1].data_ptr(), self.Ks[w], 0)
+                        for i, names in enumerate(self._fw_sets) for w, n in enumerate(names))
+        x3_rows = ()
+        if self.use_x3 and self._fw_sets:
+            x3_rows = tuple((self.params[self._fw_sets[i][w]].data_ptr(), xp[d].data_ptr(), self.Ks[w], x3fmt[w], d, 0)
+                            for i, row in enumerate(self.xplanes) for w, xp in enumerate(row) if xp is not None for d in range(2))
+        o0, o1 = "out.0.", "out.1."
+        wname = "weight_v" if self.wnorm else "weight"
+        gp = (lambda p: _p(self.params[p + "weight_g"])) if self.wnorm else (lambda p: None)
+        plan = _capi.PrepPlan(
+            _p(self._desc_dev) if self._desc_dev is not None else None, _p(self._fxprep_dev),
+            _p(self._fwpack.get(_capi.FwPackDesc, fw_rows, dev)) if fw_rows else None,
+            _p(self._x3prep.get(_capi.X3PrepDesc, x3_rows, dev)) if x3_rows else None,
+            _p(self._wr_table.get(_capi.AmaxDesc, amax_rows, dev)) if amax_rows else None,
+            _p(self._wr_word) if (wn_amax or amax_rows) else None, max([n for _, n in amax_rows] or [0]),
+            _p(self.params[o0 + wname]), gp(o0), _p(self.params[o0 + "bias"]),
+            _p(self.params[o1 + wname]), gp(o1), _p(self.params[o1 + "bias"]), _p(self.fold),
+            self._n_desc, self._max_rows if self._n_desc else 0, int(wn_amax), self._n_fx, int(self._h2()),
+            len(fw_rows), max(self.Ks) if fw_rows else 0, len(x3_rows), max([r[2] for r in x3_rows] or [0]), len(amax_rows),
+            self.C, self.H, HEAD_DIM, self.O)
+        self._k("step_prepare", lib.ffno_step_prepare, ctypes.byref(plan), st)
+        if wn_amax or amax_rows:
+            self._wr_late.post(self._wr_word)
 
     def _ff_weights(self, l, prefixes=None):
         fp = (prefixes or self.ff_prefix)[l]
diff --git a/include/ffno.h b/include/ffno.h
--- a/include/ffno.h
+++ b/include/ffno.h
@@ -21,7 +21,7 @@
 #define FFNO_MODE_NOFOURIER 2
 
 const char* ffno_build_target(void);
-#define FFNO_ABI_VERSION 13
+#define FFNO_ABI_VERSION 14
 int ffno_abi_version(void);
 
 int ffno_amax(const float* x, size_t n, uint32_t* word, void* stream);
@@ -320,6 +320,42 @@
 int ffno_weightnorm_fwd(const ffno_wn_desc* descs_dev, int n, int max_rows, void* stream);
 int ffno_weightnorm_bwd(const ffno_wn_desc* descs_dev, int n, int max_rows, void* stream);
 
+typedef struct ffno_fxprep_desc {
+    const float* src;
+    const float* g;
+    void* dst;
+    int32_t sh, sc;
+    int32_t type;
+    int32_t cols;
+} ffno_fxprep_desc;
+typedef struct ffno_x3prep_desc {
+    const float* w;
+    void* dst;
+    int32_t K, format;
+    int32_t transposed;
+    int32_t pad_;
+} ffno_x3prep_desc;
+typedef struct ffno_prep_plan {
+    const ffno_wn_desc* wn;
+    const ffno_fxprep_desc* fx;
+    const ffno_fwpack_desc* fw;
+    const ffno_x3prep_desc* x3;
+    const ffno_amax_desc* amax;
+    uint32_t* word;
+    size_t amax_max_n;
+    const float *head_wa, *head_ga, *head_ca, *head_wb, *head_gb, *head_cb;
+    float* fold;
+    int32_t n_wn, wn_max_rows;
+    int32_t wn_amax;
+    int32_t n_fx, ff_split;
+    int32_t n_fw, fw_max_K;
+    int32_t n_x3, x3_max_K;
+    int32_t n_amax;
+    int32_t C, H, D, O;
+} ffno_prep_plan;
+int ffno_step_prepare_supported(int C, int H);
+int ffno_step_prepare(const ffno_prep_plan* plan, void* stream);
+
 typedef struct ffno_tr_desc {
     const float* src;
     float* dst;
```

After: 182.2. About the same (-0.3%).
